# CalciferZh/MinimalOptiX

Measured on AMD Instinct MI355X. Metric: Mrays/s (primary+bounce+shadow rays traced per second, coffee.obj 1920x1080 256spp), higher is better.
Workload: dtype f32

## Files before the change

minimaloptix_amd/csrc/api_context.h:

```cpp
#pragma once
#include <hip/hip_runtime.h>

#include <initializer_list>
#include <string>
#include <vector>

#include "../../include/moptix.h"
#include "lbvh.h"
#include "megakernel.h"
#include "refitkernel.h"
#include "pt_signtopo.h"

struct ncclComm;

namespace pt { namespace api {

template <class T> struct DevBuf {
  T* p = nullptr; size_t n = 0;
  hipError_t ensure(size_t count) {
    if (count <= n && p) return hipSuccess;
    if (p) { (void)hipFree(p); p = nullptr; n = 0; }
    hipError_t e = hipMalloc((void**)&p, sizeof(T) * (count ? count : 1));
    if (e == hipSuccess) n = count ? count : 1;
    return e;
  }
  hipError_t upload(const std::vector<T>& v, hipStream_t s) {
    hipError_t e = ensure(v.size());
    if (e != hipSuccess || v.empty()) return e;
    return hipMemcpyAsync(p, v.data(), sizeof(T) * v.size(), hipMemcpyHostToDevice, s);
  }
  void release() { if (p) (void)hipFree(p); p = nullptr; n = 0; }
};

struct OrderList {
  long long units = -1;
  DevBuf<unsigned int> keys, keysSorted; DevBuf<int> order, iota; DevBuf<uint8_t> sortTmp;
  hipError_t ensure(long long n, hipStream_t stream);
  hipError_t sort(hipStream_t stream);
  void forget() { units = -1; }
  void release() { keys.release(); keysSorted.release(); order.release(); iota.release(); sortTmp.release(); units = -1; }
};

struct Options {
  int exitThreshold = 16, leafSize = 4, blocksPerCU = 3;
  int kernelVariant = -1;
  int tileMajor = 3;
  int starveLanes = 16, sampleBufMB = 16384, leafThreshold = 16, swapLanes = 32;
  int watchdogMs = 600000;
  int nodeFormat = 0;
  int fastShading = 0;
  int builder = 1;
  int analyticQueue = -1;
  int autoPacket = 1;
  int commBlocking = 0;
  int commTimeoutMs = 120000;
  int shadowRule = 1;
  int slotsInUse = -1;
  int drainBelow = 64;
  int auxDepth = 16;
  int specialize = 1;
  int queryBlocksPerCU = 32;
  int temporalFaceMotion = 0;
  int radianceBufferMB = 256;
};

}}

struct moptix_context_t {
  template <class T> using DevBuf = pt::api::DevBuf<T>;

  int device = 0;
  int numCUs = 256;
  hipStream_t stream = nullptr; bool ownStream = false;
  hipEvent_t ev0 = nullptr, ev1 = nullptr, ev2 = nullptr;
  std::string err;
  bool poisoned = false;
  moptix_params params{}; bool haveParams = false;
  int rank = 0, nRanks = 1;
  pt::api::Options opt;

  std::vector<pt::DevMaterial> mats;
  std::vector<pt::DevSphere> spheres; std::vector<int> sphereMat;
  std::vector<pt::DevQuad> quads;
  std::vector<pt::DevLight> lights;
  std::vector<float> facePos, faceNrm; std::vector<int> faceHasNrm, faceMat;
  std::vector<pt::TriUV> faceUV; bool anyUV = false;
  struct HostTexture { int width, height; std::vector<float> rgba; };
  std::vector<HostTexture> textures;
  bool sceneDirty = true, accelBuilt = false;
  DevBuf<pt::DevMaterial> dMats; DevBuf<pt::DevSphere> dSpheres; DevBuf<int> dSphereMat; DevBuf<pt::DevQuad> dQuads; DevBuf<pt::DevLight> dLights;
  DevBuf<float> dFacePos, dFaceNrm; DevBuf<int> dFaceHasNrm, dFaceMat;
  DevBuf<pt::TriUV> dFaceUV; DevBuf<float> dTexels; DevBuf<pt::DevTexture> dTextures;
  pt::LbvhResult bvh;
  double glassFaceShare = 0.0;
  void release_scene() {
    dMats.release(); dSpheres.release(); dSphereMat.release(); dQuads.release(); dLights.release();
    dFacePos.release(); dFaceNrm.release(); dFaceHasNrm.release(); dFaceMat.release();
    dFaceUV.release(); dTexels.release(); dTextures.release();
    pt::lbvh_free(&bvh);
  }

  DevBuf<float> dAccum; float* accumBound = nullptr; size_t accumPixels = 0;
  bool accumPlain = false;
  DevBuf<uint8_t> dRgb8;

  int nodeFormatUsed = 128;
  bool formatDecided = false;
  unsigned long long probeCounts[4] = { 0, 0, 0, 0 };
  int lastVariant = -1;
  int lastFeatures = pt::FEAT_ALL;
  int countedSpanUs = -1, countedTailUs = -1;
  double kernelMs = 0.0, reduceMs = 0.0; uint64_t nLaunches = 0;
  bool asyncPending = false;
  std::vector<int> seedStaging;
  DevBuf<int> dSeeds; DevBuf<int> dWork; DevBuf<unsigned long long> dCounters; DevBuf<int> dOverflow;
  DevBuf<uint8_t> dPoolCold; DevBuf<float> dSampleBuf;
  void release_render() {
    dSeeds.release(); dWork.release(); dCounters.release(); dOverflow.release(); dPoolCold.release(); dSampleBuf.release();
    tiles.release();
  }
  pt::api::OrderList tiles;

  struct Comm {
    ncclComm* handle = nullptr; int rank = 0, ranks = 1;
    bool nonBlocking = false;
    DevBuf<float> tileSend, tileRecv;
  } comm;

  struct Aov {
    DevBuf<float> albedo, normal, depth, hits; DevBuf<int> primId, matId;
    moptix_aov_buffers bound{};
    size_t pixels = 0;
    uint64_t samples = 0;
    DevBuf<int> seeds, work, overflow;
    void frame_resized() { pixels = 0; samples = 0; }
    void release() {
      albedo.release(); normal.release(); depth.release(); hits.release(); primId.release(); matId.release();
      seeds.release(); work.release(); overflow.release();
    }
  } aov;

  struct Denoise {
    DevBuf<pt::v4> colA, colB, guide, side; DevBuf<float> out;
    float* bound = nullptr;
    size_t pixels = 0;
    void release() { colA.release(); colB.release(); guide.release(); side.release(); out.release(); pixels = 0; }
  } dn;

  struct Temporal {
    DevBuf<pt::v4> col[2], guide[2], mom[2];
    DevBuf<pt::v4> motion;
    DevBuf<float> motionOut, historyOut;
    DevBuf<unsigned long long> counters;
    DevBuf<unsigned int> partials;
    std::vector<pt::v4> motionHost;
    int cur = 0;
    bool have = false;
    uint32_t width = 0, height = 0; int nSpheres = 0, demodulate = 0;
    moptix_cam_params cam{}; std::vector<pt::v3> centres;
    uint64_t frames = 0;
    size_t pixels = 0;
    unsigned long long last[4] = { 0, 0, 0, 0 };
    struct Faces {
      DevBuf<float> prev;
      DevBuf<pt::v4> rec;
      DevBuf<unsigned int> partials;
      DevBuf<unsigned long long> counters;
      bool have = false; size_t count = 0;
      bool changed = true;
      unsigned long long last[3] = { 0, 0, 0 };
      void release() { prev.release(); rec.release(); partials.release(); counters.release(); have = false; count = 0; }
    } faces;
    void drop() { have = false; frames = 0; faces.have = false; }
    void release() {
      for (int i = 0; i < 2; i++) { col[i].release(); guide[i].release(); mom[i].release(); }
      motion.release(); motionOut.release(); historyOut.release(); counters.release(); partials.release();
      faces.release();
      drop(); pixels = 0;
    }
  } tp;

  struct Adaptive {
    DevBuf<uint32_t> count; DevBuf<float> moments, error; DevBuf<uint8_t> converged;
    pt::api::OrderList order;
    DevBuf<unsigned int> partials, totals;
    DevBuf<float> mean;
    size_t pixels = 0;
    bool have = false;
    void drop() { pixels = 0; have = false; }
    void release() {
      count.release(); moments.release(); error.release(); converged.release();
      order.release(); partials.release(); totals.release(); mean.release();
      drop();
    }
  } ad;

  struct Query {
    DevBuf<int> overflow;
    DevBuf<float> rays; DevBuf<uint8_t> out;
    void drop() { overflow.release(); }
    void release() { drop(); rays.release(); out.release(); }
  } query;

  struct Radiance {
    DevBuf<int> overflow;
    DevBuf<float> scratch; DevBuf<int> work, seeds;
    int* seedStaging = nullptr; size_t seedStagingN = 0;
    hipEvent_t seedsUploaded = nullptr;
    DevBuf<float> rays, out; DevBuf<uint32_t> states;
    void drop() { overflow.release(); }
    void release() {
      drop(); scratch.release(); work.release(); seeds.release(); rays.release(); out.release(); states.release();
      if (seedStaging) (void)hipHostFree(seedStaging);
      if (seedsUploaded) (void)hipEventDestroy(seedsUploaded);
      seedStaging = nullptr; seedStagingN = 0; seedsUploaded = nullptr;
    }
  } radiance;

  struct Point {
    DevBuf<unsigned long long> overflow;
    DevBuf<float> points; DevBuf<uint8_t> out;
    void drop() { overflow.release(); }
    void release() { drop(); points.release(); out.release(); }
  } point;

  struct Sign {
    bool have = false, uploaded = false, stale = true;
    pt::SignTopology topo;
    uint32_t tableBuilds = 0;
    DevBuf<int> faceIds, vertexStart, vertexCorner, edgeStart, edgeFace;
    DevBuf<pt::SignFace> faces; DevBuf<pt::v4> vertexN, edgeN; DevBuf<pt::SignRecord> table;
    void release() {
      faceIds.release(); vertexStart.release(); vertexCorner.release(); edgeStart.release(); edgeFace.release();
      faces.release(); vertexN.release(); edgeN.release(); table.release();
      topo = pt::SignTopology(); have = false; uploaded = false; stale = true; tableBuilds = 0;
    }
  } sign;

  struct Refit {
    bool facesDirty = false, hostStale = false;
    size_t facesOnDevice = 0;
    bool planned = false;
    DevBuf<int> levelOrder; std::vector<int> levelFirst;
    DevBuf<pt::RefitBox> raw; DevBuf<uint32_t> sceneBox; DevBuf<double> partials; DevBuf<pt::RefitCost> cost; DevBuf<int> bad;
    struct Pinned { pt::RefitCost cost; int bad; }* pinned = nullptr;
    hipEvent_t e0 = nullptr, e1 = nullptr;
    moptix_refit_info info{};
    void drop() {
      levelOrder.release(); levelFirst.clear(); raw.release(); sceneBox.release(); partials.release(); cost.release(); bad.release();
      if (pinned) (void)hipHostFree(pinned);
      if (e0) (void)hipEventDestroy(e0);
      if (e1) (void)hipEventDestroy(e1);
      pinned = nullptr; e0 = nullptr; e1 = nullptr; planned = false; info = moptix_refit_info{};
    }
  } refit;
};

namespace pt {
struct DenoiseConsts;
namespace api {

int fail(moptix_context c, int code, const std::string& msg);
int hipFail(moptix_context c, hipError_t e, const char* what);
#define HIPCHK(c, x, what) do { hipError_t e_ = (x); if (e_ != hipSuccess) return pt::api::hipFail((c), e_, (what)); } while (0)

int check_ready(moptix_context c);
int fetch_faces(moptix_context c);
int sign_table_for_query(moptix_context c, const SignRecord*& table);
void sign_release(moptix_context c);
float* accum_ptr(moptix_context c);
int ensure_accum(moptix_context c);
int begin_call(moptix_context c, bool withAccum);
struct ReadBack { void* dst; const void* src; size_t bytes; };
int read_back(moptix_context c, std::initializer_list<ReadBack> copies, const char* what);
void fill_view(moptix_context c, SceneView& v);
int scene_features(moptix_context c);
int fill_query_view(moptix_context c, SceneView& v);
moptix_aov_buffers aov_ptrs(moptix_context c);
void comm_release(moptix_context c);
int denoise_begin(moptix_context c, bool ownGuide, size_t& px);
void denoise_consts(moptix_context c, const moptix_denoise_params* p, DenoiseConsts& k);
inline float* denoise_out(moptix_context c) { return c->dn.bound ? c->dn.bound : c->dn.out.p; }

struct LaunchPlan {
  const TraceKernel* kernel;
  int variant;
  int features;
  int nItems, tilesX;
  int nBlocks;
  long long perPass;
  int slotsInUse, auxDepth, drainBelow, ovfDepth;
  int tileMajor, unitShift; long long historyUnits;
  size_t poolBytes, overflowInts, workInts;
};
struct RenderLaunch {
  LaunchPlan p; LaunchArgs a;
  long long perPass;
  int handoutDivisor, handoutSeeds;
  bool counted, fast;
};
struct PassOverride {
  const int* order; int nWork;
  hipError_t (*reduce)(hipStream_t stream, const LaunchArgs& a, void* user); void* user;
};
int prepare_launch(moptix_context c, int32_t nSeeds, bool counted, bool byPixelSlots, RenderLaunch& r);
int launch_pass(moptix_context c, RenderLaunch& r, const int* dSeeds, int n, const PassOverride* over);

}}
```

minimaloptix_amd/csrc/api_options.hip:

```cpp
#include <climits>
#include <cstring>

#include "api_context.h"

using namespace pt;
using namespace pt::api;

namespace {

enum Invalidates { kNothing, kAccelIfChanged, kNodeFormat, kTileHistory, kFaceSnapshot };
struct Option {
  const char* name;
  int Options::* member;
  int (*read)(moptix_context) = nullptr;
  int lo = 0, hi = 0;
  const char* accepted = "";
  Invalidates invalidates = kNothing;
  int nValues = 0, values[4] = { 0, 0, 0, 0 };
  bool can_set() const { return !read; }
  bool can_get() const { return member || read; }
};

static_assert(kMaxLeaf == 8, "leaf_size's message says [1,8]");
const Option kOptions[] = {
  { "exit_threshold", &Options::exitThreshold, nullptr, 0, 64, "in [0,64]" },
  { "leaf_size", &Options::leafSize, nullptr, 1, kMaxLeaf, "in [1,8]", kAccelIfChanged },
  { "blocks_per_cu", &Options::blocksPerCU, nullptr, 1, 8, "in [1,8]" },
  { "kernel_variant", &Options::kernelVariant, nullptr, 0, 0, "in {-1,0,3,4} (1 and 2 were removed in round 3)", kNothing, 4, { -1, 0, 3, 4 } },
  { "sample_buffer_mb", &Options::sampleBufMB, nullptr, 1, INT_MAX, ">= 1" },
  { "leaf_threshold", &Options::leafThreshold, nullptr, 1, 64, "in [1,64]" },
  { "swap_lanes", &Options::swapLanes, nullptr, 1, 64, "in [1,64]" },
  { "starve_lanes", &Options::starveLanes, nullptr, 1, 64, "in [1,64]" },
  { "tile_major", &Options::tileMajor, nullptr, 0, 3, "in {0,1,2,3}" },
  { "auto_packet", &Options::autoPacket, nullptr, 0, 1, "in {0,1}" },
  { "analytic_queue", &Options::analyticQueue, nullptr, -1, 1, "in {-1,0,1}" },
  { "aux_depth", &Options::auxDepth, nullptr, 0, 100000, "in [0,100000]" },
  { "drain_below", &Options::drainBelow, nullptr, 0, 64, "in [0,64]" },
  { "specialize", &Options::specialize, nullptr, 0, 1, "in {0,1}" },
  { "slots_in_use", &Options::slotsInUse, nullptr, -1, 1024, "in [-1,1024]" },
  { "builder", &Options::builder, nullptr, 0, 1, "in {0,1}", kAccelIfChanged },
  { "fast_shading", &Options::fastShading, nullptr, 0, 1, "in {0,1}" },
  { "node_format", &Options::nodeFormat, nullptr, 0, 0, "in {0,64,128}", kNodeFormat, 3, { 0, 64, 128 } },
  { "shadow_rule", &Options::shadowRule, nullptr, 0, 1, "in {0,1}" },
  { "watchdog_ms", &Options::watchdogMs, nullptr, 1, INT_MAX, ">= 1" },
  { "comm_timeout_ms", &Options::commTimeoutMs, nullptr, 1, INT_MAX, ">= 1" },
  { "comm_blocking", &Options::commBlocking, nullptr, 0, 1, "in {0,1}" },
  { "query_blocks_per_cu", &Options::queryBlocksPerCU, nullptr, 1, 64, "in [1,64]" },
  { "radiance_buffer_mb", &Options::radianceBufferMB, nullptr, 1, 16384, "in [1,16384]" },
  { "temporal_face_motion", &Options::temporalFaceMotion, nullptr, 0, 1, "in {0,1}", kFaceSnapshot },
  { "forget_history", nullptr, nullptr, INT_MIN, INT_MAX, "", kTileHistory },
  { "comm_nonblocking_used", nullptr, [](moptix_context c) { return c->comm.nonBlocking ? 1 : 0; } },
  { "node_format_used", nullptr, [](moptix_context c) { return c->nodeFormatUsed; } },
  { "kernel_variant_used", nullptr, [](moptix_context c) { return c->lastVariant; } },
  { "kernel_features_used", nullptr, [](moptix_context c) { return c->lastFeatures; } },
  { "counted_span_us", nullptr, [](moptix_context c) { return c->countedSpanUs; } },
  { "counted_tail_us", nullptr, [](moptix_context c) { return c->countedTailUs; } },
  { "path_slots", nullptr, [](moptix_context) { return packetkernel_slots(); } },
  { "comm_ranks", nullptr, [](moptix_context c) { return c->comm.handle ? c->comm.ranks : 0; } },
  { "num_cus", nullptr, [](moptix_context c) { return c->numCUs; } },
};
const Option* find_option(const char* name) {
  for (const Option& o : kOptions) if (!strcmp(name, o.name)) return &o;
  return nullptr;
}

}

extern "C" {

int moptix_set_option(moptix_context c, const char* name, int32_t value) {
  if (!c || !name) return MOPTIX_ERR_INVALID;
  const Option* o = find_option(name);
  if (!o || !o->can_set()) return fail(c, MOPTIX_ERR_INVALID, std::string("unknown option: ") + name);
  bool ok = o->nValues == 0 && value >= o->lo && value <= o->hi;
  for (int i = 0; i < o->nValues; i++) ok = ok || value == o->values[i];
  if (!ok) return fail(c, MOPTIX_ERR_INVALID, std::string(name) + " " + o->accepted);
  if (o->invalidates == kAccelIfChanged && value != c->opt.*o->member) c->accelBuilt = false;
  if (o->invalidates == kNodeFormat) c->formatDecided = false;
  if (o->invalidates == kTileHistory) c->tiles.forget();
  if (o->invalidates == kFaceSnapshot && value == 0 && c->tp.faces.prev.p) {
    (void)hipSetDevice(c->device);
    if (!c->poisoned) (void)hipStreamSynchronize(c->stream);
    c->tp.faces.release();
  }
  if (o->invalidates == kFaceSnapshot && value == 0) c->tp.faces.have = false;
  if (o->member) c->opt.*o->member = value;
  return MOPTIX_OK;
}

int moptix_get_option(moptix_context c, const char* name, int32_t* value) {
  if (!c || !name || !value) return MOPTIX_ERR_INVALID;
  const Option* o = find_option(name);
  if (!o || !o->can_get()) return fail(c, MOPTIX_ERR_INVALID, std::string("unknown option: ") + name);
  *value = o->member ? c->opt.*o->member : o->read(c);
  return MOPTIX_OK;
}

}
```

minimaloptix_amd/csrc/api_render.hip:

```cpp
#include <rocprim/rocprim.hpp>

#include <algorithm>
#include <cstdio>
#include <cstdlib>
#include <cstring>

#include "api_context.h"
#include "pt_lanestack.h"

using namespace pt;
using namespace pt::api;

namespace {

constexpr int kProbeWidth = 128;
int choose_node_format(moptix_context c) {
  c->formatDecided = true;
  c->nodeFormatUsed = 128;
  for (auto& v : c->probeCounts) v = 0;
  if (c->bvh.nNodes <= 0 || !c->bvh.nodes64) return MOPTIX_OK;
  if (c->opt.nodeFormat != 0) { c->nodeFormatUsed = c->opt.nodeFormat; return MOPTIX_OK; }
  SceneView v; fill_view(c, v);
  v.nodes64 = c->bvh.nodes64;
  const int w = std::min(kProbeWidth, v.width), h = std::max(1, (int)((long long)v.height * w / std::max(1, v.width)));
  v.width = w; v.height = h;
  const size_t threads = ((size_t)w * h + 255) / 256 * 256;
  unsigned long long* dOut = nullptr; int* dOvf = nullptr;
  hipError_t e = hipMalloc((void**)&dOut, 4 * sizeof(unsigned long long));
  if (e == hipSuccess) e = hipMemsetAsync(dOut, 0, 4 * sizeof(unsigned long long), c->stream);
  const size_t ovf = lane_stack_overflow_entries(threads, c->bvh.stackBound, megakernel_lds_stack_entries());
  if (e == hipSuccess && ovf > 0) e = hipMalloc((void**)&dOvf, sizeof(int) * ovf);
  if (e == hipSuccess) e = launch_probe_paths(c->stream, v, 0, false, dOut, dOvf);
  if (e == hipSuccess) e = launch_probe_paths(c->stream, v, 0, true, dOut + 2, dOvf);
  if (e == hipSuccess) e = hipMemcpyAsync(c->probeCounts, dOut, 4 * sizeof(unsigned long long), hipMemcpyDeviceToHost, c->stream);
  if (e == hipSuccess) e = hipStreamSynchronize(c->stream);
  if (dOut) (void)hipFree(dOut);
  if (dOvf) (void)hipFree(dOvf);
  if (e != hipSuccess) return hipFail(c, e, "node format probe");
  const double cost128 = (double)c->probeCounts[0] + 1.3 * (double)c->probeCounts[1];
  const double cost64 = 0.93 * (double)c->probeCounts[2] + 1.3 * (double)c->probeCounts[3];
  c->nodeFormatUsed = cost64 < cost128 ? 64 : 128;
  if (getenv("MOPTIX_DEBUG"))
    fprintf(stderr, "[moptix] node format probe (%dx%d paths): 128-byte nodes %llu steps %llu triangle tests, 64-byte %llu / %llu -> %d\n", w, h,
            c->probeCounts[0], c->probeCounts[1], c->probeCounts[2], c->probeCounts[3], c->nodeFormatUsed);
  return MOPTIX_OK;
}

void report_counters(const unsigned long long* h) {
  fprintf(stderr, "[moptix] batches %llu lanes %llu full %llu allidle %llu waitingSum %llu\n", h[kCntShadeBatches], h[kCntShadeBatchLanes], h[kCntLeafBacklog], h[kCntIdleSpins], h[kCntRingBacklog]);
  const double tt = (double)h[kCntTWave];
  fprintf(stderr, "[moptix] wave time: batch %.1f%% refill %.1f%% node %.1f%% leaf %.1f%% finish %.1f%% (steps %llu, cycles/wave %.3g)\n",
          100 * h[kCntTBatch] / tt, 100 * h[kCntTSwap] / tt, 100 * h[kCntTNode] / tt, 100 * h[kCntTLeaf] / tt, 100 * h[kCntTFinish] / tt, h[kCntTraversalSteps], tt);
  fprintf(stderr, "[moptix] idle spins %llu\n", h[kCntIdleSpins]);
  if (h[kCntLastWaveOut] && h[kCntFirstWaveIn] != ~0ull && h[kCntLastWaveOut] > h[kCntFirstWaveIn])
    fprintf(stderr, "[moptix] pass ticks: batch %llu (load %llu run %llu store %llu) node %llu leaf %llu txn %llu lock %llu local %llu idle %llu | waves' time %llu over a span of %.1f us | "
                    "batches %llu node runs %llu leaf passes %llu iterations %llu transactions %llu\n", h[kCntTBatch], h[kCntTBatchLoad], h[kCntTBatchRun], h[kCntTBatchStore], h[kCntTNode], h[kCntTLeaf], h[kCntTTxn], h[kCntTLock], h[kCntTLocal], h[kCntTIdle], h[kCntTWave],
            (double)(h[kCntLastWaveOut] - h[kCntFirstWaveIn]) * 1e-2, h[kCntShadeBatches], h[kCntNodeRuns], h[kCntLeafPasses], h[kCntIterations], h[kCntTransactions]);
  if (h[kCntIterations]) fprintf(stderr, "[moptix] swap detail: local %.1f%% lock-wait %.1f%% txn %.1f%% idle %.1f%% | batch detail: load %.1f%% run %.1f%% store %.1f%% | "
                     "iterations %llu transactions %llu (cycles/iter %.0f)\n", 100 * h[kCntTLocal] / tt, 100 * h[kCntTLock] / tt, 100 * h[kCntTTxn] / tt, 100 * h[kCntTIdle] / tt,
                     100 * h[kCntTBatchLoad] / tt, 100 * h[kCntTBatchRun] / tt, 100 * h[kCntTBatchStore] / tt, h[kCntIterations], h[kCntTransactions], tt / (double)h[kCntIterations]);
  if (h[kCntLastWaveOut]) fprintf(stderr, "[moptix] timeline (100 MHz clock): items ran out %.2f ms after the first wave started, last wave left %.2f ms after that\n",
                     (double)(h[kCntItemsRanOut] - h[kCntFirstWaveIn]) * 1e-5, (double)(h[kCntLastWaveOut] - h[kCntItemsRanOut]) * 1e-5);
  if (h[kCntLastWaveOut]) {
    int lastB = 0; for (int b = 0; b < kCntTailBuckets; b++) if (h[kCntTailCount + b]) lastB = b;
    const int ranOut = (int)((double)(h[kCntItemsRanOut] - h[kCntFirstWaveIn]) * 1e-5);
    fprintf(stderr, "[moptix] samples finishing per ms from the moment the items ran out (count, mean depth, max depth):");
    for (int b = ranOut > 2 ? ranOut - 2 : 0; b <= lastB; b++)
      fprintf(stderr, " [%d: %llu %.1f %llu]", b, h[kCntTailCount + b], h[kCntTailCount + b] ? (double)h[kCntTailDepthSum + b] / (double)h[kCntTailCount + b] : 0.0, h[kCntTailMaxDepth + b]);
    fprintf(stderr, "\n");
  }
  if (h[kCntNodeRuns]) fprintf(stderr, "[moptix] node runs %llu: node-ready slots waiting in the wave's ring %.1f, leaf ring %.1f (averages at the start of a run)\n",
                     h[kCntNodeRuns], (double)h[kCntRingBacklog] / (double)h[kCntNodeRuns], (double)h[kCntLeafBacklog] / (double)h[kCntNodeRuns]);
  if (h[kCntIterations]) fprintf(stderr, "[moptix] batch iterations executing on_result %llu, on_lights %llu, new item %llu (batches %llu)\n", h[kCntIterResult], h[kCntIterLights], h[kCntIterNewItem], h[kCntShadeBatches]);
  if ((h[kCntSlotRows] | h[kCntSlotRows + 1])) {
    const double rays = (double)(h[kCntPrimaryRays] + h[kCntBounceRays] + h[kCntShadowRays]);
    fprintf(stderr, "[moptix] slot-record rows (16 B each) per ray: shading visit loads %.2f stores %.2f | leaf pass loads %.2f stores %.2f | total %.1f B per ray in %.2f shading visits and %.2f leaf visits per ray\n",
            h[kCntSlotRows] / rays, h[kCntSlotRows + 1] / rays, h[kCntSlotRows + 2] / rays, h[kCntSlotRows + 3] / rays, 16.0 * (double)(h[kCntSlotRows] + h[kCntSlotRows + 1] + h[kCntSlotRows + 2] + h[kCntSlotRows + 3]) / rays, (double)h[kCntShadeBatchLanes] / rays, (double)h[kCntLeafLanes] / rays);
  }
  if ((h[kCntHandedOver] | h[kCntDrainTaken])) fprintf(stderr, "[moptix] hand-over: %llu paths handed over by the packet kernel, %llu taken by the drain kernel; samples finished: %llu by the packet kernel + %llu by the drain kernel (of %llu)\n", h[kCntHandedOver], h[kCntDrainTaken], h[kCntPacketFinished], h[kCntDrainFinished], h[kCntSamples]);
  if (h[kCntLeafPasses]) fprintf(stderr, "[moptix] node steps %llu (%.1f lanes avg), leaf passes %llu (%.1f lanes avg)\n", h[kCntTraversalSteps] - h[kCntLeafPasses],
          (double)(h[kCntActiveLaneSteps] - h[kCntLeafLanes]) / (double)(h[kCntTraversalSteps] - h[kCntLeafPasses]), h[kCntLeafPasses], (double)h[kCntLeafLanes] / (double)h[kCntLeafPasses]);
  if (h[kCntCensusWaves]) {
    static const char* names[kCensusRegions] = { "result visit (on_result_packet)", "  miss", "  closest hit (hit_attributes + material)", "    light material",
      "    depth cap", "    lambertian", "    metal", "    glass", "    disney GLASS", "    disney (on_lights_packet)", "      light 0 faces: pdf + eval", "      light 1 faces: pdf + eval",
      "      light 2 faces: pdf + eval", "      bounce: pdf + eval", "new work item (begin_sample)", "leaf pass: triangle 0 tested", "leaf pass: triangle 1 tested",
      "leaf pass: triangle 2 tested", "leaf pass: triangle 3 tested", "  triangle hit accepted by tri_test", "  shadow result folded", "      light draw (per light)", "      bounce: disney_sample", "node step: branched tail (stack nearly full)" };
    fprintf(stderr, "[moptix] lane census: region | waves that entered | lanes that entered | lanes per wave (of 64)\n");
    for (int i = 0; i < kCensusRegions; i++)
      if (h[kCntCensusWaves + i]) fprintf(stderr, "[moptix]   %-46s %12llu %14llu %6.1f\n", names[i], h[kCntCensusWaves + i], h[kCntCensusLanes + i], (double)h[kCntCensusLanes + i] / (double)h[kCntCensusWaves + i]);
  }
}

int read_stats(moptix_context c, moptix_stats* stats) {
  unsigned long long h[kCntTotal] = {};
  HIPCHK(c, hipMemcpy(h, c->dCounters.p, sizeof(h), hipMemcpyDeviceToHost), "read counters");
  stats->samples = h[kCntSamples]; stats->primaryRays = h[kCntPrimaryRays]; stats->bounceRays = h[kCntBounceRays]; stats->shadowRays = h[kCntShadowRays];
  stats->nodeFetches = h[kCntNodeFetches]; stats->triTests = h[kCntTriTests]; stats->closestHits = h[kCntClosestHits]; stats->lightLoads = h[kCntLightLoads];
  stats->analyticTests = h[kCntAnalyticTests]; stats->traversalSteps = h[kCntTraversalSteps]; stats->activeLaneSteps = h[kCntActiveLaneSteps];
  stats->shadeBatches = h[kCntShadeBatches]; stats->shadeBatchLanes = h[kCntShadeBatchLanes];
  c->countedSpanUs = -1; c->countedTailUs = -1;
  if (h[kCntLastWaveOut] && h[kCntFirstWaveIn] != ~0ull) { c->countedSpanUs = (int)((h[kCntLastWaveOut] - h[kCntFirstWaveIn]) / 100); c->countedTailUs = (h[kCntItemsRanOut] != ~0ull && h[kCntLastWaveOut] > h[kCntItemsRanOut]) ? (int)((h[kCntLastWaveOut] - h[kCntItemsRanOut]) / 100) : 0; }
  if (getenv("MOPTIX_DEBUG")) report_counters(h);
  return MOPTIX_OK;
}

int plan_launch(moptix_context c, const SceneView& scene, int32_t nSeeds, bool byPixelSlots, LaunchPlan& p) {
  memset(&p, 0, sizeof(p));
  const int tilesX = ((int)c->params.width + 7) / 8, tilesY = ((int)c->params.height + 7) / 8;
  const long long nTiles = (long long)tilesX * tilesY;
  const long long localTiles = (nTiles + c->nRanks - 1) / c->nRanks;
  if (localTiles * 64 > 0x7fffffffLL) return fail(c, MOPTIX_ERR_LIMIT, "frame too large");
  p.nItems = (int)(localTiles * 64); p.tilesX = tilesX;
  if (p.nItems == 0) return MOPTIX_OK;
  const long long budget = (long long)c->opt.sampleBufMB << 20;
  p.perPass = budget / ((long long)p.nItems * 12);
  p.nBlocks = c->numCUs * c->opt.blocksPerCU;
  const long long counterSlack = (long long)c->numCUs * std::max(4, c->opt.blocksPerCU) * 1024 + 65536;
  if ((long long)p.nItems + counterSlack > 0x7fffffffLL) return fail(c, MOPTIX_ERR_LIMIT, "frame too large");
  p.perPass = std::min(p.perPass, (0x7fffffffLL - counterSlack) / p.nItems);
  p.perPass = std::max(1LL, std::min(p.perPass, (long long)nSeeds));

  const bool hasTris = scene.rootRef != kEmptyRef;
  const bool analyticQueue = c->opt.analyticQueue >= 0 ? c->opt.analyticQueue != 0 : (c->spheres.size() + c->quads.size() >= 64);
  const bool packetOk = hasTris && scene.nLights <= 3 && !scene.anyDisneyAnalytic;
  const double nSamples = (double)p.nItems * (double)nSeeds;
  const bool autoPacket = nSamples >= 1.0e6 && nSeeds >= 16;
  const bool variantExplicit = c->opt.kernelVariant >= 0;
  const int variant = variantExplicit ? c->opt.kernelVariant : 3;
  const bool usePacket = packetOk && (variant == 4 || (!variantExplicit && c->opt.autoPacket != 0 && autoPacket));
  const bool useQueue = !usePacket && (byPixelSlots || ((variant >= 3) && (hasTris || analyticQueue)));
  p.kernel = usePacket ? &kPacketKernel : !useQueue ? nullptr : hasTris ? &kQueueKernel : &kLeanQueueKernel;
  p.variant = usePacket ? 4 : useQueue ? 3 : 0;
  const bool faceTableOk = (unsigned long long)tri_face_offset(0) + (unsigned long long)scene.nTris * (sizeof(TriShade) + sizeof(TriFace)) + 64ull < (1ull << 32);
  p.features = (usePacket && c->opt.specialize != 0 && faceTableOk) ? scene_features(c) : FEAT_ALL;
  if (p.kernel == &kLeanQueueKernel && c->opt.blocksPerCU == 3) p.nBlocks = c->numCUs * 4;
  p.slotsInUse = c->opt.slotsInUse >= 0 ? c->opt.slotsInUse : (usePacket && c->opt.auxDepth > 0 && nSamples < 1.0e8 && c->glassFaceShare <= 0.5 ? packetkernel_slots() * 7 / 8 : 0);
  p.auxDepth = usePacket ? c->opt.auxDepth : 0;
  if (usePacket) {
    bool glassMaterial = false;
    for (const DevMaterial& m : c->mats) if (m.kind == MAT_DISNEY && m.brdfType == BRDF_GLASS) glassMaterial = true;
    p.drainBelow = (glassMaterial && !scene.shadowNearest) ? 0 : c->opt.drainBelow;
  }
  if (p.kernel) {
    p.ovfDepth = hasTris ? std::max(0, c->bvh.stackBound - p.kernel->lds_stack_entries() + 1) : 0;
    p.overflowInts = p.ovfDepth > 0 ? p.kernel->overflow_ints(p.nBlocks, p.ovfDepth) : 0;
    p.poolBytes = p.kernel->cold_bytes(p.nBlocks);
  } else {
    p.overflowInts = lane_stack_overflow_entries((size_t)p.nBlocks * 256, c->bvh.stackBound, megakernel_lds_stack_entries());
  }
  p.workInts = kHandoutWords + 2 + drain_list_ints(p.nBlocks, p.drainBelow);
  p.tileMajor = byPixelSlots ? 3 : p.kernel ? c->opt.tileMajor : 0;
  p.unitShift = p.tileMajor == 3 ? 0 : 6;
  p.historyUnits = (localTiles * 64) >> p.unitShift;
  return MOPTIX_OK;
}

int report_tile_history(moptix_context c) {
  std::vector<unsigned int> cost((size_t)c->tiles.units);
  HIPCHK(c, hipMemcpy(cost.data(), c->tiles.keys.p, sizeof(unsigned int) * cost.size(), hipMemcpyDeviceToHost), "read tile cost");
  size_t hist[6] = { 0, 0, 0, 0, 0, 0 };
  for (size_t i = 0; i < cost.size(); i++) {
    const unsigned int v = cost[i];
    hist[v == 0 ? 0 : v < 16 ? 1 : v < 64 ? 2 : v < 256 ? 3 : 4]++;
    if (v >= 256 && i < cost.size() / 2) hist[5]++;
  }
  fprintf(stderr, "[moptix] depth history (%zu units): none %zu, depth 8-15 %zu, 16-63 %zu, 64-255 %zu, capped %zu (of which %zu in the first half)\n",
          cost.size(), hist[0], hist[1], hist[2], hist[3], hist[4], hist[5]);
  return MOPTIX_OK;
}

#ifdef PT_EVLOG
constexpr size_t kEvLogWords = 65536;
int evlog_begin(moptix_context c, DevBuf<unsigned long long>& evLog, LaunchArgs& a) {
  HIPCHK(c, evLog.ensure(kEvLogWords + 8), "alloc event log");
  HIPCHK(c, hipMemsetAsync(evLog.p, 0, sizeof(unsigned long long) * (kEvLogWords + 8), c->stream), "zero event log");
  a.evLog = evLog.p;
  return MOPTIX_OK;
}
int evlog_write(moptix_context c, const DevBuf<unsigned long long>& evLog) {
  std::vector<unsigned long long> h(kEvLogWords);
  HIPCHK(c, hipMemcpy(h.data(), evLog.p, sizeof(unsigned long long) * h.size(), hipMemcpyDeviceToHost), "read event log");
  FILE* f = fopen(getenv("MOPTIX_EVLOG"), "wb");
  if (f) { fwrite(h.data(), sizeof(unsigned long long), (size_t)std::min<unsigned long long>(h[0], 65000ull) + 1, f); fclose(f); }
  return MOPTIX_OK;
}
#endif

}

namespace pt { namespace api {

int prepare_launch(moptix_context c, int32_t nSeeds, bool counted, bool byPixelSlots, RenderLaunch& r) {
  int rc;
  if (!c->formatDecided && (rc = choose_node_format(c)) != MOPTIX_OK) return rc;
  LaunchArgs& a = r.a;
  LaunchPlan& p = r.p;
  memset(&a, 0, sizeof(a));
  fill_view(c, a.scene);
  if ((rc = plan_launch(c, a.scene, nSeeds, byPixelSlots, p)) != MOPTIX_OK || p.nItems == 0) return rc;
  c->lastVariant = p.variant;
  r.counted = counted; r.fast = c->opt.fastShading != 0;
  c->lastFeatures = p.kernel == &kPacketKernel ? packetkernel_features(r.counted, r.fast, p.features) : FEAT_ALL;

  a.accum = accum_ptr(c);
  a.nItems = p.nItems; a.tilesX = p.tilesX; a.rank = c->rank; a.nRanks = c->nRanks;
  a.exitThreshold = c->opt.exitThreshold; a.leafThreshold = c->opt.leafThreshold;
  a.starveLanes = c->opt.starveLanes; a.swapLanes = c->opt.swapLanes;
  a.slotsInUse = p.slotsInUse; a.auxDepth = p.auxDepth; a.ovfDepth = p.ovfDepth;
  a.watchdogTicks = (unsigned long long)c->opt.watchdogMs * 100000ull;
  if (p.overflowInts > 0) {
    HIPCHK(c, c->dOverflow.ensure(p.overflowInts), "alloc stack overflow area");
    a.stackOverflow = c->dOverflow.p;
  }
  if (p.kernel) {
    HIPCHK(c, c->dPoolCold.ensure(p.poolBytes), "alloc path pool");
    a.poolCold = c->dPoolCold.p;
  }
  long long perPass = p.perPass;
  for (;;) {
    const hipError_t e = c->dSampleBuf.ensure((size_t)perPass * a.nItems * 3);
    if (e == hipSuccess) break;
    if (e != hipErrorOutOfMemory || perPass <= 1) return hipFail(c, e, "alloc per-sample buffer");
    (void)hipGetLastError();
    perPass = (perPass + 1) / 2;
  }
  r.perPass = perPass;
  a.sampleBuf = c->dSampleBuf.p;
  HIPCHK(c, c->dWork.ensure(p.workInts), "alloc work counter");
  {
    struct { HandoutConsts hc; int hdr[2 + kDrainEntries]; } w = { handout_consts(p.tileMajor, a.nItems, (int)std::min<long long>(perPass, nSeeds), a.tilesX, a.nRanks),
                                                                   { 0, 0, 0, 0, 0, 0, p.nBlocks * p.drainBelow, p.drainBelow } };
    static_assert(sizeof(w) == sizeof(int) * (kHandoutWords + 2 + kDrainEntries), "the work header is packed");
    HIPCHK(c, hipMemcpyAsync(c->dWork.p, &w, sizeof(w), hipMemcpyHostToDevice, c->stream), "init work counter");
    HIPCHK(c, hipStreamSynchronize(c->stream), "sync");
    r.handoutDivisor = handout_divisor(p.tileMajor, a.nItems, (int)std::min<long long>(perPass, nSeeds)); r.handoutSeeds = (int)std::min<long long>(perPass, nSeeds);
  }
  a.workCounter = c->dWork.p + kHandoutWords;
  a.tileMajor = p.tileMajor; a.unitShift = p.unitShift;
  if (p.tileMajor) {
    HIPCHK(c, c->tiles.ensure(p.historyUnits, c->stream), "start depth history");
    a.tileOrder = c->tiles.order.p; a.tileCost = c->tiles.keys.p;
  }
  if (counted) {
    HIPCHK(c, c->dCounters.ensure(kCntTotal), "alloc counters");
    HIPCHK(c, hipMemsetAsync(c->dCounters.p, 0, sizeof(unsigned long long) * kCntTotal, c->stream), "zero counters");
    HIPCHK(c, hipMemsetAsync(c->dCounters.p + kCntFirstWaveIn, 0xff, sizeof(unsigned long long) * 2, c->stream), "init min counters");
    a.counters = c->dCounters.p;
  }
  return MOPTIX_OK;
}

static hipError_t sort_pairs_desc(void* tmp, size_t& tmpBytes, OrderList& l, size_t n, hipStream_t stream) {
  return rocprim::radix_sort_pairs_desc(tmp, tmpBytes, l.keys.p, l.keysSorted.p, l.iota.p, l.order.p, n, 0, 32, stream);
}

hipError_t OrderList::ensure(long long n, hipStream_t stream) {
  if (units == n) return hipSuccess;
  units = -1;
  std::vector<int> ids((size_t)n);
  for (size_t i = 0; i < ids.size(); i++) ids[i] = (int)i;
  hipError_t e = keys.ensure((size_t)n);
  if (e == hipSuccess) e = keysSorted.ensure((size_t)n);
  if (e == hipSuccess) e = order.ensure((size_t)n);
  if (e == hipSuccess) e = iota.upload(ids, stream);
  if (e == hipSuccess) e = hipMemsetAsync(keys.p, 0, sizeof(unsigned int) * (size_t)n, stream);
  size_t tmpBytes = 0;
  if (e == hipSuccess) e = sort_pairs_desc(nullptr, tmpBytes, *this, (size_t)n, stream);
  if (e == hipSuccess) e = sortTmp.ensure(tmpBytes);
  if (e == hipSuccess) e = hipStreamSynchronize(stream);
  if (e == hipSuccess) units = n;
  return e;
}

hipError_t OrderList::sort(hipStream_t stream) {
  size_t tmpBytes = sortTmp.n;
  return sort_pairs_desc(sortTmp.p, tmpBytes, *this, (size_t)units, stream);
}

int launch_pass(moptix_context c, RenderLaunch& r, const int* dSeeds, int n, const PassOverride* over) {
  LaunchArgs& a = r.a;
  const LaunchPlan& p = r.p;
  a.seeds = dSeeds; a.nSeeds = n; a.nWork = over ? over->nWork : n * a.nItems;
  if (handout_divisor(a.tileMajor, a.nItems, n) != r.handoutDivisor || n != r.handoutSeeds) {
    const HandoutConsts hc = handout_consts(a.tileMajor, a.nItems, n, a.tilesX, a.nRanks);
    HIPCHK(c, hipMemcpyAsync(a.workCounter - kHandoutWords, &hc, sizeof(hc), hipMemcpyHostToDevice, c->stream), "write hand-out constants");
    HIPCHK(c, hipStreamSynchronize(c->stream), "sync");
    r.handoutDivisor = handout_divisor(a.tileMajor, a.nItems, n); r.handoutSeeds = n;
  }
  HIPCHK(c, hipMemsetAsync(a.workCounter, 0, (2 + kDrainCap) * sizeof(int), c->stream), "zero work counter");
  if (over) a.tileOrder = over->order;
  else if (a.tileMajor && a.tileCost) HIPCHK(c, c->tiles.sort(c->stream), "sort tiles");
  HIPCHK(c, hipEventRecord(c->ev0, c->stream), "event");
  if (p.kernel) HIPCHK(c, p.kernel->launch(c->stream, a, p.nBlocks, r.counted, r.fast, p.features), p.kernel->launchWhat);
  else HIPCHK(c, launch_megakernel(c->stream, a, p.nBlocks, r.counted), "launch megakernel");
  if (p.drainBelow > 0) HIPCHK(c, launch_drainkernel(c->stream, a, c->numCUs, r.counted, r.fast), "launch drain kernel");
  else if (p.kernel == &kPacketKernel) HIPCHK(c, launch_megakernel(c->stream, a, p.nBlocks, r.counted), "launch megakernel");
  HIPCHK(c, hipEventRecord(c->ev1, c->stream), "event");
  if (over) HIPCHK(c, over->reduce(c->stream, a, over->user), "launch adaptive reduction");
  else HIPCHK(c, launch_reduce_samples(c->stream, a), "launch sample reduction");
  HIPCHK(c, hipEventRecord(c->ev2, c->stream), "event");
  c->asyncPending = true;
  return MOPTIX_OK;
}

}}

namespace {

int do_render(moptix_context c, const int32_t* seeds, int32_t nSeeds, bool counted, bool blocking, moptix_stats* stats) {
  int rc = check_ready(c);
  if (rc != MOPTIX_OK) return rc;
  if (nSeeds < 0 || (nSeeds > 0 && !seeds)) return fail(c, MOPTIX_ERR_INVALID, "bad seeds");
  if (c->ad.have) return fail(c, MOPTIX_ERR_STATE, "the accumulation buffer holds an adaptive render (per-pixel sample counts): moptix_adaptive_clear or moptix_accum_clear first");
  if ((rc = begin_call(c, true)) != MOPTIX_OK) return rc;
  if (nSeeds == 0) return MOPTIX_OK;
  RenderLaunch r;
  if ((rc = prepare_launch(c, nSeeds, counted, false, r)) != MOPTIX_OK || r.p.nItems == 0) return rc;
#ifdef PT_EVLOG
  DevBuf<unsigned long long> evLog;
  if ((rc = evlog_begin(c, evLog, r.a)) != MOPTIX_OK) return rc;
#endif
  c->seedStaging.assign(seeds, seeds + nSeeds);
  HIPCHK(c, c->dSeeds.upload(c->seedStaging, c->stream), "upload seeds");
  c->accumPlain = true;

  for (long long first = 0; first < nSeeds; first += r.perPass) {
    const int n = (int)std::min(r.perPass, (long long)nSeeds - first);
    if ((rc = launch_pass(c, r, c->dSeeds.p + first, n, nullptr)) != MOPTIX_OK) return rc;
    const bool last = first + r.perPass >= nSeeds;
    if (!last || blocking) { if ((rc = moptix_sync(c)) != MOPTIX_OK) return rc; }
  }
#ifdef PT_EVLOG
  if (blocking && !counted && getenv("MOPTIX_EVLOG") && (rc = evlog_write(c, evLog)) != MOPTIX_OK) return rc;
  evLog.release();
#endif
  if (blocking && r.a.tileCost && getenv("MOPTIX_DEBUG") && (rc = report_tile_history(c)) != MOPTIX_OK) return rc;
  if (blocking && counted && stats) return read_stats(c, stats);
  return MOPTIX_OK;
}

}

extern "C" {

int moptix_launch(moptix_context c, int32_t randSeed) { return do_render(c, &randSeed, 1, false, true, nullptr); }
int moptix_render(moptix_context c, const int32_t* seeds, int32_t nSeeds) { return do_render(c, seeds, nSeeds, false, true, nullptr); }
int moptix_render_async(moptix_context c, const int32_t* seeds, int32_t nSeeds) { return do_render(c, seeds, nSeeds, false, false, nullptr); }
int moptix_render_counted(moptix_context c, const int32_t* seeds, int32_t nSeeds, moptix_stats* out) {
  if (out) memset(out, 0, sizeof(*out));
  return do_render(c, seeds, nSeeds, true, true, out);
}

int moptix_sync(moptix_context c) {
  if (!c) return MOPTIX_ERR_INVALID;
  HIPCHK(c, hipStreamSynchronize(c->stream), "stream synchronize");
  if (c->asyncPending) {
    float ms = 0.f, ms2 = 0.f;
    if (hipEventElapsedTime(&ms, c->ev0, c->ev1) == hipSuccess) { c->kernelMs += ms; c->nLaunches++; }
    if (hipEventElapsedTime(&ms2, c->ev1, c->ev2) == hipSuccess) c->reduceMs += ms2;
    c->asyncPending = false;
    int flags[2] = { 0, 0 };
    if (c->dWork.p) HIPCHK(c, hipMemcpy(flags, c->dWork.p + kHandoutWords, sizeof(flags), hipMemcpyDeviceToHost), "read watchdog flag");
    if (flags[1] != 0) return fail(c, MOPTIX_ERR_HIP, "render kernel hit its watchdog (option watchdog_ms); this pass was not added to accuBuffer");
  }
  return MOPTIX_OK;
}

}
```

minimaloptix_amd/csrc/megakernel.h:

```cpp
#pragma once
#include <hip/hip_runtime.h>
#include "pt_counters.h"
#include "pt_types.h"

namespace pt {

struct LaunchArgs {
  SceneView scene;
  const int* seeds; int nSeeds;
  float* accum;
  float* sampleBuf;
  int* workCounter;
  int nItems;
  int nWork;
  int tilesX; int rank, nRanks;
  int exitThreshold;
  int leafThreshold;
  int* stackOverflow;
  unsigned long long* counters;
  void* poolCold;
  int starveLanes;
  int swapLanes;
  int ovfDepth;
  int slotsInUse;
  int auxDepth;
  unsigned long long watchdogTicks;
  int tileMajor;
  int unitShift;
  const int* tileOrder;
  unsigned int* tileCost;
#ifdef PT_EVLOG
  unsigned long long* evLog;
#endif
};
constexpr int kDeepPath = 8;
constexpr int kDrainDeep = 24;
constexpr int kDrainList = 2, kDrainDeepN = 0, kDrainNext = 1, kDrainOtherN = 2, kDrainCap = 4, kDrainBelow = 5, kDrainEntries = 6;

PT_HD bool item_to_pixel(const LaunchArgs& a, int k, int& sample, int& pixel) {
  sample = k / a.nItems;
  const int i = k - sample * a.nItems;
  const int lt = i >> 6, in = i & 63;
  const int gt = lt * a.nRanks + (a.rank + lt) % a.nRanks;
  const int tx = gt % a.tilesX, ty = gt / a.tilesX;
  const int x = tx * 8 + (in & 7), y = ty * 8 + (in >> 3);
  pixel = y * a.scene.width + x;
  return (x < a.scene.width) & (y < a.scene.height);
}
PT_HD int handout_to_item(const LaunchArgs& a, int k) {
  if (!a.tileMajor) return k;
  if (a.tileMajor == 3) {
    const int ui = k / a.nSeeds, sample = k - ui * a.nSeeds;
    return sample * a.nItems + (a.tileOrder ? a.tileOrder[ui] : ui);
  }
  const int per = a.nSeeds << 6;
  const int ti = k / per, r = k - ti * per;
  const int lt = a.tileOrder ? a.tileOrder[ti] : ti;
  if (a.tileMajor == 2) {
    const int in = r / a.nSeeds, sample = r - in * a.nSeeds;
    return sample * a.nItems + (lt << 6) + in;
  }
  return (r >> 6) * a.nItems + (lt << 6) + (r & 63);
}
struct MagicDiv { unsigned int mul, shift; };
struct HandoutConsts { MagicDiv first, tilesX, ranks, seeds; };
constexpr int kHandoutWords = 8;
static_assert(sizeof(HandoutConsts) == kHandoutWords * sizeof(int), "HandoutConsts is kHandoutWords ints");
inline MagicDiv magic_div(int d) {
  int l = 0;
  while ((1ll << l) < (long long)d) l++;
  MagicDiv m; m.shift = 31u + (unsigned int)l;
  m.mul = (unsigned int)(((1ull << m.shift) + (unsigned long long)d - 1ull) / (unsigned long long)d);
  return m;
}
PT_HD int magic_quot(int n, MagicDiv m) { return (int)(((unsigned long long)(unsigned int)n * (unsigned long long)m.mul) >> m.shift); }
inline int handout_divisor(int tileMajor, int nItems, int nSeeds) { return !tileMajor ? nItems : tileMajor == 3 ? nSeeds : nSeeds << 6; }
inline HandoutConsts handout_consts(int tileMajor, int nItems, int nSeeds, int tilesX, int nRanks) {
  HandoutConsts h;
  h.first = magic_div(handout_divisor(tileMajor, nItems, nSeeds)); h.tilesX = magic_div(tilesX); h.ranks = magic_div(nRanks); h.seeds = magic_div(nSeeds);
  return h;
}

struct WorkItem { int item, sample, x, y, pixel; };
PT_HD bool handout_lean(const LaunchArgs& a, const HandoutConsts* hc, int k, WorkItem& w) {
  int slot;
  const int q = magic_quot(k, load_uniform(&hc->first));
  if (!a.tileMajor) {
    w.sample = q; slot = k - q * a.nItems;
  } else if (a.tileMajor == 3) {
    w.sample = k - q * a.nSeeds;
    slot = a.tileOrder ? a.tileOrder[q] : q;
  } else {
    const int r = k - q * (a.nSeeds << 6);
    const int lt = a.tileOrder ? a.tileOrder[q] : q;
    int in;
    if (a.tileMajor == 2) { in = magic_quot(r, load_uniform(&hc->seeds)); w.sample = r - in * a.nSeeds; }
    else { w.sample = r >> 6; in = r & 63; }
    slot = (lt << 6) + in;
  }
  w.item = a.tileMajor ? w.sample * a.nItems + slot : k;
  const int lt = slot >> 6, in = slot & 63;
  int gt = lt;
  if (__builtin_expect(a.nRanks != 1, 0)) { const int s = a.rank + lt; gt = lt * a.nRanks + (s - magic_quot(s, load_uniform(&hc->ranks)) * a.nRanks); }
  const int ty = magic_quot(gt, load_uniform(&hc->tilesX)), tx = gt - ty * a.tilesX;
  w.x = tx * 8 + (in & 7); w.y = ty * 8 + (in >> 3);
  w.pixel = w.y * a.scene.width + w.x;
  return (w.x < a.scene.width) & (w.y < a.scene.height);
}
#if defined(__HIPCC__)
__device__ __forceinline__ void store_sample(const LaunchArgs& a, int item, v3 value) {
  float* sp = a.sampleBuf + 3 * (size_t)item;
  sp[0] = value.x; sp[1] = value.y; sp[2] = value.z;
}
#endif

int megakernel_lds_stack_entries();
hipError_t launch_reduce_samples(hipStream_t stream, const LaunchArgs& a);
hipError_t launch_megakernel(hipStream_t stream, const LaunchArgs& a, int nBlocks, bool counted);
int queuekernel_lds_stack_entries();
int queuekernel_slots();
size_t queuekernel_cold_bytes(int nBlocks);
size_t queuekernel_overflow_ints(int nBlocks, int ovfDepth);
hipError_t launch_queuekernel(hipStream_t stream, const LaunchArgs& a, int nBlocks, bool counted, bool fastShading, int features);
int queuekernel_lds_stack_entries_lean();
int queuekernel_slots_lean();
size_t queuekernel_cold_bytes_lean(int nBlocks);
size_t queuekernel_overflow_ints_lean(int nBlocks, int ovfDepth);
hipError_t launch_queuekernel_lean(hipStream_t stream, const LaunchArgs& a, int nBlocks, bool counted, bool fastShading, int features);
int packetkernel_lds_stack_entries();
int packetkernel_slots();
size_t packetkernel_cold_bytes(int nBlocks);
size_t packetkernel_overflow_ints(int nBlocks, int ovfDepth);
hipError_t launch_packetkernel(hipStream_t stream, const LaunchArgs& a, int nBlocks, bool counted, bool fastShading, int features);
int packetkernel_features(bool counted, bool fastShading, int sceneFeatures);
struct TraceKernel {
  const char* launchWhat;
  int (*lds_stack_entries)();
  size_t (*cold_bytes)(int nBlocks);
  size_t (*overflow_ints)(int nBlocks, int ovfDepth);
  hipError_t (*launch)(hipStream_t stream, const LaunchArgs& a, int nBlocks, bool counted, bool fastShading, int features);
};
inline constexpr TraceKernel kQueueKernel = { "launch queue megakernel", queuekernel_lds_stack_entries, queuekernel_cold_bytes, queuekernel_overflow_ints, launch_queuekernel };
inline constexpr TraceKernel kLeanQueueKernel = { "launch queue megakernel (lean)", queuekernel_lds_stack_entries_lean, queuekernel_cold_bytes_lean, queuekernel_overflow_ints_lean, launch_queuekernel_lean };
inline constexpr TraceKernel kPacketKernel = { "launch packet megakernel", packetkernel_lds_stack_entries, packetkernel_cold_bytes, packetkernel_overflow_ints, launch_packetkernel };
hipError_t launch_drainkernel(hipStream_t stream, const LaunchArgs& a, int nCUs, bool counted, bool fastShading);
size_t drain_list_ints(int nBlocks, int drainBelow);
hipError_t launch_debug_trace(hipStream_t stream, const SceneView& sc, const float* dRays, int n, float* dT, int* dPrim, int* stackOverflow);
hipError_t launch_probe_paths(hipStream_t stream, const SceneView& sc, int launchSeed, bool node64, unsigned long long* dOut, int* stackOverflow);
hipError_t launch_resolve_rgb8(hipStream_t stream, float* accum, int width, int height, float nAccumulation, int clearBuffer, uint8_t* dOut);

}
```

minimaloptix_amd/csrc/packetkernel.hip:

```cpp
#include <hip/hip_runtime.h>

#include "megakernel.h"
#include "pt_lanestack.h"
#include "pt_path.h"
#include "pt_packet.h"
#include "pt_slot.h"

namespace pt {

namespace {

constexpr int kBlockThreads = 256;
constexpr int kWaves = kBlockThreads / 64;
#ifndef PT_PK_KP
#define PT_PK_KP 144
#endif
#ifndef PT_PK_STACKN
#define PT_PK_STACKN 9
#endif
#define PT_KP PT_PK_KP
#define PT_STACKN PT_PK_STACKN
#ifndef PT_WAVES_PER_SIMD
#define PT_WAVES_PER_SIMD 3
#endif
constexpr int kP = PT_KP;
constexpr int kStackN = PT_STACKN;
constexpr int kWavesPerSimd = PT_WAVES_PER_SIMD;
constexpr int ring_capacity(int n) { return n; }
template <int NS> __device__ __forceinline__ int ring_wrap(int i) {
  if constexpr ((NS & (NS - 1)) == 0) return i & (NS - 1); else return i >= NS ? i - NS : i;
}
static_assert(PT_KP * kWaves <= (1 << kSlotBits), "slot ids are 10 bits");


enum { Q_SHADE = 0, Q_GEN = 1, kNumQ = 2, Q_NODE = 2, Q_LEAF = 3, DEST_DONE = 4, DEST_NONE = -1 };

template <int NS>
struct PoolLds {
  v4 nodeA[NS];
  v4 nodeB[NS];
  int stack[NS][kStackN + 1];
  unsigned short queue[kNumQ][ring_capacity(NS)];
  int qHead[kNumQ], qCount[kNumQ];
  int done, lock;
  int drainAt;
  unsigned int freeMask[NS / 32];
  int nFree;
};

template <int NS>
struct WavePriv {
  unsigned short qnode[ring_capacity(NS)];
  unsigned short qleaf[256];
  unsigned short outbox[2][160];
};

typedef __attribute__((address_space(3))) int lds_int;

struct SlotStack {
  lds_int* lds;
  int* ovf;
  __device__ __forceinline__ void store(int sp, int v) {
    if (__builtin_expect(sp < kStackN, 1)) lds[sp] = v; else ovf[sp - kStackN] = v;
  }
  __device__ __forceinline__ int load(int sp) const {
    int v;
    if (__builtin_expect(sp < kStackN, 1)) v = lds[sp]; else v = ovf[sp - kStackN];
    return v;
  }
  __device__ __forceinline__ bool roomy(int sp) const { return sp + 3 <= kStackN; }
  __device__ __forceinline__ void store_fast(int sp, int v) { lds[sp] = v; }
  static constexpr bool kFlat = true;
  __device__ __forceinline__ bool fits_fast(int sp, int m) const { return sp + m <= kStackN && sp < kStackN; }
  __device__ __forceinline__ int peek_fast(int sp) const { return lds[min(sp, kStackN) - 1]; }
};

__device__ __forceinline__ const LaunchArgs& fresh_args() {
  typedef __attribute__((address_space(4))) const LaunchArgs CA;
  unsigned long long p = (unsigned long long)__builtin_amdgcn_kernarg_segment_ptr();
  asm volatile("" : "+s"(p));
  return *(const LaunchArgs*)(CA*)p;
}

__device__ __forceinline__ int route(int node, int kind, int bestPrim) {
  if (node == kTravDone) return (kind == RK_SHADOW || bestPrim >= 0) ? Q_SHADE : Q_GEN;
  return node >= 0 ? Q_NODE : Q_LEAF;
}

struct SlotSink {
  SlotCold* cold; int slot; v4* nodeA; v4* nodeB; int (*stack)[kStackN + 1]; const PathState* ps; int root;
  int axp;
  __device__ __forceinline__ void shadow(int j, v3 d, float tmax, v3 w, float inv) const {
    SlotCold* cw = at32(cold, slot);
    slot_store(&cw->pend[j], mk4(w.x, w.y, w.z, inv));
    if (axp >= 0) {
      const int ax = (axp >> (kSlotBits * j)) & kSlotMask;
      nodeA[ax] = mk4(ps->o.x, ps->o.y, ps->o.z, tmax); nodeB[ax] = mk4(d.x, d.y, d.z, i2f(root));
      stack[ax][0] = kAuxSlot | kShadowRay | (1 << kNShShift) | aux_parent_bits(slot);
    } else if (j == 0) { nodeA[slot] = mk4(ps->o.x, ps->o.y, ps->o.z, tmax); nodeB[slot] = mk4(d.x, d.y, d.z, i2f(root)); }
    else slot_store(&cw->ray[j - 1], mk4(d.x, d.y, d.z, tmax));
  }
};

template <bool CNT, bool SHARED, bool FAST = false, bool NEAR = false, bool N64 = false>
__global__ void __launch_bounds__(kBlockThreads, kWavesPerSimd) pt_packetkernel(const LaunchArgs a) {
  constexpr int F = 0;
#include "packetkernel_body.h"
}
template <bool CNT, bool SHARED, bool FAST = false, bool NEAR = false, bool N64 = false>
__global__ void __launch_bounds__(kBlockThreads, kWavesPerSimd) pt_packetkernel_general(const LaunchArgs a) {
  constexpr int F = FEAT_ALL;
#include "packetkernel_body.h"
}

}

#ifndef PT_PK_N128
int packetkernel_features(bool counted, bool fastShading, int sceneFeatures) { return (counted || fastShading || sceneFeatures != 0) ? FEAT_ALL : 0; }
int packetkernel_lds_stack_entries() { return kStackN; }
int packetkernel_slots() { return kP * kWaves; }
size_t packetkernel_cold_bytes(int nBlocks) { return (size_t)nBlocks * kWaves * kP * sizeof(SlotCold); }
size_t packetkernel_overflow_ints(int nBlocks, int ovfDepth) { return (size_t)nBlocks * kWaves * kP * (size_t)ovfDepth; }
constexpr bool kThisFileN64 = true;
#define PT_PK_LAUNCH launch_packetkernel_n64
#else
constexpr bool kThisFileN64 = false;
#define PT_PK_LAUNCH launch_packetkernel_n128
#endif

template <bool CNT, bool FAST>
static void launch_pk(dim3 grid, dim3 block, hipStream_t stream, const LaunchArgs& a) {
  if (a.scene.shadowNearest) pt_packetkernel_general<CNT, true, FAST, true, kThisFileN64><<<grid, block, 0, stream>>>(a);
  else                       pt_packetkernel_general<CNT, true, FAST, false, kThisFileN64><<<grid, block, 0, stream>>>(a);
}
hipError_t PT_PK_LAUNCH(hipStream_t stream, const LaunchArgs& a, int nBlocks, bool counted, bool fastShading, int features) {
  dim3 grid(nBlocks), block(kBlockThreads);
  if (packetkernel_features(counted, fastShading, features) == 0) {
    if (a.scene.shadowNearest) pt_packetkernel<false, true, false, true, kThisFileN64><<<grid, block, 0, stream>>>(a);
    else                       pt_packetkernel<false, true, false, false, kThisFileN64><<<grid, block, 0, stream>>>(a);
  } else if (fastShading) { if (counted) launch_pk<true, true>(grid, block, stream, a); else launch_pk<false, true>(grid, block, stream, a); }
  else             { if (counted) launch_pk<true, false>(grid, block, stream, a); else launch_pk<false, false>(grid, block, stream, a); }
  return hipGetLastError();
}
#ifndef PT_PK_N128
hipError_t launch_packetkernel_n128(hipStream_t stream, const LaunchArgs& a, int nBlocks, bool counted, bool fastShading, int features);
hipError_t launch_packetkernel(hipStream_t stream, const LaunchArgs& a, int nBlocks, bool counted, bool fastShading, int features) {
  return a.scene.nodes64 != nullptr ? launch_packetkernel_n64(stream, a, nBlocks, counted, fastShading, features) : launch_packetkernel_n128(stream, a, nBlocks, counted, fastShading, features);
}
#endif

}
```

minimaloptix_amd/csrc/packetkernel_body.h:

```cpp
  constexpr int NS = SHARED ? kP * kWaves : kP;
  __shared__ PoolLds<NS> sPool[SHARED ? 1 : kWaves];
  __shared__ WavePriv<NS> sPriv[kWaves];
#ifdef PT_EVLOG
  __shared__ int sEvOn;
  if (threadIdx.x == 0) sEvOn = 0;
#define PT_EV(code, val) do { if (sEvOn && (threadIdx.x & 63) == 0) { const unsigned long long i_ = atomicAdd(a.evLog, 1ull); \
    if (i_ < 65000ull) a.evLog[1 + i_] = (__builtin_amdgcn_s_memrealtime() << 24) | (((unsigned long long)(val) & 0xffffull) << 8) | ((unsigned long long)(threadIdx.x >> 6) << 4) | (unsigned long long)(code); } } while (0)
#else
#define PT_EV(code, val) do { } while (0)
#endif

  SceneView scv = a.scene;
  scv.shadowNearest = NEAR ? 1 : 0;
  const SceneView& sc = scv;
  const int lane = threadIdx.x & 63, wave = threadIdx.x >> 6;
  PoolLds<NS>& W = sPool[SHARED ? 0 : wave];
  const int gpool = SHARED ? blockIdx.x : blockIdx.x * kWaves + wave;
  SlotCold* cold = reinterpret_cast<SlotCold*>(a.poolCold) + (size_t)gpool * NS;
  int* ovfBase = a.stackOverflow ? a.stackOverflow + (size_t)gpool * NS * a.ovfDepth : nullptr;

  unsigned long long tLocal = 0, tLock = 0, tTxn = 0, tIdle = 0, tBLoad = 0, tBRun = 0, tBStore = 0, nTxn = 0, nIter = 0;
  unsigned long long tSub = 0, nIterResult = 0, nIterLights = 0, nIterGen = 0, nodeRuns = 0, ringBacklog = 0, leafBacklog = 0;
#define PT_SUB0() do { if (CNT) tSub = __builtin_amdgcn_s_memtime(); } while (0)
#define PT_SUB(acc) do { if (CNT) { const unsigned long long now_ = __builtin_amdgcn_s_memtime(); acc += now_ - tSub; tSub = now_; } } while (0)
  int qHead[kNumQ] = { 0, 0 }, qCount[kNumQ] = { 0, 0 };
  int nDone = 0;

  [[maybe_unused]] auto q_push = [&](int q, bool pred, int slot) {
    const unsigned long long m = __ballot(pred);
    if (m == 0ull) return;
    if (pred) W.queue[q][ring_wrap<NS>(qHead[q] + qCount[q] + lane_rank(m))] = (unsigned short)slot;
    qCount[q] += __popcll(m);
  };
  auto q_pop = [&](int q, bool want) -> int {
    const unsigned long long m = __ballot(want);
    const int n = min((int)__popcll(m), qCount[q]);
    int slot = -1;
    if (want) { const int r = lane_rank(m); if (r < n) slot = W.queue[q][ring_wrap<NS>(qHead[q] + r)]; }
    qHead[q] = ring_wrap<NS>(qHead[q] + n);
    qCount[q] -= n;
    return slot;
  };
  auto txn_begin = [&]() {
    if constexpr (SHARED) {
      if (lane == 0) { while (atomicCAS(&W.lock, 0, 1) != 0) __builtin_amdgcn_s_sleep(1); }
      __builtin_amdgcn_fence(__ATOMIC_ACQUIRE, "workgroup");
      if (CNT) { (void)__builtin_amdgcn_readfirstlane(W.lock); PT_SUB(tLock); nTxn++; }
      for (int q = 0; q < kNumQ; q++) {
        qHead[q] = __builtin_amdgcn_readfirstlane(W.qHead[q]);
        qCount[q] = __builtin_amdgcn_readfirstlane(W.qCount[q]);
      }
      nDone = __builtin_amdgcn_readfirstlane(W.done);
    }
  };
  auto txn_end = [&]() {
    if constexpr (SHARED) {
      if (lane == 0) {
        for (int q = 0; q < kNumQ; q++) { W.qHead[q] = qHead[q]; W.qCount[q] = qCount[q]; }
        W.done = nDone;
      }
      __builtin_amdgcn_fence(__ATOMIC_RELEASE, "workgroup");
      if (lane == 0) __hip_atomic_store(&W.lock, 0, __ATOMIC_RELAXED, __HIP_MEMORY_SCOPE_WORKGROUP);
    }
  };
  auto make_stack = [&](int slot) {
    SlotStack st;
    st.lds = (lds_int*)&W.stack[slot][1];
    st.ovf = ovfBase ? reinterpret_cast<int*>(reinterpret_cast<char*>(ovfBase) + (uint32_t)((uint32_t)slot * (uint32_t)a.ovfDepth * 4u)) : nullptr;
    return st;
  };

  auto store_flags = [&](int slot, int value) {
    if (__builtin_expect((value & kHasAux) != 0, 0)) { atomicAnd(&W.stack[slot][0], kJoinMask); atomicOr(&W.stack[slot][0], value & ~kJoinMask); }
    else W.stack[slot][0] = value;
  };
  auto arrive_parks = [&](int slot) -> bool {
    const int old = atomicOr(&W.stack[slot][0], kArrived);
    return ((old >> kJoinShift) & 3) != 0;
  };
  auto aux_done = [&](int fl, int& dest) -> int {
    const int parent = aux_parent(fl);
    const int old = atomicSub(&W.stack[parent][0], 1 << kJoinShift);
    const bool last = (old & kJoinMask) == ((1 << kJoinShift) | kArrived);
    dest = last ? ((old & kShadeFlag) ? Q_SHADE : Q_GEN) : DEST_NONE;
    return last ? parent : -1;
  };

  const bool auxOn = SHARED && a.auxDepth > 0 && sc.rootRef >= 0;
  const int nUse = (a.slotsInUse > 0 && a.slotsInUse < NS) ? (SHARED ? a.slotsInUse : max(64, a.slotsInUse / kWaves)) : NS;
  {
    if (SHARED && threadIdx.x < NS / 32) {
      const int lo = (int)threadIdx.x * 32;
      W.freeMask[threadIdx.x] = !auxOn || nUse >= lo + 32 ? 0u : (nUse <= lo ? ~0u : ~0u << (nUse - lo));
    }
    if (threadIdx.x == 0) W.nFree = auxOn ? NS - nUse : 0;
    const int first = SHARED ? threadIdx.x : lane, step = SHARED ? kBlockThreads : 64;
    for (int s = first; s < nUse; s += step) {
      i4 ctl; ctl.x = -1; ctl.y = 0; ctl.z = 0; ctl.w = M_NEW_PIXEL;
      cold[s].ctl = ctl;
      W.stack[s][0] = 0;
      W.queue[Q_GEN][s] = (unsigned short)s;
    }
    if constexpr (SHARED) {
      if (threadIdx.x == 0) {
        for (int q = 0; q < kNumQ; q++) { W.qHead[q] = 0; W.qCount[q] = 0; }
        W.qCount[Q_GEN] = nUse; const int below = a.workCounter[kDrainList + kDrainBelow];
        W.done = NS - nUse; W.drainAt = below > 0 ? max(NS - below, NS - nUse + 1) : 0x7fff; W.lock = 0;
      }
      __builtin_amdgcn_fence(__ATOMIC_RELEASE, "workgroup");
      __syncthreads();
    } else {
      qCount[Q_GEN] = nUse; nDone = NS - nUse;
      __builtin_amdgcn_fence(__ATOMIC_RELEASE, "workgroup");
    }
  }

  Counters ct = {};
  uint32_t rows[4] = { 0, 0, 0, 0 };
#define PT_ROWS(i, n) do { if (CNT) rows[i] += (uint32_t)(n); } while (0)
  uint32_t nodeSteps = 0, nodeLanes = 0, leafPasses = 0, leafLanes = 0, batches = 0, batchLanes = 0, idleSpins = 0;
  unsigned long long tBatch = 0, tSwap = 0, tNode = 0, tLeaf = 0, tStamp = 0;
  const unsigned long long tStart = CNT ? __builtin_amdgcn_s_memtime() : 0ull;
  [[maybe_unused]] const unsigned long long rtStart = CNT ? __builtin_amdgcn_s_memrealtime() : 0ull;
#define PT_STAMP(acc) do { if (CNT) { const unsigned long long now_ = __builtin_amdgcn_s_memtime(); acc += now_ - tStamp; tStamp = now_; } } while (0)
  tStamp = tStart;

  int ns = -1;
  int nsFlag = 0;
  PathState nray;
  nray.o = mk3(0, 0, 0); nray.tmin = sc.epsT; nray.d = mk3(0, 0, 1); nray.tmax = 0; nray.kind = RK_RADIANCE; nray.mode = M_TRACE;
  Trav ntv;
  ntv.node = kTravDone; ntv.sp = 0; ntv.tbest = 0; ntv.inv = mk3(0, 0, 0); ntv.noi = mk3(0, 0, 0); ntv.bestPrim = -1; ntv.bestTri = -1;
  ntv.beta = 0; ntv.gamma = 0; ntv.att = mk3(1, 1, 1); ntv.started = 1;

  int pendSlot = -1, pendDest = DEST_NONE;

  unsigned short* myNodeQ = sPriv[wave].qnode;
  int nqHead = 0, nqCount = 0;
  unsigned short* myLeafQ = sPriv[wave].qleaf;
  int lqHead = 0, lqCount = 0;
  int obCount[2] = { 0, 0 };
  int localDone = 0;
  auto local_push = [&](int dest, int slot) {
    {
      const unsigned long long m = __ballot(dest == Q_NODE);
      if (m != 0ull) {
        if (dest == Q_NODE) myNodeQ[ring_wrap<NS>(nqHead + nqCount + lane_rank(m))] = (unsigned short)slot;
        nqCount += __popcll(m);
      }
    }
    {
      const unsigned long long m = __ballot(dest == Q_LEAF);
      if (m != 0ull) {
        if (dest == Q_LEAF) myLeafQ[(lqHead + lqCount + lane_rank(m)) & 255] = (unsigned short)slot;
        lqCount += __popcll(m);
      }
    }
    for (int d = 0; d < 2; d++) {
      const unsigned long long m = __ballot(dest == Q_SHADE + d);
      if (m != 0ull) {
        if (dest == Q_SHADE + d) sPriv[wave].outbox[d][obCount[d] + lane_rank(m)] = (unsigned short)slot;
        obCount[d] += __popcll(m);
      }
    }
    localDone += __popcll(__ballot(dest == DEST_DONE));
  };

  auto leaf_pass = [&](int slot) {
    const LaunchArgs& a = fresh_args();
    SceneView scl = a.scene; scl.shadowNearest = NEAR ? 1 : 0;
    const SceneView& sc = scl;
    const bool have = slot >= 0;
    if (CNT) { leafPasses++; leafLanes += (uint32_t)__popcll(__ballot(have)); }
    PT_EV(7, __popcll(__ballot(have)));
    pendSlot = slot; pendDest = DEST_NONE;
    __builtin_amdgcn_fence(__ATOMIC_RELEASE, "workgroup");
    __builtin_amdgcn_fence(__ATOMIC_ACQUIRE, "workgroup");
    if (have) {
      const v4 na = W.nodeA[slot], nb = W.nodeB[slot];
      const int fl = W.stack[slot][0];
      const int node0 = f2i(nb.w);
      const bool isSwitch = node0 == kSwitchRef;
      const bool shadow = (fl & kShadowRay) != 0, hitValid = (fl & kHitValid) != 0;
      const int cur = fl_cur(fl);
      const SlotCold* cs = at32(cold, slot);
      LeafChunk ch;
      leaf_fetch4(sc, isSwitch ? make_leaf_ref(0, 1) : node0, 0, ch);
      v4 wr = mk4(0.f, 0.f, 1.f, 0.f), wn = mk4(0.f, 0.f, 1.f, 0.f);
      const bool more = fl_more(fl);
      if (more && (isSwitch || shadow || (fl & kSpMask) == 0)) { wn = slot_load(&cs->ray[cur]); PT_ROWS(2, 1); }
      if (!isSwitch) {
        if (shadow) { if (fl_stat(fl, cur) == 2) { wr = slot_load(&cs->att[cur]); PT_ROWS(2, 1); } }
      }
      auto next_ray = [&](int flags) {
        const int nxt = cur + 1;
        const bool nshadow = nxt < fl_nsh(flags);
        W.nodeB[slot] = mk4(wn.x, wn.y, wn.z, i2f(sc.rootRef));
        W.nodeA[slot].w = wn.w;
        W.stack[slot][0] = (flags & ~(kSpMask | (3 << kCurShift) | kShadowRay)) | (nxt << kCurShift) | (nshadow ? kShadowRay : 0);
        pendDest = sc.rootRef >= 0 ? Q_NODE : Q_LEAF;
      };
      if (isSwitch) {
        next_ray(fl);
      } else {
        PathState ps; Trav tv;
        ps.tmin = sc.epsT; ps.mode = M_TRACE;
        ps.o = mk3(na.x, na.y, na.z); ps.d = mk3(nb.x, nb.y, nb.z);
        ps.kind = shadow ? RK_SHADOW : RK_RADIANCE;
        ps.tmax = shadow ? na.w : kRtDefaultMax;
        tv.inv = mk3(0.f, 0.f, 0.f); tv.tbest = na.w;
        tv.node = node0; tv.sp = fl & kSpMask;
        tv.bestTri = -1; tv.bestPrim = -1; tv.beta = 0.f; tv.gamma = 0.f; tv.att = mk3(1.f, 1.f, 1.f); tv.bestCls = SHADOW_NONE;
        if (shadow) { if (fl_stat(fl, cur) == 2) { tv.att = mk3(wr.x, wr.y, wr.z); if (sc.shadowNearest) tv.bestPrim = f2i(wr.w); } }
        else if (hitValid) tv.bestPrim = kPrimUnknown;
        const int oldPrim = tv.bestPrim;
        const v3 oldAtt = tv.att;
        SlotStack st = make_stack(slot);
        trav_leaf_step_fetched<CNT>(sc, ps, tv, st, ct, ch);
        int nfl = fl & ~kSpMask;
        if (shadow) {
          if (sc.shadowNearest) {
            if (tv.bestPrim != oldPrim) {
              nfl = (nfl & ~(3 << (kStatShift + 2 * cur))) | (2 << (kStatShift + 2 * cur));
              slot_store(&at32(cold, slot)->att[cur], mk4(tv.att.x, tv.att.y, tv.att.z, i2f(tv.bestPrim))); PT_ROWS(3, 1);
            }
          } else if (tv.att.x != oldAtt.x || tv.att.y != oldAtt.y || tv.att.z != oldAtt.z) {
            const bool zero = tv.att.x == 0.f && tv.att.y == 0.f && tv.att.z == 0.f;
            nfl = (nfl & ~(3 << (kStatShift + 2 * cur))) | ((zero ? 1 : 2) << (kStatShift + 2 * cur));
            if (!zero) { slot_store(&at32(cold, slot)->att[cur], mk4(tv.att.x, tv.att.y, tv.att.z, 0.f)); PT_ROWS(3, 1); }
          }
        } else if (tv.bestPrim != oldPrim) {
          bool keep = true;
          if (hitValid && tv.tbest == na.w) { const v4 held = slot_load(&cs->hit); PT_ROWS(2, 1); keep = !(f2i(held.y) < tv.bestPrim); }
          if (keep) {
            slot_store(&at32(cold, slot)->hit, mk4(i2f(tv.bestTri), i2f(tv.bestPrim), tv.beta, tv.gamma)); PT_ROWS(3, 1);
            nfl = (nfl & ~kShadeFlag) | kHitValid | (tv.bestCls == SHADOW_OPAQUE ? kShadeFlag : 0);
          }
        }
        if (tv.node == kTravDone && more) {
          next_ray(nfl);
        } else {
          W.nodeA[slot].w = tv.tbest;
          W.nodeB[slot].w = i2f(tv.node);
          store_flags(slot, tv.sp | nfl);
          pendDest = tv.node == kTravDone ? ((nfl & kShadeFlag) ? Q_SHADE : Q_GEN) : (tv.node >= 0 ? Q_NODE : Q_LEAF);
          if (__builtin_expect(tv.node == kTravDone && (nfl & (kHasAux | kAuxSlot)) != 0, 0)) {
            if (nfl & kAuxSlot) {
              __builtin_amdgcn_fence(__ATOMIC_RELEASE, "workgroup");
              pendSlot = aux_done(nfl, pendDest);
            } else if (arrive_parks(slot)) pendDest = DEST_NONE;
          }
        }
      }
    }
    if constexpr (!SHARED) __builtin_amdgcn_fence(__ATOMIC_RELEASE, "workgroup");
    PT_EV(8, 0);
  };

  auto run_batch = [&](int slot, bool shadeBatch) {
    const LaunchArgs& a = fresh_args();
    SceneView scl = a.scene; scl.shadowNearest = NEAR ? 1 : 0;
    const SceneView& sc = scl;
    const bool have = slot >= 0;
    if (CNT) { batches++; batchLanes += (uint32_t)__popcll(__ballot(have)); }
    PT_EV(1, __popcll(__ballot(have)));
    PT_SUB0();
    pendSlot = slot; pendDest = DEST_NONE;
    PathState ps; Trav res;
    ps.mode = M_DONE; ps.kind = RK_RADIANCE;
    res.node = kTravDone; res.bestPrim = -1;
    __builtin_amdgcn_fence(__ATOMIC_RELEASE, "workgroup");
    __builtin_amdgcn_fence(__ATOMIC_ACQUIRE, "workgroup");
    Packet pk; packet_clear(pk);
    v3 att[kPacketShadows] = { mk3(1.f, 1.f, 1.f), mk3(1.f, 1.f, 1.f), mk3(1.f, 1.f, 1.f) };
    int axp = -1;
    if (have) {
      const SlotCold* cs = at32(cold, slot);
      const int fl = W.stack[slot][0];
      const bool hitValid = (fl & kHitValid) != 0;
      const int nSh = (fl >> kPendShift) & 3;
      const bool hadAux = (fl & kHasAux) != 0;
      const i4 ctl = slot_load(&cs->ctl);
#ifdef PT_EVLOG
      if (ctl.y >= 100) sEvOn = 1;
#endif
      const v4 thrIn = slot_load(&cs->thr), radIn = slot_load(&cs->rad);
      v4 wh = mk4(0.f, 0.f, 0.f, 0.f), wb = mk4(1.f, 1.f, 1.f, 1.f);
      v4 wp[kPacketShadows], wa[kPacketShadows];
      if (ctl.w & kCtlHoldsAux) axp = f2i(thrIn.w);
      PT_ROWS(0, 3);
      if (hitValid) { wh = slot_load(&cs->hit); PT_ROWS(0, 1); }
      if (fl & kHasScale) { wb = slot_load(&cs->bsc); PT_ROWS(0, 1); }
#pragma unroll
      for (int i = 0; i < kPacketShadows; i++) {
        wp[i] = mk4(0.f, 0.f, 0.f, 0.f); wa[i] = mk4(1.f, 1.f, 1.f, 0.f);
        if (i < nSh) {
          wp[i] = slot_load(&cs->pend[i]); PT_ROWS(0, 1);
          const int ax = (axp >> (kSlotBits * i)) & kSlotMask;
          const int stt = hadAux ? fl_stat(W.stack[ax][0], 0) : fl_stat(fl, i);
          if (stt == 2) { wa[i] = hadAux ? slot_load(&at32(cold, ax)->att[0]) : slot_load(&cs->att[i]); PT_ROWS(0, 1); }
          else if (stt == 1) wa[i] = mk4(0.f, 0.f, 0.f, 0.f);
        }
      }
      const v4 na = W.nodeA[slot], wd = W.nodeB[slot];
      ps.mode = ctl.w & 7; ps.light = 0; ps.item = ctl.x; ps.depth = ctl.y; ps.seed = (uint32_t)ctl.z; ps.pixel = 0;
      pk.nShadow = (ctl.w >> 3) & 3; pk.hasBounce = (ctl.w >> 5) & 1; pk.hasScale = (ctl.w >> 6) & 1;
      pk.bscale = mk3(wb.x, wb.y, wb.z); pk.binv = wb.w;
#pragma unroll
      for (int i = 0; i < kPacketShadows; i++) { pk.pendW[i] = mk3(wp[i].x, wp[i].y, wp[i].z); pk.pendInv[i] = wp[i].w; att[i] = mk3(wa[i].x, wa[i].y, wa[i].z); }
      ps.thr = mk3(thrIn.x, thrIn.y, thrIn.z); ps.rad = mk3(radIn.x, radIn.y, radIn.z);
      ps.N = mk3(0.f, 0.f, 1.f); ps.mat = 0; ps.V = mk3(0.f, 0.f, 1.f);
      ps.pendW = mk3(0.f, 0.f, 0.f); ps.pendInv = 0.f; ps.accum = mk3(0, 0, 0); ps.cdlin = mk3(0.f, 0.f, 0.f);
      ps.o = mk3(na.x, na.y, na.z); ps.d = mk3(wd.x, wd.y, wd.z); ps.tmin = sc.epsT; ps.tmax = kRtDefaultMax;
      ps.kind = RK_RADIANCE;
      res.tbest = na.w; res.bestTri = -1; res.bestPrim = -1; res.beta = 0.f; res.gamma = 0.f; res.att = mk3(1.f, 1.f, 1.f);
      if (hitValid) { res.bestTri = f2i(wh.x); res.bestPrim = f2i(wh.y); res.beta = wh.z; res.gamma = wh.w; }
      if (ps.mode == M_TRACE) ps.mode = M_RESULT;
    }
    const SlotSink sink{ cold, slot >= 0 ? slot : 0, W.nodeA, W.nodeB, W.stack, &ps, sc.rootRef, axp };
    if (CNT) { __builtin_amdgcn_s_waitcnt(0); PT_SUB(tBLoad); }
#ifdef PT_EVLOG
    __builtin_amdgcn_s_waitcnt(0); PT_EV(2, 0);
#endif
    for (;;) {
      if (have && ps.mode == M_NEW_SAMPLE) {
        if (CNT) {
          const unsigned long long b = min((unsigned long long)(kCntTailBuckets - 1), (__builtin_amdgcn_s_memrealtime() - rtStart) / 100000ull);
          atomicAdd(a.counters + kCntTailCount + b, 1ull); atomicMax(a.counters + kCntTailMaxDepth + b, (unsigned long long)ps.depth); atomicAdd(a.counters + kCntTailDepthSum + b, (unsigned long long)ps.depth);
        }
        store_sample(a, ps.item, ps.accum);
        if (CNT) atomicAdd(a.counters + kCntPacketFinished, 1ull);
        if (a.tileCost != nullptr && ps.depth >= kDeepPath) atomicMax(a.tileCost + ((ps.item % a.nItems) >> a.unitShift), (unsigned int)ps.depth);
        ps.mode = M_NEW_PIXEL;
      }
      const bool resultFirst = __ballot(have && ps.mode == M_RESULT) != 0ull;
      const bool run = have && ps.mode != M_TRACE && ps.mode != M_DONE &&
                       !((shadeBatch || resultFirst) && ps.mode == M_NEW_PIXEL);
      if (__ballot(run) == 0ull) break;
      if (CNT) {
        if (__ballot(run && ps.mode == M_RESULT)) nIterResult++;
        if (__ballot(run && ps.mode == M_NEW_PIXEL)) nIterGen++;
      }
      if (run) {
        if (ps.mode == M_RESULT) {
          on_result_packet<CNT, FAST, SlotSink, (F == 0 && !N64) ? FEAT_SPLIT_HIT : F>(sc, ps, pk, res, att, ct, sink);
        } else {
          int k = atomicAdd(a.workCounter, 1);
          if constexpr (F == 0) {
            const HandoutConsts* hc = reinterpret_cast<const HandoutConsts*>(a.workCounter) - 1;
            WorkItem w;
            if (k >= a.nWork) { ps.mode = M_DONE; }
            else if (handout_lean(a, hc, k, w)) { ps.pixel = w.pixel; ps.item = w.item; begin_sample_xy<CNT>(sc, ps, w.x, w.y, a.seeds[w.sample], ct); packet_primary(pk); }
          } else {
          k = (k >= a.nWork) ? -1 : handout_to_item(a, k);
          if (CNT && k < 0) atomicMin(a.counters + kCntItemsRanOut, (unsigned long long)__builtin_amdgcn_s_memrealtime());
          int s;
          if (k < 0) { ps.mode = M_DONE; }
          else if (item_to_pixel(a, k, s, ps.pixel)) { ps.item = k; begin_sample<CNT>(sc, ps, a.seeds[s], ct); packet_primary(pk); }
          }
        }
      }
    }
    if (CNT) { __builtin_amdgcn_s_waitcnt(0); PT_SUB(tBRun); }
#ifdef PT_EVLOG
    __builtin_amdgcn_s_waitcnt(0); PT_EV(3, 0);
#endif
    bool useAux = false;
    if (have) {
      SlotCold* cw = at32(cold, slot);
      if (axp >= 0 && !(ps.mode == M_TRACE && ps.depth >= a.auxDepth)) {
        for (int j = 0; j < kPacketShadows; j++) { const int ax = (axp >> (kSlotBits * j)) & kSlotMask; atomicOr(&W.freeMask[ax >> 5], 1u << (ax & 31)); }
        atomicAdd(&W.nFree, kPacketShadows);
        axp = -1;
      }
      int axpNext = axp;
      if (auxOn) {
        const bool wantAux = axp < 0 && ps.mode == M_TRACE && ps.depth >= a.auxDepth;
        if (wantAux && W.nFree >= kPacketShadows) {
          int got = 0, pack = 0;
          for (int wi = 0; wi < NS / 32 && got < kPacketShadows; wi++) {
            unsigned int cur = W.freeMask[wi];
            while (cur != 0u && got < kPacketShadows) {
              const int b = __builtin_ctz(cur);
              const unsigned int prev = atomicAnd(&W.freeMask[wi], ~(1u << b));
              if (prev & (1u << b)) { pack |= (wi * 32 + b) << (kSlotBits * got); got++; }
              cur = prev & ~(1u << b);
            }
          }
          if (got == kPacketShadows) { axpNext = pack; atomicSub(&W.nFree, kPacketShadows); }
          else for (int j = 0; j < got; j++) { const int ax = (pack >> (kSlotBits * j)) & kSlotMask; atomicOr(&W.freeMask[ax >> 5], 1u << (ax & 31)); }
        }
      }
      i4 ctl; ctl.x = ps.item; ctl.y = ps.depth; ctl.z = (int)ps.seed;
      ctl.w = ps.mode | (pk.nShadow << 3) | (pk.hasBounce << 5) | (pk.hasScale << 6);
      if (axpNext >= 0) ctl.w |= kCtlHoldsAux;
      slot_store(&cw->ctl, ctl);
      slot_store(&cw->thr, mk4(ps.thr.x, ps.thr.y, ps.thr.z, i2f(axpNext)));
      slot_store(&cw->rad, mk4(ps.rad.x, ps.rad.y, ps.rad.z, 0.f));
      PT_ROWS(1, 3);
      if (ps.mode == M_TRACE) {
        float tb0 = kRtDefaultMax; int bp0 = -1;
        if (pk.hasBounce) {
          Trav tv;
          ps.kind = RK_RADIANCE;
          trav_begin<CNT, false, F>(sc, ps, tv, ct);
          tb0 = tv.tbest; bp0 = tv.bestPrim;
        }
        const bool hitNow = bp0 >= 0;
        if (hitNow) { slot_store(&cw->hit, mk4(i2f(-1), i2f(bp0), 0.f, 0.f)); PT_ROWS(1, 1); }
        PT_ROWS(1, pk.nShadow + ((axp >= 0 || pk.nShadow == 0) ? 0 : pk.nShadow - 1));
        useAux = axp >= 0 && pk.nShadow > 0;
        const int nOwnSh = useAux ? 0 : pk.nShadow;
        const int nRays = nOwnSh + pk.hasBounce;
        const v4 rb = mk4(ps.d.x, ps.d.y, ps.d.z, tb0);
        if (nOwnSh == 0) {
          W.nodeA[slot] = mk4(ps.o.x, ps.o.y, ps.o.z, rb.w);
          W.nodeB[slot] = mk4(rb.x, rb.y, rb.z, i2f(sc.rootRef));
        } else if (pk.hasBounce) {
          if (pk.nShadow == 1) slot_store(&cw->ray[0], rb);
          else if (pk.nShadow == 2) slot_store(&cw->ray[1], rb);
          else slot_store(&cw->ray[2], rb);
          PT_ROWS(1, 1);
        }
        if (pk.hasScale) { slot_store(&cw->bsc, mk4(pk.bscale.x, pk.bscale.y, pk.bscale.z, pk.binv)); PT_ROWS(1, 1); }
        W.stack[slot][0] = (nOwnSh << kNShShift) | ((max(nRays, 1) - 1) << kNRayShift) | (nOwnSh > 0 ? kShadowRay : 0) | (pk.nShadow << kPendShift) |
                           (hitNow ? kHitValid : 0) | (pk.hasScale ? kHasScale : 0) |
                           (useAux ? kHasAux : 0);
        pendDest = sc.rootRef >= 0 ? Q_NODE : Q_LEAF;
        if (useAux) {
          W.stack[slot][0] |= (pk.nShadow << kJoinShift) | (pk.hasBounce ? 0 : kArrived);
          if (!pk.hasBounce) pendDest = DEST_NONE;
        }
      } else {
        W.stack[slot][0] = 0;
        pendDest = (ps.mode == M_NEW_PIXEL) ? Q_GEN : DEST_DONE;
        if (auxOn && ps.mode != M_NEW_PIXEL) {
          atomicOr(&W.freeMask[slot >> 5], 1u << (slot & 31)); atomicAdd(&W.nFree, 1);
        }
      }
    }
    if (auxOn && __ballot(useAux) != 0ull) {
      for (int j = 0; j < kPacketShadows; j++) local_push((useAux && j < pk.nShadow) ? Q_NODE : DEST_NONE, (axp >> (kSlotBits * j)) & kSlotMask);
    }
    if constexpr (!SHARED) __builtin_amdgcn_fence(__ATOMIC_RELEASE, "workgroup");
    PT_SUB(tBStore);
    PT_EV(4, __popcll(__ballot(useAux)));
  };

  unsigned int guard = 0;
  const unsigned long long wdStart = __builtin_amdgcn_s_memrealtime();
  for (;;) {
    if ((++guard & 4095u) == 0u && __builtin_amdgcn_s_memrealtime() - wdStart > a.watchdogTicks) { if (lane == 0) atomicOr(a.workCounter + 1, 1); break; }
    PT_SUB0(); if (CNT) nIter++;
    if (__ballot(pendDest != DEST_NONE) != 0ull) { local_push(pendDest, pendSlot); pendDest = DEST_NONE; }
    {
      const bool leave = ns >= 0 && !(ntv.node >= 0 && ntv.node != kTravDone);
      if (__ballot(leave) != 0ull) {
        int dest = DEST_NONE, pushSlot = ns;
        if (leave) {
          const int nodeOut = (ntv.node == kTravDone && fl_more(nsFlag)) ? kSwitchRef : ntv.node;
          W.nodeB[ns].w = i2f(nodeOut); store_flags(ns, ntv.sp | nsFlag);
          dest = (nodeOut == kTravDone) ? ((nsFlag & kShadeFlag) ? Q_SHADE : Q_GEN) : Q_LEAF;
          if (__builtin_expect(nodeOut == kTravDone && (nsFlag & (kHasAux | kAuxSlot)) != 0, 0)) {
            if (nsFlag & kAuxSlot) {
              __builtin_amdgcn_fence(__ATOMIC_RELEASE, "workgroup");
              pushSlot = aux_done(nsFlag, dest);
            } else if (arrive_parks(ns)) dest = DEST_NONE;
          }
        }
        local_push(dest, pushSlot);
        if (leave) ns = -1;
      }
      if (nqCount > 0 && __ballot(ns < 0) != 0ull) {
        const unsigned long long m = __ballot(ns < 0);
        const int n = min((int)__popcll(m), nqCount);
        if (ns < 0) {
          const int r = lane_rank(m);
          if (r < n) {
            ns = myNodeQ[ring_wrap<NS>(nqHead + r)];
            const v4 na = W.nodeA[ns], nb = W.nodeB[ns];
            const int spw = W.stack[ns][0];
            nray.o = mk3(na.x, na.y, na.z); ntv.tbest = na.w;
            ntv.inv = mk3(node_inv(nb.x), node_inv(nb.y), node_inv(nb.z)); ntv.node = f2i(nb.w);
            ntv.noi = neg_o_inv(nray.o, ntv.inv);
            ntv.sp = spw & kSpMask; nsFlag = spw & ~kSpMask;
          }
        }
        nqHead = ring_wrap<NS>(nqHead + n); nqCount -= n;
      }
    }
    const int nActive = __popcll(__ballot(ns >= 0));
    const bool starving = nActive <= 64 - a.starveLanes;
    int pass = -1;
    int mySlot = -1;
    auto leaf_pop = [&]() -> int {
      const int n = min(64, lqCount);
      const int slot = lane < n ? (int)myLeafQ[(lqHead + lane) & 255] : -1;
      lqHead = (lqHead + n) & 255; lqCount -= n;
      return slot;
    };
    const bool flush = obCount[0] >= 32 || obCount[1] >= 32;
    if (!flush && (lqCount >= 64 || (starving && lqCount >= 32))) {
      pass = 0; mySlot = leaf_pop();
      PT_SUB(tLocal);
    } else if (starving || flush) {
      PT_SUB(tLocal);
      PT_EV(9, nActive);
      txn_begin();
      for (int d = 0; d < 2; d++) {
        const int q = Q_SHADE + d;
        for (int base = 0; base < obCount[d]; base += 64) {
          const int i = base + lane;
          if (i < obCount[d]) W.queue[q][ring_wrap<NS>(qHead[q] + qCount[q] + i)] = sPriv[wave].outbox[d][i];
        }
        qCount[q] += obCount[d]; obCount[d] = 0;
      }
      nDone += localDone; localDone = 0;
      if (qCount[Q_SHADE] >= 64) pass = 1;
      else if (qCount[Q_GEN] >= 64) pass = 2;
      else if (lqCount >= 64) pass = 0;
      else if (starving) {
        const int l = lqCount;
        int sh = qCount[Q_SHADE], g = qCount[Q_GEN];
        if (nDone >= W.drainAt) { if (nDone + sh + g == NS && nActive == 0 && l == 0) pass = 4; sh = 0; g = 0; }
        if (pass != 4) {
          if (l + sh + g == 0) { if (nActive == 0) pass = (nDone == NS) ? 4 : 3; }
          else pass = (l >= sh && l >= g) ? 0 : (sh >= g ? 1 : 2);
        }
      }
      if (pass == 1 || pass == 2) mySlot = q_pop(pass == 1 ? Q_SHADE : Q_GEN, true);
      txn_end();
      if (pass == 0) mySlot = leaf_pop();
      PT_EV(10, pass + 1);
      PT_SUB(tTxn);
    } else PT_SUB(tLocal);
    PT_STAMP(tSwap);
    if (pass == 4) break;
    if (pass == 3) { if (CNT) idleSpins++; __builtin_amdgcn_s_sleep(32); PT_SUB(tIdle); PT_STAMP(tSwap); continue; }
    if (pass == 0) { leaf_pass(mySlot); PT_STAMP(tLeaf); continue; }
    if (pass > 0) { run_batch(mySlot, pass == 1); PT_STAMP(tBatch); continue; }

    if (CNT) { nodeRuns++; ringBacklog += (unsigned long long)nqCount; leafBacklog += (unsigned long long)lqCount; }
    {
      SlotStack st = make_stack(ns >= 0 ? ns : 0);
      PT_EV(5, nActive);
#ifdef PT_EVLOG
      int evSteps = 0;
#endif
      for (;;) {
#ifdef PT_EVLOG
        evSteps++;
#endif
        const bool atNode = ns >= 0 && ntv.node >= 0 && ntv.node != kTravDone;
        const unsigned long long m = __ballot(atNode);
        const int n = __popcll(m);
        if (n == 0 || nActive - n >= a.swapLanes) break;
        if (CNT) { nodeSteps++; nodeLanes += (uint32_t)n; }
        if (atNode) trav_node_step<CNT, N64>(sc, nray, ntv, st, ct);
      }
#ifdef PT_EVLOG
      PT_EV(6, evSteps - 1);
#endif
    }
    PT_STAMP(tNode);
  }

  if constexpr (SHARED) {
    __syncthreads();
    const LaunchArgs& a = fresh_args();
    SlotCold* cold = reinterpret_cast<SlotCold*>(a.poolCold) + (size_t)blockIdx.x * NS;
    const int gpool = blockIdx.x;
    PoolLds<NS>& W = sPool[0];
    if (W.done != NS && __hip_atomic_load(a.workCounter + 1, __ATOMIC_RELAXED, __HIP_MEMORY_SCOPE_AGENT) == 0) {
      __builtin_amdgcn_fence(__ATOMIC_ACQUIRE, "workgroup");
      const int nSh = W.qCount[Q_SHADE], nGe = W.qCount[Q_GEN];
      for (int e = threadIdx.x; e < nSh + nGe; e += kBlockThreads) {
        const int q = e < nSh ? Q_SHADE : Q_GEN, r = e < nSh ? e : e - nSh;
        const int slot = W.queue[q][ring_wrap<NS>(W.qHead[q] + r)];
        SlotCold* cw = at32(cold, slot);
        int fl = W.stack[slot][0];
        const i4 ctl = slot_load(&cw->ctl);
        if ((ctl.w & 7) != M_TRACE) continue;
        if (fl & kHasAux) {
          const int axp = f2i(slot_load(&cw->thr).w);
          const int nS = (fl >> kPendShift) & 3;
#pragma unroll
          for (int i = 0; i < kPacketShadows; i++) {
            if (i < nS) {
              const int ax = (axp >> (kSlotBits * i)) & kSlotMask;
              const int stt = fl_stat(W.stack[ax][0], 0);
              fl = (fl & ~(3 << (kStatShift + 2 * i))) | (stt << (kStatShift + 2 * i));
              if (stt == 2) slot_store(&cw->att[i], slot_load(&at32(cold, ax)->att[0]));
            }
          }
          fl &= ~(kHasAux | kJoinMask);
        }
        const v4 na = W.nodeA[slot], nb = W.nodeB[slot];
        slot_store(&cw->spare[0], na);
        slot_store(&cw->spare[1], mk4(nb.x, nb.y, nb.z, i2f(fl)));
        const bool deep = ctl.y >= kDrainDeep;
        int* dl = a.workCounter + kDrainList;
        const int idx = atomicAdd(dl + (deep ? kDrainDeepN : kDrainOtherN), 1);
        dl[deep ? kDrainEntries + idx : kDrainEntries + dl[kDrainCap] - 1 - idx] = gpool * NS + slot;
        if (CNT) atomicAdd(a.counters + kCntHandedOver, 1ull);
      }
    }
  }

  if constexpr (CNT) {
    unsigned long long* c = a.counters;
    uint32_t v[kCntPerLane];
    wave_sum_counters(ct, v);
    const uint32_t rw[4] = { wave_sum(rows[0]), wave_sum(rows[1]), wave_sum(rows[2]), wave_sum(rows[3]) };
    for (int i = 0; i < kCensusRegions; i++) {
      const uint32_t cl = wave_sum(ct.censusLanes[i]), cw = wave_sum(ct.censusWaves[i]);
      if (lane == 0 && cw != 0u) { atomicAdd(&c[kCntCensusLanes + i], (unsigned long long)cl); atomicAdd(&c[kCntCensusWaves + i], (unsigned long long)cw); }
    }
    if (lane == 0) {
      for (int i = 0; i < kCntPerLane; i++) atomicAdd(&c[i], (unsigned long long)v[i]);
      atomicAdd(&c[kCntTraversalSteps], (unsigned long long)nodeSteps + leafPasses);
      atomicAdd(&c[kCntActiveLaneSteps], (unsigned long long)nodeLanes + leafLanes);
      atomicAdd(&c[kCntShadeBatches], (unsigned long long)batches);
      atomicAdd(&c[kCntShadeBatchLanes], (unsigned long long)batchLanes);
      atomicAdd(&c[kCntIdleSpins], (unsigned long long)idleSpins);
      atomicAdd(&c[kCntTBatch], tBatch); atomicAdd(&c[kCntTSwap], tSwap); atomicAdd(&c[kCntTNode], tNode); atomicAdd(&c[kCntTLeaf], tLeaf);
      atomicAdd(&c[kCntTWave], __builtin_amdgcn_s_memtime() - tStart);
      atomicAdd(&c[kCntLeafPasses], (unsigned long long)leafPasses); atomicAdd(&c[kCntLeafLanes], (unsigned long long)leafLanes);
      atomicMax(&c[kCntLastWaveOut], (unsigned long long)__builtin_amdgcn_s_memrealtime());
      atomicMin(&c[kCntFirstWaveIn], rtStart);
      atomicAdd(&c[kCntTLocal], tLocal); atomicAdd(&c[kCntTLock], tLock); atomicAdd(&c[kCntTTxn], tTxn); atomicAdd(&c[kCntTIdle], tIdle);
      atomicAdd(&c[kCntNodeRuns], nodeRuns); atomicAdd(&c[kCntRingBacklog], ringBacklog); atomicAdd(&c[kCntLeafBacklog], leafBacklog);
      atomicAdd(&c[kCntIterResult], nIterResult); atomicAdd(&c[kCntIterLights], nIterLights); atomicAdd(&c[kCntIterNewItem], nIterGen);
      atomicAdd(&c[kCntSlotRows], (unsigned long long)rw[0]); atomicAdd(&c[kCntSlotRows + 1], (unsigned long long)rw[1]);
      atomicAdd(&c[kCntSlotRows + 2], (unsigned long long)rw[2]); atomicAdd(&c[kCntSlotRows + 3], (unsigned long long)rw[3]);
      atomicAdd(&c[kCntTBatchLoad], tBLoad); atomicAdd(&c[kCntTBatchRun], tBRun); atomicAdd(&c[kCntTBatchStore], tBStore); atomicAdd(&c[kCntTransactions], nTxn); atomicAdd(&c[kCntIterations], nIter);
    }
  }
```

minimaloptix_amd/csrc/pt_path.h:

```cpp
#pragma once
#include "pt_types.h"
#include "pt_rng.h"
#include "pt_geom.h"
#include "pt_disney.h"
#include "pt_texture.h"

namespace pt {

enum { M_NEW_PIXEL = 0, M_NEW_SAMPLE = 1, M_TRACE = 2, M_RESULT = 3, M_LIGHTS = 4, M_DONE = 5 };
enum { RK_RADIANCE = 0, RK_SHADOW = 1 };

struct Counters {
  uint32_t samples, primaryRays, bounceRays, shadowRays;
  uint32_t nodeFetches, triTests, closestHits, lightLoads, analyticTests;
  uint32_t censusLanes[kCensusRegions], censusWaves[kCensusRegions];
};
template <bool CNT> PT_HD void cnt(uint32_t& c, uint32_t n = 1) { if (CNT) c += n; }
enum { CR_RESULT = 0, CR_MISS, CR_HIT, CR_LIGHT, CR_DEPTHCAP, CR_LAMBERT, CR_METAL, CR_GLASS, CR_DISNEY_GLASS, CR_DISNEY, CR_LIGHT0, CR_LIGHT1,
       CR_LIGHT2, CR_BOUNCE_EVAL, CR_GEN, CR_TRI0, CR_TRI1, CR_TRI2, CR_TRI3, CR_TRI_HIT, CR_SHADOW_FOLD, CR_LIGHT_DRAW, CR_BOUNCE_SAMPLE, CR_NODE_BRANCHED };
template <bool CNT> PT_HD void census(Counters& ct, int region) {
#if defined(__HIP_DEVICE_COMPILE__)
  if constexpr (CNT) {
    const unsigned long long m = __ballot(1);
    ct.censusLanes[region]++;
    if (__builtin_amdgcn_mbcnt_hi((unsigned)(m >> 32), __builtin_amdgcn_mbcnt_lo((unsigned)m, 0u)) == 0) ct.censusWaves[region]++;
  }
#endif
}

struct Trav {
  int node;
  int sp;
  int started;
  float tbest;
  int bestPrim;
  int bestTri;
  int bestCls;
  float beta, gamma;
  v3 att;
  v3 inv;
  v3 noi;
};

struct PathState {
  int mode;
  int pixel;
  int item;
  v3 accum;
  v3 thr, rad;
  int depth; uint32_t seed;
  v3 o, d; float tmin, tmax; int kind;
  v3 N, V; int mat; int light;
  v3 pendW; float pendInv;
  v3 cdlin;
};


PT_HD bool shadow_any_hit(const SceneView& sc, int mat, v3& att) {
  const DevMaterial m = load_const(at32(sc.mats, mat));
  if (m.kind != MAT_DISNEY) return false;
  if (m.brdfType == BRDF_GLASS) { att = att * m.color; return false; }
  att = mk3(0.f, 0.f, 0.f);
  return true;
}
PT_HD void shadow_candidate(const SceneView& sc, int mat, float t, int prim, float tmin, float& tbest, int& bestPrim, v3& att) {
  if (!potential(t, prim, tmin, tbest, bestPrim)) return;
  const DevMaterial m = load_const(at32(sc.mats, mat));
  if (m.kind != MAT_DISNEY) return;
  tbest = t; bestPrim = prim;
  att = (m.brdfType == BRDF_GLASS) ? m.color : mk3(0.f, 0.f, 0.f);
}

PT_HD bool shadow_any_hit_tri(const SceneView& sc, int cls, int mat, v3& att) {
  if (cls == SHADOW_NONE) return false;
  if (cls == SHADOW_GLASS) { att = att * load_const(&at32(sc.mats, mat)->color); return false; }
  att = mk3(0.f, 0.f, 0.f);
  return true;
}
PT_HD void shadow_candidate_tri(const SceneView& sc, int cls, int mat, float t, int prim, float tmin, float& tbest, int& bestPrim, v3& att) {
  if (cls == SHADOW_NONE || !potential(t, prim, tmin, tbest, bestPrim)) return;
  tbest = t; bestPrim = prim;
  att = (cls == SHADOW_GLASS) ? load_const(&at32(sc.mats, mat)->color) : mk3(0.f, 0.f, 0.f);
}

constexpr float kSlabMinDir = 1e-19f;
PT_HD float slab_inv(float d) { return 1.0f / (__builtin_fabsf(d) < kSlabMinDir ? __builtin_copysignf(kSlabMinDir, d) : d); }
PT_HD v3 neg_o_inv(v3 o, v3 inv) { return mk3(-(o.x * inv.x), -(o.y * inv.y), -(o.z * inv.z)); }

template <bool CNT, bool WINDOW = true, int F = FEAT_ALL>
PT_HD void trav_begin(const SceneView& sc, const PathState& ps, Trav& tv, Counters& ct) {
  tv.tbest = ps.tmax; tv.bestPrim = -1; tv.bestTri = -1; tv.beta = 0.f; tv.gamma = 0.f;
  tv.att = mk3(1.f, 1.f, 1.f);
  tv.inv = mk3(slab_inv(ps.d.x), slab_inv(ps.d.y), slab_inv(ps.d.z));
  tv.noi = neg_o_inv(ps.o, tv.inv);
  tv.sp = 0; tv.started = 1;
  bool terminated = false;
  if (ps.kind == RK_RADIANCE) {
    int i0 = 0;
#ifndef PT_SPHERE_CHUNK
#define PT_SPHERE_CHUNK 4
#endif
#if defined(__HIP_DEVICE_COMPILE__)
    for (; has<F>(FEAT_SPHERES) && i0 + PT_SPHERE_CHUNK <= sc.nSpheres; i0 += PT_SPHERE_CHUNK) {
      float bq[PT_SPHERE_CHUNK], dq[PT_SPHERE_CHUNK];
#pragma unroll
      for (int k = 0; k < PT_SPHERE_CHUNK; k++) {
        const DevSphere s = load_uniform(sc.spheres + i0 + k);
        const v3 oc = ps.o - s.center;
        bq[k] = dot(ps.d, oc);
        const float c = dot(oc, oc) - s.radius * s.radius;
        dq[k] = bq[k] * bq[k] - c;
      }
#pragma unroll
      for (int k = 0; k < PT_SPHERE_CHUNK; k++) {
        bool look = !(dq[k] < 0);
        if constexpr (WINDOW) {
          const float sa = __builtin_amdgcn_sqrtf(fmaxf_(dq[k], 0.f));
          const float margin = 1e-4f * (1.f + __builtin_fabsf(bq[k]) + sa);
          look = look && (sa - bq[k]) > ps.tmin - margin && (-bq[k] - sa) < tv.tbest + margin;
        }
        if (look) {
          const float sq = __builtin_sqrtf(dq[k]);
          const float t1 = -bq[k] - sq, t2 = -bq[k] + sq;
          if (potential(t1, i0 + k, ps.tmin, tv.tbest, tv.bestPrim)) { tv.tbest = t1; tv.bestPrim = i0 + k; }
          else if (potential(t2, i0 + k, ps.tmin, tv.tbest, tv.bestPrim)) { tv.tbest = t2; tv.bestPrim = i0 + k; }
        }
      }
    }
#endif
    for (int i = i0; has<F>(FEAT_SPHERES) && i < sc.nSpheres; i++) {
      const DevSphere s = sc.spheres[i];
      float t1, t2;
      if (sphere_roots(s.center, s.radius, ps.o, ps.d, t1, t2)) {
        if (potential(t1, i, ps.tmin, tv.tbest, tv.bestPrim)) { tv.tbest = t1; tv.bestPrim = i; }
        else if (potential(t2, i, ps.tmin, tv.tbest, tv.bestPrim)) { tv.tbest = t2; tv.bestPrim = i; }
      }
    }
    for (int i = 0; i < sc.nQuads; i++) {
      const DevQuad q = load_uniform(sc.quads + i);
      float t; const int id = sc.nSpheres + i;
      if (quad_test(q.plane, q.v1, q.v2, q.anchor, ps.o, ps.d, ps.tmin, ps.tmax, t) &&
          potential(t, id, ps.tmin, tv.tbest, tv.bestPrim)) { tv.tbest = t; tv.bestPrim = id; }
    }
    cnt<CNT>(ct.analyticTests, (uint32_t)(sc.nSpheres + sc.nQuads));
  } else if (sc.anyDisneyAnalytic) {
    for (int i = 0; has<F>(FEAT_SPHERES) && i < sc.nSpheres && !terminated; i++) {
      const int mat = load_uniform(sc.sphereMat + i);
      if (sc.mats[mat].kind != MAT_DISNEY) continue;
      const DevSphere s = load_uniform(sc.spheres + i);
      float t1, t2;
      if (!sphere_roots(s.center, s.radius, ps.o, ps.d, t1, t2)) continue;
      if (sc.shadowNearest) {
        shadow_candidate(sc, mat, t1, i, ps.tmin, tv.tbest, tv.bestPrim, tv.att);
        shadow_candidate(sc, mat, t2, i, ps.tmin, tv.tbest, tv.bestPrim, tv.att);
      } else if ((t1 > ps.tmin && t1 < ps.tmax) || (t2 > ps.tmin && t2 < ps.tmax))
        terminated = shadow_any_hit(sc, mat, tv.att);
    }
    for (int i = 0; i < sc.nQuads && !terminated; i++) {
      const DevQuad q = load_uniform(sc.quads + i);
      if (sc.mats[q.mat].kind != MAT_DISNEY) continue;
      float t;
      if (quad_test(q.plane, q.v1, q.v2, q.anchor, ps.o, ps.d, ps.tmin, ps.tmax, t)) {
        if (sc.shadowNearest) shadow_candidate(sc, q.mat, t, sc.nSpheres + i, ps.tmin, tv.tbest, tv.bestPrim, tv.att);
        else terminated = shadow_any_hit(sc, q.mat, tv.att);
      }
    }
    cnt<CNT>(ct.analyticTests, (uint32_t)(sc.nSpheres + sc.nQuads));
  }
  tv.node = (terminated || sc.rootRef == kEmptyRef) ? kTravDone : sc.rootRef;
}

PT_HD bool slab(v3 lo, v3 hi, v3 o, v3 inv, float tmin, float tmax, float& tn) {
  float t0x = (lo.x - o.x) * inv.x, t1x = (hi.x - o.x) * inv.x;
  float t0y = (lo.y - o.y) * inv.y, t1y = (hi.y - o.y) * inv.y;
  float t0z = (lo.z - o.z) * inv.z, t1z = (hi.z - o.z) * inv.z;
  tn = fmaxf_(fmaxf_(fminf_(t0x, t1x), fminf_(t0y, t1y)), fmaxf_(fminf_(t0z, t1z), tmin));
  float tf = fminf_(fminf_(fmaxf_(t0x, t1x), fmaxf_(t0y, t1y)), fminf_(fmaxf_(t0z, t1z), tmax));
  return tn <= tf * 1.0000005f;
}

template <class Stack>
PT_HD void trav_pop(Trav& tv, Stack& st) {
  if (tv.sp == 0) tv.node = kTravDone;
  else { tv.sp--; tv.node = st.load(tv.sp); }
}

struct ChildKey {
#if defined(__HIP_DEVICE_COMPILE__)
  double v;
  PT_HD static ChildKey make(float t, int ref) {
    ChildKey k; k.v = __builtin_bit_cast(double, ((unsigned long long)(uint32_t)f2i(t) << 32) | (uint32_t)ref); return k;
  }
  PT_HD float t() const { return i2f((int32_t)(__builtin_bit_cast(unsigned long long, v) >> 32)); }
  PT_HD int ref() const { return (int32_t)(uint32_t)__builtin_bit_cast(unsigned long long, v); }
  PT_HD static void order(ChildKey& a, ChildKey& b) {
    double lo, hi;
    asm("v_min_f64 %0, %1, %2" : "=v"(lo) : "v"(a.v), "v"(b.v));
    asm("v_max_f64 %0, %1, %2" : "=v"(hi) : "v"(a.v), "v"(b.v));
    a.v = lo; b.v = hi;
  }
#else
  unsigned long long v;
  PT_HD static ChildKey make(float t, int ref) { ChildKey k; k.v = ((unsigned long long)(uint32_t)f2i(t) << 32) | (uint32_t)ref; return k; }
  PT_HD float t() const { return i2f((int32_t)(v >> 32)); }
  PT_HD int ref() const { return (int32_t)(uint32_t)v; }
  PT_HD static void order(ChildKey& a, ChildKey& b) { if (b.v < a.v) { const unsigned long long x = a.v; a.v = b.v; b.v = x; } }
#endif
};
#ifndef PT_STACK_ROOMY
#define PT_STACK_ROOMY 1
#endif
template <bool CNT, class Stack>
PT_HD void node_step_nearfar(const PathState& ps, Trav& tv, Stack& st, Counters& ct, const float nx[4], const float fx[4], const float ny[4],
                             const float fy[4], const float nz[4], const float fz[4], int r0, int r1, int r2, int r3, int top) {
  const int r[4] = { r0, r1, r2, r3 };
  cnt<CNT>(ct.nodeFetches);
  const float kFar = 3.0e38f;
  ChildKey k[4];
#if defined(__HIP_DEVICE_COMPILE__)
#pragma unroll
#endif
  for (int c = 0; c < 4; c++) {
    const float tn = fmaxf_(fmaxf_(nx[c], ny[c]), fmaxf_(nz[c], ps.tmin));
    const float tf = fminf_(fminf_(fx[c], fy[c]), fminf_(fz[c], tv.tbest));
    const bool in = (c < 2) ? (tn <= tf * 1.0000005f) : (tn <= tf * 1.0000005f && r[c] != kEmptyRef);
    k[c] = ChildKey::make(in ? tn : kFar, r[c]);
  }
  ChildKey::order(k[0], k[1]); ChildKey::order(k[2], k[3]); ChildKey::order(k[0], k[2]);
  ChildKey::order(k[1], k[3]); ChildKey::order(k[1], k[2]);
  if constexpr (Stack::kFlat) {
    const bool h0 = k[0].t() < kFar, h1 = k[1].t() < kFar, h2 = k[2].t() < kFar, h3 = k[3].t() < kFar;
    const int m = (int)h1 + (int)h2 + (int)h3;
    if (__builtin_expect(st.fits_fast(tv.sp, m), 1)) {
      const int r1 = k[1].ref(), r2 = k[2].ref(), r3 = k[3].ref();
      const int p1 = tv.sp + (int)h2, p2 = p1 + (int)h3;
      st.store_fast(tv.sp, h3 ? r3 : (h2 ? r2 : r1)); st.store_fast(p1, h3 ? r2 : r1); st.store_fast(p2, r1);
      tv.node = h0 ? k[0].ref() : (tv.sp > 0 ? top : kTravDone);
      tv.sp = h0 ? p2 + (int)h1 : (tv.sp > 0 ? tv.sp - 1 : 0);
      return;
    }
    census<CNT>(ct, CR_NODE_BRANCHED);
  }
  if (k[0].t() < kFar) {
    if (PT_STACK_ROOMY && st.roomy(tv.sp)) {
      if (k[3].t() < kFar) { st.store_fast(tv.sp, k[3].ref()); tv.sp++; }
      if (k[2].t() < kFar) { st.store_fast(tv.sp, k[2].ref()); tv.sp++; }
      if (k[1].t() < kFar) { st.store_fast(tv.sp, k[1].ref()); tv.sp++; }
    } else {
      if (k[3].t() < kFar) { st.store(tv.sp, k[3].ref()); tv.sp++; }
      if (k[2].t() < kFar) { st.store(tv.sp, k[2].ref()); tv.sp++; }
      if (k[1].t() < kFar) { st.store(tv.sp, k[1].ref()); tv.sp++; }
    }
    tv.node = k[0].ref();
  } else {
    trav_pop(tv, st);
  }
}
PT_HD void planes4(const v4& p, float inv, float noi, float out[4]) {
  out[0] = fma_(p.x, inv, noi); out[1] = fma_(p.y, inv, noi); out[2] = fma_(p.z, inv, noi); out[3] = fma_(p.w, inv, noi);
}
PT_HD void planes4q(uint32_t w, float step, float base, float out[4]) {
  out[0] = fma_((float)(w & 0xffu), step, base); out[1] = fma_((float)((w >> 8) & 0xffu), step, base);
  out[2] = fma_((float)((w >> 16) & 0xffu), step, base); out[3] = fma_((float)(w >> 24), step, base);
}
template <bool CNT, class Stack>
PT_HD void trav_node_step64(const Node64& n, const PathState& ps, Trav& tv, Stack& st, Counters& ct, int top) {
  float nx[4], fx[4], ny[4], fy[4], nz[4], fz[4];
  const float sx = n.sx * tv.inv.x, sy = n.sy * tv.inv.y, sz = n.sz * tv.inv.z;
  const float cx = fma_(n.ox, tv.inv.x, tv.noi.x), cy = fma_(n.oy, tv.inv.y, tv.noi.y), cz = fma_(n.oz, tv.inv.z, tv.noi.z);
  const bool bx = tv.inv.x < 0.f, by = tv.inv.y < 0.f, bz = tv.inv.z < 0.f;
  planes4q(bx ? n.q[3] : n.q[0], sx, cx, nx); planes4q(bx ? n.q[0] : n.q[3], sx, cx, fx);
  planes4q(by ? n.q[4] : n.q[1], sy, cy, ny); planes4q(by ? n.q[1] : n.q[4], sy, cy, fy);
  planes4q(bz ? n.q[5] : n.q[2], sz, cz, nz); planes4q(bz ? n.q[2] : n.q[5], sz, cz, fz);
  node_step_nearfar<CNT>(ps, tv, st, ct, nx, fx, ny, fy, nz, fz, n.ref[0], n.ref[1], n.ref[2], n.ref[3], top);
}
template <bool CNT, bool N64 = false, class Stack>
PT_HD void trav_node_step(const SceneView& sc, const PathState& ps, Trav& tv, Stack& st, Counters& ct) {
  float nx[4], fx[4], ny[4], fy[4], nz[4], fz[4];
  int top = kTravDone;
  if constexpr (Stack::kFlat) top = st.peek_fast(tv.sp);
  if constexpr (N64) {
    const Node64 n = load_const(at32(sc.nodes64, tv.node));
    trav_node_step64<CNT>(n, ps, tv, st, ct, top);
  } else {
#if defined(__HIP_DEVICE_COMPILE__)
    const char* nb = reinterpret_cast<const char*>(sc.nodes);
    const uint32_t no = (uint32_t)tv.node * (uint32_t)sizeof(Node128);
    const uint32_t sx = (uint32_t)(f2i(tv.inv.x) >> 31) & 48u, sy = (uint32_t)(f2i(tv.inv.y) >> 31) & 48u, sz = (uint32_t)(f2i(tv.inv.z) >> 31) & 48u;
    const v4 pnx = load_const(reinterpret_cast<const v4*>(nb + (no + sx)));
    const v4 pfx = load_const(reinterpret_cast<const v4*>(nb + (no + (48u - sx))));
    const v4 pny = load_const(reinterpret_cast<const v4*>(nb + (no + (16u + sy))));
    const v4 pfy = load_const(reinterpret_cast<const v4*>(nb + (no + (64u - sy))));
    const v4 pnz = load_const(reinterpret_cast<const v4*>(nb + (no + (32u + sz))));
    const v4 pfz = load_const(reinterpret_cast<const v4*>(nb + (no + (80u - sz))));
    const i4r rf = load_const(reinterpret_cast<const i4r*>(nb + (no + 96u)));
    planes4(pnx, tv.inv.x, tv.noi.x, nx); planes4(pfx, tv.inv.x, tv.noi.x, fx);
    planes4(pny, tv.inv.y, tv.noi.y, ny); planes4(pfy, tv.inv.y, tv.noi.y, fy);
    planes4(pnz, tv.inv.z, tv.noi.z, nz); planes4(pfz, tv.inv.z, tv.noi.z, fz);
    node_step_nearfar<CNT>(ps, tv, st, ct, nx, fx, ny, fy, nz, fz, rf.x, rf.y, rf.z, rf.w, top);
    return;
#endif
    const Node128 n = load_const(at32(sc.nodes, tv.node));
    float a[4], b[4];
    planes4(n.lox, tv.inv.x, tv.noi.x, a); planes4(n.hix, tv.inv.x, tv.noi.x, b);
    for (int c = 0; c < 4; c++) { nx[c] = fminf_(a[c], b[c]); fx[c] = fmaxf_(a[c], b[c]); }
    planes4(n.loy, tv.inv.y, tv.noi.y, a); planes4(n.hiy, tv.inv.y, tv.noi.y, b);
    for (int c = 0; c < 4; c++) { ny[c] = fminf_(a[c], b[c]); fy[c] = fmaxf_(a[c], b[c]); }
    planes4(n.loz, tv.inv.z, tv.noi.z, a); planes4(n.hiz, tv.inv.z, tv.noi.z, b);
    for (int c = 0; c < 4; c++) { nz[c] = fminf_(a[c], b[c]); fz[c] = fmaxf_(a[c], b[c]); }
    node_step_nearfar<CNT>(ps, tv, st, ct, nx, fx, ny, fy, nz, fz, n.ref[0], n.ref[1], n.ref[2], n.ref[3], top);
  }
}

struct LeafChunk { v3 p0[4], e0[4], e1[4]; int mat[4], prim[4], shadow[4]; };
PT_HD void leaf_fetch4(const SceneView& sc, int leafRef, int base, LeafChunk& ch) {
  const int first = leaf_first(leafRef), count = leaf_count(leafRef);
#if defined(__HIP_DEVICE_COMPILE__)
#pragma unroll
#endif
  for (int j = 0; j < 4; j++) {
    const int k = base + j < count ? base + j : count - 1;
    const Tri48 tpv = load_const(at32(sc.tris, first + k));
    const Tri48* tp = &tpv;
    ch.p0[j] = tp->p0; ch.e0[j] = tp->e0; ch.e1[j] = tp->e1; ch.mat[j] = tp->mat; ch.prim[j] = tp->prim; ch.shadow[j] = tp->shadow;
  }
}
template <bool CNT, class Stack>
PT_HD void trav_leaf_step_fetched(const SceneView& sc, const PathState& ps, Trav& tv, Stack& st, Counters& ct, LeafChunk& ch) {
  {
    const int first = leaf_first(tv.node), count = leaf_count(tv.node);
    const int triBase = sc.nSpheres + sc.nQuads;
    bool terminated = false;
    const float tmaxTest = (ps.kind == RK_SHADOW && sc.shadowNearest) ? kRtDefaultMax : ps.tmax;
    for (int base = 0; base < count && !terminated; base += 4) {
      if (base > 0) leaf_fetch4(sc, tv.node, base, ch);
#pragma unroll
      for (int j = 0; j < 4; j++) {
        if (base + j < count && !terminated) {
          cnt<CNT>(ct.triTests); census<CNT>(ct, CR_TRI0 + j);
          v3 n; float t, be, ga;
          if (tri_test(ps.o, ps.d, ps.tmin, tmaxTest, ch.p0[j], ch.e0[j], ch.e1[j], n, t, be, ga)) {
            census<CNT>(ct, CR_TRI_HIT);
            if (ps.kind == RK_RADIANCE) {
              if (potential(t, triBase + ch.prim[j], ps.tmin, tv.tbest, tv.bestPrim)) {
                tv.tbest = t; tv.bestPrim = triBase + ch.prim[j]; tv.bestTri = first + base + j; tv.beta = be; tv.gamma = ga; tv.bestCls = ch.shadow[j];
              }
            } else if (sc.shadowNearest) {
              shadow_candidate_tri(sc, ch.shadow[j], ch.mat[j], t, triBase + ch.prim[j], ps.tmin, tv.tbest, tv.bestPrim, tv.att);
            } else if (shadow_any_hit_tri(sc, ch.shadow[j], ch.mat[j], tv.att)) terminated = true;
          }
        }
      }
    }
    if (terminated) tv.node = kTravDone;
    else trav_pop(tv, st);
  }
}
template <bool CNT, class Stack>
PT_HD void trav_leaf_step(const SceneView& sc, const PathState& ps, Trav& tv, Stack& st, Counters& ct) {
  LeafChunk ch;
  leaf_fetch4(sc, tv.node, 0, ch);
  trav_leaf_step_fetched<CNT>(sc, ps, tv, st, ct, ch);
}

template <bool CNT, bool N64 = false, class Stack>
PT_HD void trav_step(const SceneView& sc, const PathState& ps, Trav& tv, Stack& st, Counters& ct) {
  if (tv.node >= 0) trav_node_step<CNT, N64>(sc, ps, tv, st, ct);
  else trav_leaf_step<CNT>(sc, ps, tv, st, ct);
}


template <bool CNT>
PT_HD void begin_sample_xy(const SceneView& sc, PathState& ps, int x, int y, int launchSeed, Counters& ct) {
  ps.depth = 1;
  ps.seed = tea16((uint32_t)y * (uint32_t)sc.width + (uint32_t)x, (uint32_t)launchSeed);
  ps.thr = mk3(1.f, 1.f, 1.f); ps.rad = mk3(0.f, 0.f, 0.f);
  const v3 randInLens = rand_in_unit_disk(ps.seed) * sc.cam.lensRadius;
  const v3 offs = sc.cam.u * randInLens.x + sc.cam.v * randInLens.y;
  const float r1 = rnd(ps.seed); const float r2 = rnd(ps.seed);
  const float xyx = ((float)x + r1 - 0.5f) / (float)sc.width;
  const float xyy = ((float)y + r2 - 0.5f) / (float)sc.height;
  ps.o = sc.cam.origin + offs;
  ps.d = normalize((((sc.cam.scrLowerLeftCorner + sc.cam.horizontal * xyx) + sc.cam.vertical * xyy) - sc.cam.origin) - offs);
  ps.tmin = sc.epsT; ps.tmax = kRtDefaultMax; ps.kind = RK_RADIANCE;
  ps.mode = M_TRACE;
  cnt<CNT>(ct.samples); cnt<CNT>(ct.primaryRays); census<CNT>(ct, CR_GEN);
}
template <bool CNT>
PT_HD void begin_sample(const SceneView& sc, PathState& ps, int launchSeed, Counters& ct) {
  const int x = ps.pixel % sc.width, y = ps.pixel / sc.width;
  begin_sample_xy<CNT>(sc, ps, x, y, launchSeed, ct);
}

PT_HD void end_sample(PathState& ps) {
  ps.accum = mk3(clampf(ps.rad.x, 0.f, 1.f), clampf(ps.rad.y, 0.f, 1.f), clampf(ps.rad.z, 0.f, 1.f));
  ps.mode = M_NEW_SAMPLE;
}

PT_HD void bounce(const SceneView& sc, PathState& ps, v3 o, v3 d, uint32_t childSeed) {
  ps.o = o; ps.d = d; ps.tmin = sc.epsT; ps.tmax = kRtDefaultMax; ps.kind = RK_RADIANCE;
  ps.depth++; ps.seed = childSeed;
  ps.mode = M_TRACE;
}

template <bool CNT>
PT_HD void glass_body(const SceneView& sc, PathState& ps, float ior, v3 tint, const HitAttr& h, Counters& ct) {
  v3 normal = h.shadingNormal;
  float cosThetaI = -dot(ps.d, normal);
  float refIdx;
  if (cosThetaI > 0.f) { refIdx = ior; }
  else { refIdx = 1.f / ior; cosThetaI = -cosThetaI; normal = -normal; }
  v3 refracted;
  const bool totalReflection = !refract(refracted, ps.d, normal, refIdx);
  const float cosThetaT = -dot(normal, refracted);
  const float reflectProb = totalReflection ? 1.f : fresnel(cosThetaI, cosThetaT, refIdx);
  const uint32_t childSeed = fork_seed(ps.seed, ps.depth + 1);
  v3 no, nd;
  if (rnd(ps.seed) < reflectProb) { no = h.front; nd = reflect(ps.d, normal); }
  else { no = h.back; nd = refracted; }
  ps.thr = ps.thr * tint;
  cnt<CNT>(ct.bounceRays);
  bounce(sc, ps, no, nd, childSeed);
}

PT_HD void hit_attributes_face(const SceneView& sc, const PathState& ps, const Trav& tv, HitAttr& h) {
  const TriFace fv = load_const(tri_face(sc, tv.bestTri));
  h.mat = fv.matNrm & 0x7fffffff;
  h.texu = 0.f; h.texv = 0.f;
  h.geoNormal = fv.gn;
  if (fv.matNrm < 0) {
    const v3 n0 = mk3(fv.n0x, fv.n0y, fv.n0z), n1 = mk3(fv.n1x, fv.n1y, fv.n1z), n2 = mk3(fv.n2x, fv.n2y, fv.n2z);
    h.shadingNormal = normalize((n1 * tv.beta + n2 * tv.gamma) + n0 * (1.f - tv.beta - tv.gamma));
  } else {
    h.shadingNormal = h.geoNormal;
  }
  refine_hitpoint(ray_at(ps.o, ps.d, tv.tbest), ps.d, h.geoNormal, fv.p0, h.back, h.front);
}

template <int F = FEAT_ALL>
PT_HD void hit_attributes(const SceneView& sc, const PathState& ps, const Trav& tv, HitAttr& h) {
  const float t = tv.tbest;
  if constexpr (F == 0) { if (tv.bestPrim >= sc.nSpheres + sc.nQuads) { hit_attributes_face(sc, ps, tv, h); return; } }
  if (has<F>(FEAT_SPHERES) && tv.bestPrim < sc.nSpheres) {
    const DevSphere s = sc.spheres[tv.bestPrim];
    const v3 p = ray_at(ps.o, ps.d, t);
    h.geoNormal = normalize(p - s.center);
    h.shadingNormal = h.geoNormal;
    h.texu = 0.f; h.texv = 0.f;
    h.front = p; h.back = p;
    h.mat = sc.sphereMat[tv.bestPrim];
  } else if (tv.bestPrim < sc.nSpheres + sc.nQuads) {
    const DevQuad* q = sc.quads + (tv.bestPrim - sc.nSpheres);
    const v3 n = xyz(q->plane);
    h.geoNormal = n; h.shadingNormal = n;
    h.texu = 0.f; h.texv = 0.f;
    h.front = ray_at(ps.o, ps.d, t); h.back = h.front;
    h.mat = q->mat;
  } else {
    const Tri48 tpv = load_const(at32(sc.tris, tv.bestTri));
    const TriShade spv = load_const(at32(sc.triShade, tv.bestTri));
    const Tri48* tp = &tpv;
    const TriShade* sp = &spv;
    const v3 p0 = tp->p0, e0 = tp->e0, e1 = tp->e1;
    const v3 sn0 = sp->n0, sn1 = sp->n1, sn2 = sp->n2;
    const int hasNormals = sp->hasNormals;
    h.mat = tp->mat;
    h.texu = 0.f; h.texv = 0.f;
    if (has<F>(FEAT_TEXTURE) && sc.triUV != nullptr && at32(sc.mats, h.mat)->albedoTex != 0) {
      const TriUV* up = sc.triUV + tp->prim;
      if (up->hasUV) {
        const float w0 = 1.f - tv.beta - tv.gamma;
        h.texu = (up->u1 * tv.beta + up->u2 * tv.gamma) + up->u0 * w0;
        h.texv = (up->v1 * tv.beta + up->v2 * tv.gamma) + up->v0 * w0;
      }
    }
    h.geoNormal = normalize(cross(e1, e0));
    if (hasNormals) {
      const v3 n0 = sn0, n1 = sn1, n2 = sn2;
      h.shadingNormal = normalize((n1 * tv.beta + n2 * tv.gamma) + n0 * (1.f - tv.beta - tv.gamma));
    } else {
      h.shadingNormal = h.geoNormal;
    }
    refine_hitpoint(ray_at(ps.o, ps.d, t), ps.d, h.geoNormal, p0, h.back, h.front);
  }
}

template <bool CNT, int F = FEAT_ALL>
PT_HD void on_result(const SceneView& sc, PathState& ps, const Trav& tv, Counters& ct) {
  if (ps.kind == RK_SHADOW) {
    if (ps.pendInv != 0.f && length_is_nonzero(tv.att)) {
      const v3 c = (ps.pendW * tv.att) * ps.pendInv;
      ps.rad = ps.rad + ps.thr * c;
    }
    ps.light++;
    ps.mode = M_LIGHTS;
    return;
  }
  if (tv.bestPrim < 0) {
    census<CNT>(ct, CR_MISS);
    ps.rad = ps.rad + ps.thr * sc.bg;
    end_sample(ps);
    return;
  }
  cnt<CNT>(ct.closestHits); census<CNT>(ct, CR_HIT);
  HitAttr h;
  hit_attributes<F>(sc, ps, tv, h);
  const DevMaterial m = load_const(at32(sc.mats, h.mat));
  if (m.kind == MAT_LIGHT) {
    census<CNT>(ct, CR_LIGHT);
    ps.rad = ps.rad + ps.thr * m.emission;
    end_sample(ps);
    return;
  }
  if (ps.depth > sc.maxDepth) { census<CNT>(ct, CR_DEPTHCAP); end_sample(ps); return; }

  if (has<F>(FEAT_PLAIN_MATERIALS) && m.kind == MAT_LAMBERTIAN) {
    census<CNT>(ct, CR_LAMBERT);
    const v3 no = ray_at(ps.o, ps.d, tv.tbest);
    const v3 nd = normalize(h.geoNormal + rand_in_unit_sphere(ps.seed));
    const uint32_t childSeed = fork_seed(ps.seed, ps.depth + 1);
    ps.thr = ps.thr * m.albedo;
    cnt<CNT>(ct.bounceRays);
    bounce(sc, ps, no, nd, childSeed);
  } else if (has<F>(FEAT_PLAIN_MATERIALS) && m.kind == MAT_METAL) {
    census<CNT>(ct, CR_METAL);
    const v3 no = ray_at(ps.o, ps.d, tv.tbest);
    const v3 nd = normalize(reflect(ps.d, h.geoNormal) + rand_in_unit_sphere(ps.seed) * m.fuzz);
    const uint32_t childSeed = fork_seed(ps.seed, ps.depth + 1);
    ps.thr = ps.thr * m.albedo;
    cnt<CNT>(ct.bounceRays);
    bounce(sc, ps, no, nd, childSeed);
  } else if (has<F>(FEAT_PLAIN_MATERIALS) && m.kind == MAT_GLASS) {
    census<CNT>(ct, CR_GLASS);
    glass_body<CNT>(sc, ps, m.refIdx, m.albedo, h, ct);
  } else {
    v3 baseColor = m.color;
    if (has<F>(FEAT_TEXTURE) && m.albedoTex != 0) {
      baseColor = xyz(tex2d(sc.textures[m.albedoTex - 1], h.texu, h.texv));
      ps.cdlin = srgb2lin(baseColor);
    }
    if (m.brdfType == BRDF_GLASS) { census<CNT>(ct, CR_DISNEY_GLASS); glass_body<CNT>(sc, ps, 1.45f, baseColor, h, ct); return; }
    census<CNT>(ct, CR_DISNEY);
    ps.N = faceforward(h.shadingNormal, -ps.d, h.geoNormal);
    ps.V = -ps.d;
    ps.mat = h.mat;
    ps.o = h.front;
    ps.rad = ps.rad + ps.thr * m.emission;
    ps.light = 0;
    ps.mode = M_LIGHTS;
  }
}

template <bool CNT, bool FAST = false>
PT_HD void on_lights(const SceneView& sc, PathState& ps, Counters& ct) {
  const DevMaterial m = load_const(at32(sc.mats, ps.mat));
  int choice = 0;
  v3 L = mk3(0.f, 0.f, 1.f), H = mk3(0.f, 0.f, 1.f), emission = mk3(0.f, 0.f, 0.f);
  float lightDst = 0.f, lightPdf = 0.f;
  while (ps.light < sc.nLights) {
    const DevLight ltv = load_const(sc.lights + ps.light);
    const DevLight* lt = &ltv;
    cnt<CNT>(ct.lightLoads);
    v3 pointOnLight, normalOnLight;
    if (lt->shape == LIGHT_SPHERE) {
      pointOnLight = lt->position + rand_in_unit_sphere(ps.seed) * lt->radius;
      normalOnLight = normalize(pointOnLight - lt->position);
    } else {
      const float r1 = rnd(ps.seed); const float r2 = rnd(ps.seed);
      pointOnLight = (lt->position + lt->u * r1) + lt->v * r2;
      normalOnLight = lt->normal;
    }
    L = pointOnLight - ps.o;
    lightDst = length(L);
    L = normalize(L);
    if (dot(L, ps.N) > 0.f && dot(L, normalOnLight) < 0.f) {
      H = normalize(L + ps.V);
      lightPdf = lightDst * lightDst / lt->area / dot(normalOnLight, -L);
      emission = lt->emission;
      choice = 1;
      break;
    }
    ps.light++;
  }
  const Onb onb = make_onb(ps.N);
  if (choice == 0) {
    disney_sample(ps.seed, m, onb, ps.V, L, H);
    if (dot(ps.N, L) > 0.0f && dot(ps.N, ps.V) > 0.0f) choice = 2;
  }
  if (choice == 0) { end_sample(ps); return; }

  v3 Cdlin = m.Cdlin, Cspec0 = m.Cspec0, Csheen = m.Csheen;
  if (m.albedoTex != 0) {
    Cdlin = ps.cdlin;
    disney_color_constants(Cdlin, m.specular, m.specularTint, m.sheenTint, m.metallic, Cspec0, Csheen);
  }
  const float pdf = disney_pdf<FAST>(m, ps.N, L, H);
  const v3 brdf = disney_eval<FAST>(m, Cdlin, Cspec0, Csheen, onb, L, ps.V, H);

  if (choice == 1) {
    if (lightPdf > 0 && pdf > 0) {
      ps.pendW = (brdf * powerHeuristic(lightPdf, pdf)) * emission;
      ps.pendInv = 1.0f / fmaxf_(0.001f, lightPdf);
    } else {
      ps.pendW = mk3(0.f, 0.f, 0.f); ps.pendInv = 0.f;
    }
    ps.d = L; ps.tmin = sc.epsT; ps.tmax = lightDst - sc.epsT; ps.kind = RK_SHADOW;
    ps.mode = M_TRACE;
    cnt<CNT>(ct.shadowRays);
    return;
  }
  const uint32_t childSeed = fork_seed(ps.seed, ps.depth + 1);
  if (pdf > 0) {
    ps.thr = (ps.thr * brdf) * (1.0f / pdf);
    cnt<CNT>(ct.bounceRays);
    bounce(sc, ps, ps.o, L, childSeed);
    return;
  }
  end_sample(ps);
}

}
```

minimaloptix_amd/csrc/queuekernel.hip:

```cpp
#include <hip/hip_runtime.h>

#include "megakernel.h"
#include "pt_lanestack.h"
#include "pt_path.h"

namespace pt {

namespace {

constexpr int kBlockThreads = 256;
constexpr int kWaves = kBlockThreads / 64;
#ifndef PT_KP
#define PT_KP 128
#endif
#ifndef PT_STACKN
#define PT_STACKN 11
#endif
#ifndef PT_WAVES_PER_SIMD
#define PT_WAVES_PER_SIMD 3
#endif
constexpr int kP = PT_KP;
constexpr int kStackN = PT_STACKN;
constexpr int kWavesPerSimd = PT_WAVES_PER_SIMD;
constexpr int ring_capacity(int n) { int c = 1; while (c < n) c <<= 1; return c; }

enum { Q_SHADE = 0, Q_GEN = 1, kNumQ = 2, Q_NODE = 2, Q_LEAF = 3, DEST_DONE = 4, DEST_NONE = -1 };

struct alignas(16) i4 { int x, y, z, w; };
struct alignas(16) SlotCold {
  i4 ctl;
  v4 thr;
  v4 rad;
  v4 spare;
  v4 hit;
  v4 nrm;
  v4 view;
  v4 pend;
};
static_assert(sizeof(SlotCold) == 128, "SlotCold layout");

#ifndef PT_SLOT_NT
#define PT_SLOT_NT 0
#endif
typedef float f4v __attribute__((ext_vector_type(4)));
template <class T> __device__ __forceinline__ T slot_load(const T* p) {
  static_assert(sizeof(T) % 16 == 0, "16-byte granules");
  if constexpr (PT_SLOT_NT) {
    T out;
    const f4v* src = reinterpret_cast<const f4v*>(p); f4v* dst = reinterpret_cast<f4v*>(&out);
#pragma unroll
    for (unsigned i = 0; i < sizeof(T) / 16; i++) dst[i] = __builtin_nontemporal_load(src + i);
    return out;
  } else {
    return *p;
  }
}
template <class T> __device__ __forceinline__ void slot_store(T* p, const T& v) {
  static_assert(sizeof(T) % 16 == 0, "16-byte granules");
  if constexpr (PT_SLOT_NT) {
    const f4v* src = reinterpret_cast<const f4v*>(&v); f4v* dst = reinterpret_cast<f4v*>(p);
#pragma unroll
    for (unsigned i = 0; i < sizeof(T) / 16; i++) __builtin_nontemporal_store(src[i], dst + i);
  } else {
    *p = v;
  }
}

template <int NS>
struct PoolLds {
  v4 nodeA[NS];
  v4 nodeB[NS];
  int stack[NS][kStackN + 1];
  unsigned short queue[kNumQ][ring_capacity(NS)];
  int qHead[kNumQ], qCount[kNumQ];
  int done, lock;
};

template <int NS>
struct WavePriv {
  unsigned short qnode[ring_capacity(NS)];
  unsigned short qleaf[256];
  unsigned short outbox[2][160];
};

typedef __attribute__((address_space(3))) int lds_int;

constexpr int kShadeFlag = 1 << 30;
constexpr int kShadowRay = 1 << 29;
constexpr int kHitValid = 1 << 28;
constexpr int kSlotFlags = kShadeFlag | kShadowRay | kHitValid;

struct SlotStack {
  lds_int* lds;
  int* ovf;
  __device__ __forceinline__ void store(int sp, int v) {
    if (__builtin_expect(sp < kStackN, 1)) lds[sp] = v; else ovf[sp - kStackN] = v;
  }
  __device__ __forceinline__ int load(int sp) const {
    int v;
    if (__builtin_expect(sp < kStackN, 1)) v = lds[sp]; else v = ovf[sp - kStackN];
    return v;
  }
  __device__ __forceinline__ bool roomy(int sp) const { return sp + 3 <= kStackN; }
  __device__ __forceinline__ void store_fast(int sp, int v) { lds[sp] = v; }
  static constexpr bool kFlat = false;
  __device__ __forceinline__ bool fits_fast(int, int) const { return false; }
  __device__ __forceinline__ int peek_fast(int) const { return 0; }
};

__device__ __forceinline__ int route(int node, int kind, int bestPrim) {
  if (node == kTravDone) return (kind == RK_SHADOW || bestPrim >= 0) ? Q_SHADE : Q_GEN;
  return node >= 0 ? Q_NODE : Q_LEAF;
}

__device__ __forceinline__ const LaunchArgs& fresh_args() {
  typedef __attribute__((address_space(4))) const LaunchArgs CA;
  unsigned long long p = (unsigned long long)__builtin_amdgcn_kernarg_segment_ptr();
  asm volatile("" : "+s"(p));
  return *(const LaunchArgs*)(CA*)p;
}

template <bool CNT, bool SHARED, bool FAST = false, bool NEAR = false>
__global__ void __launch_bounds__(kBlockThreads, kWavesPerSimd) pt_queuekernel(const LaunchArgs a) {
  constexpr int NS = SHARED ? kP * kWaves : kP;
  constexpr int RC = ring_capacity(NS);
  __shared__ PoolLds<NS> sPool[SHARED ? 1 : kWaves];
  __shared__ WavePriv<NS> sPriv[kWaves];

  SceneView scv = a.scene;
  scv.shadowNearest = NEAR ? 1 : 0;
  const SceneView& sc = scv;
  const int lane = threadIdx.x & 63, wave = threadIdx.x >> 6;
  PoolLds<NS>& W = sPool[SHARED ? 0 : wave];
  const int gpool = SHARED ? blockIdx.x : blockIdx.x * kWaves + wave;
  SlotCold* cold = reinterpret_cast<SlotCold*>(a.poolCold) + (size_t)gpool * NS;
  int* ovfBase = a.stackOverflow ? a.stackOverflow + (size_t)gpool * NS * a.ovfDepth : nullptr;

  unsigned long long tLocal = 0, tLock = 0, tTxn = 0, tIdle = 0, tBLoad = 0, tBRun = 0, tBStore = 0, nTxn = 0, nIter = 0;
  unsigned long long tSub = 0, nIterResult = 0, nIterLights = 0, nIterGen = 0, nodeRuns = 0, ringBacklog = 0, leafBacklog = 0;
#define PT_SUB0() do { if (CNT) tSub = __builtin_amdgcn_s_memtime(); } while (0)
#define PT_SUB(acc) do { if (CNT) { const unsigned long long now_ = __builtin_amdgcn_s_memtime(); acc += now_ - tSub; tSub = now_; } } while (0)
  int qHead[kNumQ] = { 0, 0 }, qCount[kNumQ] = { 0, 0 };
  int nDone = 0;

  [[maybe_unused]] auto q_push = [&](int q, bool pred, int slot) {
    const unsigned long long m = __ballot(pred);
    if (m == 0ull) return;
    if (pred) W.queue[q][(qHead[q] + qCount[q] + lane_rank(m)) & (RC - 1)] = (unsigned short)slot;
    qCount[q] += __popcll(m);
  };
  auto q_pop = [&](int q, bool want) -> int {
    const unsigned long long m = __ballot(want);
    const int n = min((int)__popcll(m), qCount[q]);
    int slot = -1;
    if (want) { const int r = lane_rank(m); if (r < n) slot = W.queue[q][(qHead[q] + r) & (RC - 1)]; }
    qHead[q] = (qHead[q] + n) & (RC - 1);
    qCount[q] -= n;
    return slot;
  };
  auto txn_begin = [&]() {
    if constexpr (SHARED) {
      if (lane == 0) { while (atomicCAS(&W.lock, 0, 1) != 0) __builtin_amdgcn_s_sleep(1); }
      __builtin_amdgcn_fence(__ATOMIC_ACQUIRE, "workgroup");
      if (CNT) { (void)__builtin_amdgcn_readfirstlane(W.lock); PT_SUB(tLock); nTxn++; }
      for (int q = 0; q < kNumQ; q++) {
        qHead[q] = __builtin_amdgcn_readfirstlane(W.qHead[q]);
        qCount[q] = __builtin_amdgcn_readfirstlane(W.qCount[q]);
      }
      nDone = __builtin_amdgcn_readfirstlane(W.done);
    }
  };
  auto txn_end = [&]() {
    if constexpr (SHARED) {
      if (lane == 0) {
        for (int q = 0; q < kNumQ; q++) { W.qHead[q] = qHead[q]; W.qCount[q] = qCount[q]; }
        W.done = nDone;
      }
      __builtin_amdgcn_fence(__ATOMIC_RELEASE, "workgroup");
      if (lane == 0) __hip_atomic_store(&W.lock, 0, __ATOMIC_RELAXED, __HIP_MEMORY_SCOPE_WORKGROUP);
    }
  };
  auto make_stack = [&](int slot) {
    SlotStack st;
    st.lds = (lds_int*)&W.stack[slot][1];
    st.ovf = ovfBase ? ovfBase + (size_t)slot * a.ovfDepth : nullptr;
    return st;
  };

  const int nUse = (a.slotsInUse > 0 && a.slotsInUse < NS) ? (SHARED ? a.slotsInUse : max(64, a.slotsInUse / kWaves)) : NS;
  {
    const int first = SHARED ? threadIdx.x : lane, step = SHARED ? kBlockThreads : 64;
    for (int s = first; s < nUse; s += step) {
      i4 ctl; ctl.x = -1; ctl.y = 0; ctl.z = 0; ctl.w = M_NEW_PIXEL;
      cold[s].ctl = ctl;
      W.stack[s][0] = 0;
      W.queue[Q_GEN][s] = (unsigned short)s;
    }
    if constexpr (SHARED) {
      if (threadIdx.x == 0) {
        for (int q = 0; q < kNumQ; q++) { W.qHead[q] = 0; W.qCount[q] = 0; }
        W.qCount[Q_GEN] = nUse; W.done = NS - nUse; W.lock = 0;
      }
      __builtin_amdgcn_fence(__ATOMIC_RELEASE, "workgroup");
      __syncthreads();
    } else {
      qCount[Q_GEN] = nUse; nDone = NS - nUse;
      __builtin_amdgcn_fence(__ATOMIC_RELEASE, "workgroup");
    }
  }

  Counters ct = {};
  uint32_t nodeSteps = 0, nodeLanes = 0, leafPasses = 0, leafLanes = 0, batches = 0, batchLanes = 0, idleSpins = 0;
  unsigned long long tBatch = 0, tSwap = 0, tNode = 0, tLeaf = 0, tStamp = 0;
  const unsigned long long tStart = CNT ? __builtin_amdgcn_s_memtime() : 0ull;
  [[maybe_unused]] const unsigned long long rtStart = CNT ? __builtin_amdgcn_s_memrealtime() : 0ull;
#define PT_STAMP(acc) do { if (CNT) { const unsigned long long now_ = __builtin_amdgcn_s_memtime(); acc += now_ - tStamp; tStamp = now_; } } while (0)
  tStamp = tStart;

  int ns = -1;
  int nsFlag = 0;
  PathState nray;
  nray.o = mk3(0, 0, 0); nray.tmin = sc.epsT; nray.d = mk3(0, 0, 1); nray.tmax = 0; nray.kind = RK_RADIANCE; nray.mode = M_TRACE;
  Trav ntv;
  ntv.node = kTravDone; ntv.sp = 0; ntv.tbest = 0; ntv.inv = mk3(0, 0, 0); ntv.noi = mk3(0, 0, 0); ntv.bestPrim = -1; ntv.bestTri = -1;
  ntv.beta = 0; ntv.gamma = 0; ntv.att = mk3(1, 1, 1); ntv.started = 1;

  int pendSlot = -1, pendDest = DEST_NONE;

  auto leaf_pass = [&](int slot) {
    const LaunchArgs& a = fresh_args();
    SceneView scl = a.scene; scl.shadowNearest = NEAR ? 1 : 0;
    const SceneView& sc = scl;
    const bool have = slot >= 0;
    if (CNT) { leafPasses++; leafLanes += (uint32_t)__popcll(__ballot(have)); }
    pendSlot = slot; pendDest = DEST_NONE;
    __builtin_amdgcn_fence(__ATOMIC_RELEASE, "workgroup");
    __builtin_amdgcn_fence(__ATOMIC_ACQUIRE, "workgroup");
    if (have) {
      PathState ps; Trav tv;
      ps.tmin = sc.epsT; ps.mode = M_TRACE;
      const v4 na = W.nodeA[slot], nb = W.nodeB[slot];
      const int fl = W.stack[slot][0];
      const bool shadow = (fl & kShadowRay) != 0, hitValid = (fl & kHitValid) != 0;
      LeafChunk ch;
      leaf_fetch4(sc, f2i(nb.w), 0, ch);
      const SlotCold* cs = cold + slot;
      v4 wh = mk4(0.f, 0.f, 0.f, 0.f);
      if (hitValid) wh = slot_load(&cs->hit);
      ps.o = mk3(na.x, na.y, na.z); ps.d = mk3(nb.x, nb.y, nb.z);
      ps.kind = shadow ? RK_SHADOW : RK_RADIANCE;
      ps.tmax = shadow ? na.w : kRtDefaultMax;
      tv.inv = mk3(0.f, 0.f, 0.f); tv.tbest = na.w;
      tv.node = f2i(nb.w); tv.sp = fl & ~kSlotFlags;
      tv.bestTri = -1; tv.bestPrim = -1; tv.beta = 0.f; tv.gamma = 0.f; tv.att = mk3(1.f, 1.f, 1.f);
      if (hitValid) {
        if (shadow) { tv.att = mk3(wh.x, wh.y, wh.z); if (sc.shadowNearest) tv.bestPrim = f2i(wh.w); }
        else { tv.bestTri = f2i(wh.x); tv.bestPrim = f2i(wh.y); tv.beta = wh.z; tv.gamma = wh.w; }
      }
      const int oldTri = tv.bestTri, oldPrim = tv.bestPrim;
      const v3 oldAtt = tv.att;
      SlotStack st = make_stack(slot);
      trav_leaf_step_fetched<CNT>(sc, ps, tv, st, ct, ch);
      const bool changed = shadow ? ((tv.att.x != oldAtt.x || tv.att.y != oldAtt.y || tv.att.z != oldAtt.z) || (sc.shadowNearest && tv.bestPrim != oldPrim))
                                  : (tv.bestTri != oldTri || tv.bestPrim != oldPrim);
      if (changed) {
        v4 o2;
        if (shadow) o2 = mk4(tv.att.x, tv.att.y, tv.att.z, i2f(tv.bestPrim));
        else o2 = mk4(i2f(tv.bestTri), i2f(tv.bestPrim), tv.beta, tv.gamma);
        slot_store(&cold[slot].hit, o2);
      }
      W.nodeA[slot].w = tv.tbest;
      W.nodeB[slot].w = i2f(tv.node);
      W.stack[slot][0] = tv.sp | (fl & kShadowRay) | ((hitValid || changed) ? kHitValid : 0) |
                         ((shadow || tv.bestPrim >= 0) ? kShadeFlag : 0);
      pendDest = route(tv.node, ps.kind, tv.bestPrim);
    }
    if constexpr (!SHARED) __builtin_amdgcn_fence(__ATOMIC_RELEASE, "workgroup");
  };

  auto run_batch = [&](int slot, bool shadeBatch) {
    const LaunchArgs& a = fresh_args();
    SceneView scl = a.scene; scl.shadowNearest = NEAR ? 1 : 0;
    const SceneView& sc = scl;
    const bool have = slot >= 0;
    if (CNT) { batches++; batchLanes += (uint32_t)__popcll(__ballot(have)); }
    PT_SUB0();
    pendSlot = slot; pendDest = DEST_NONE;
    PathState ps; Trav res;
    ps.mode = M_DONE; ps.kind = RK_RADIANCE;
    res.node = kTravDone; res.bestPrim = -1;
    __builtin_amdgcn_fence(__ATOMIC_RELEASE, "workgroup");
    __builtin_amdgcn_fence(__ATOMIC_ACQUIRE, "workgroup");
    bool shadowIn = false;
    int depthIn = 0, itemIn = 0;
    bool radDirty = false, texDirty = false;
    if (have) {
      const SlotCold* cs = cold + slot;
      const int fl = W.stack[slot][0];
      const bool shadow = (fl & kShadowRay) != 0, hitValid = (fl & kHitValid) != 0;
      const i4 ctl = slot_load(&cs->ctl);
      const v4 thrIn = slot_load(&cs->thr), radIn = slot_load(&cs->rad);
      depthIn = ctl.y; itemIn = ctl.x;
      v4 wh = mk4(0.f, 0.f, 0.f, 0.f);
      v4 wn = mk4(0.f, 0.f, 1.f, 0.f), wv = mk4(0.f, 0.f, 1.f, 0.f), wp = mk4(0.f, 0.f, 0.f, 0.f);
      if (hitValid) wh = slot_load(&cs->hit);
      if (shadow) { wn = slot_load(&cs->nrm); wv = slot_load(&cs->view); wp = slot_load(&cs->pend); }
      const v4 na = W.nodeA[slot], wd = W.nodeB[slot];
      ps.mode = ctl.w & 7; ps.light = ctl.w >> 3; ps.item = ctl.x; ps.depth = ctl.y; ps.seed = (uint32_t)ctl.z; ps.pixel = 0;
      ps.thr = mk3(thrIn.x, thrIn.y, thrIn.z); ps.rad = mk3(radIn.x, radIn.y, radIn.z);
      ps.N = mk3(wn.x, wn.y, wn.z); ps.mat = f2i(wn.w); ps.V = mk3(wv.x, wv.y, wv.z);
      ps.pendW = mk3(wp.x, wp.y, wp.z); ps.pendInv = wp.w; ps.accum = mk3(0, 0, 0);
      ps.cdlin = mk3(wv.w, thrIn.w, radIn.w);
      ps.o = mk3(na.x, na.y, na.z); ps.d = mk3(wd.x, wd.y, wd.z); ps.tmin = sc.epsT; ps.tmax = kRtDefaultMax;
      ps.kind = shadow ? RK_SHADOW : RK_RADIANCE;
      res.tbest = na.w; res.bestTri = -1; res.bestPrim = -1; res.beta = 0.f; res.gamma = 0.f; res.att = mk3(1.f, 1.f, 1.f);
      if (hitValid) {
        if (shadow) res.att = mk3(wh.x, wh.y, wh.z);
        else { res.bestTri = f2i(wh.x); res.bestPrim = f2i(wh.y); res.beta = wh.z; res.gamma = wh.w; }
      }
      if (ps.mode == M_TRACE) { ps.mode = M_RESULT; shadowIn = shadow; }
    }
    if (CNT) { __builtin_amdgcn_s_waitcnt(0); PT_SUB(tBLoad); }
    for (;;) {
      if (have && ps.mode == M_NEW_SAMPLE) {
        if (CNT) {
          const unsigned long long b = min((unsigned long long)(kCntTailBuckets - 1), (__builtin_amdgcn_s_memrealtime() - rtStart) / 100000ull);
          atomicAdd(a.counters + kCntTailCount + b, 1ull); atomicMax(a.counters + kCntTailMaxDepth + b, (unsigned long long)ps.depth); atomicAdd(a.counters + kCntTailDepthSum + b, (unsigned long long)ps.depth);
        }
        store_sample(a, ps.item, ps.accum);
        if (a.tileCost != nullptr && ps.depth >= kDeepPath) atomicMax(a.tileCost + ((ps.item % a.nItems) >> a.unitShift), (unsigned int)ps.depth);
        ps.mode = M_NEW_PIXEL;
      }
      const bool resultFirst = __ballot(have && ps.mode == M_RESULT) != 0ull;
      const bool run = have && ps.mode != M_TRACE && ps.mode != M_DONE &&
                       !((shadeBatch || resultFirst) && ps.mode == M_NEW_PIXEL);
      if (__ballot(run) == 0ull) break;
      if (CNT) {
        if (__ballot(run && ps.mode == M_RESULT)) nIterResult++;
        if (__ballot(run && ps.mode == M_LIGHTS)) nIterLights++;
        if (__ballot(run && ps.mode == M_NEW_PIXEL)) nIterGen++;
      }
      if (run) {
        if (ps.mode == M_RESULT) {
          const v3 r0 = ps.rad, c0 = ps.cdlin;
          on_result<CNT>(sc, ps, res, ct);
          radDirty = radDirty || f2i(r0.x) != f2i(ps.rad.x) || f2i(r0.y) != f2i(ps.rad.y) || f2i(r0.z) != f2i(ps.rad.z);
          texDirty = texDirty || f2i(c0.x) != f2i(ps.cdlin.x) || f2i(c0.y) != f2i(ps.cdlin.y) || f2i(c0.z) != f2i(ps.cdlin.z);
        } else if (ps.mode == M_LIGHTS) {
          on_lights<CNT, FAST>(sc, ps, ct);
        } else {
          int k = atomicAdd(a.workCounter, 1);
          k = (k >= a.nWork) ? -1 : handout_to_item(a, k);
          if (CNT && k < 0) atomicMin(a.counters + kCntItemsRanOut, (unsigned long long)__builtin_amdgcn_s_memrealtime());
          int s;
          if (k < 0) { ps.mode = M_DONE; }
          else if (item_to_pixel(a, k, s, ps.pixel)) { ps.item = k; begin_sample<CNT>(sc, ps, a.seeds[s], ct); }
        }
      }
    }
    if (CNT) { __builtin_amdgcn_s_waitcnt(0); PT_SUB(tBRun); }
    if (have) {
      SlotCold* cw = cold + slot;
      i4 ctl; ctl.x = ps.item; ctl.y = ps.depth; ctl.z = (int)ps.seed; ctl.w = ps.mode | (ps.light << 3);
      slot_store(&cw->ctl, ctl);
      const bool newPath = ps.item != itemIn || ps.depth != depthIn;
      if (newPath || texDirty) slot_store(&cw->thr, mk4(ps.thr.x, ps.thr.y, ps.thr.z, ps.cdlin.y));
      if (ps.item != itemIn || radDirty || texDirty) slot_store(&cw->rad, mk4(ps.rad.x, ps.rad.y, ps.rad.z, ps.cdlin.z));
      if (ps.mode == M_TRACE) {
        Trav tv;
        trav_begin<CNT>(sc, ps, tv, ct);
        v4 na, nb;
        na.x = ps.o.x; na.y = ps.o.y; na.z = ps.o.z; na.w = tv.tbest;
        nb.x = ps.d.x; nb.y = ps.d.y; nb.z = ps.d.z; nb.w = i2f(tv.node);
        W.nodeA[slot] = na; W.nodeB[slot] = nb;
        const bool shadow = ps.kind == RK_SHADOW;
        const bool hitNow = shadow ? ((tv.att.x != 1.f || tv.att.y != 1.f || tv.att.z != 1.f) || (sc.shadowNearest && tv.bestPrim >= 0)) : (tv.bestPrim >= 0);
        W.stack[slot][0] = ((shadow || tv.bestPrim >= 0) ? kShadeFlag : 0) | (shadow ? kShadowRay : 0) | (hitNow ? kHitValid : 0);
        if (hitNow) slot_store(&cw->hit, shadow ? mk4(tv.att.x, tv.att.y, tv.att.z, i2f(tv.bestPrim)) : mk4(i2f(tv.bestTri), i2f(tv.bestPrim), tv.beta, tv.gamma));
        if (shadow) {
          slot_store(&cw->pend, mk4(ps.pendW.x, ps.pendW.y, ps.pendW.z, ps.pendInv));
          if (!shadowIn) {
            slot_store(&cw->nrm, mk4(ps.N.x, ps.N.y, ps.N.z, i2f(ps.mat)));
            slot_store(&cw->view, mk4(ps.V.x, ps.V.y, ps.V.z, ps.cdlin.x));
          }
        }
        pendDest = route(tv.node, ps.kind, tv.bestPrim);
      } else {
        W.stack[slot][0] = 0;
        pendDest = (ps.mode == M_NEW_PIXEL) ? Q_GEN : DEST_DONE;
      }
    }
    if constexpr (!SHARED) __builtin_amdgcn_fence(__ATOMIC_RELEASE, "workgroup");
    PT_SUB(tBStore);
  };

  unsigned short* myNodeQ = sPriv[wave].qnode;
  int nqHead = 0, nqCount = 0;
  unsigned short* myLeafQ = sPriv[wave].qleaf;
  int lqHead = 0, lqCount = 0;
  int obCount[2] = { 0, 0 };
  int localDone = 0;
  auto local_push = [&](int dest, int slot) {
    {
      const unsigned long long m = __ballot(dest == Q_NODE);
      if (m != 0ull) {
        if (dest == Q_NODE) myNodeQ[(nqHead + nqCount + lane_rank(m)) & (RC - 1)] = (unsigned short)slot;
        nqCount += __popcll(m);
      }
    }
    {
      const unsigned long long m = __ballot(dest == Q_LEAF);
      if (m != 0ull) {
        if (dest == Q_LEAF) myLeafQ[(lqHead + lqCount + lane_rank(m)) & 255] = (unsigned short)slot;
        lqCount += __popcll(m);
      }
    }
    for (int d = 0; d < 2; d++) {
      const unsigned long long m = __ballot(dest == Q_SHADE + d);
      if (m != 0ull) {
        if (dest == Q_SHADE + d) sPriv[wave].outbox[d][obCount[d] + lane_rank(m)] = (unsigned short)slot;
        obCount[d] += __popcll(m);
      }
    }
    localDone += __popcll(__ballot(dest == DEST_DONE));
  };

  unsigned int guard = 0;
  const unsigned long long wdStart = __builtin_amdgcn_s_memrealtime();
  for (;;) {
    if ((++guard & 4095u) == 0u && __builtin_amdgcn_s_memrealtime() - wdStart > a.watchdogTicks) { if (lane == 0) atomicOr(a.workCounter + 1, 1); break; }
    PT_SUB0(); if (CNT) nIter++;
    if (__ballot(pendDest != DEST_NONE) != 0ull) { local_push(pendDest, pendSlot); pendDest = DEST_NONE; }
    {
      const bool leave = ns >= 0 && !(ntv.node >= 0 && ntv.node != kTravDone);
      if (__ballot(leave) != 0ull) {
        int dest = DEST_NONE;
        if (leave) {
          W.nodeB[ns].w = i2f(ntv.node); W.stack[ns][0] = ntv.sp | nsFlag;
          dest = (ntv.node == kTravDone) ? ((nsFlag & kShadeFlag) ? Q_SHADE : Q_GEN) : Q_LEAF;
        }
        local_push(dest, ns);
        if (leave) ns = -1;
      }
      if (nqCount > 0 && __ballot(ns < 0) != 0ull) {
        const unsigned long long m = __ballot(ns < 0);
        const int n = min((int)__popcll(m), nqCount);
        if (ns < 0) {
          const int r = lane_rank(m);
          if (r < n) {
            ns = myNodeQ[(nqHead + r) & (RC - 1)];
            const v4 na = W.nodeA[ns], nb = W.nodeB[ns];
            const int spw = W.stack[ns][0];
            nray.o = mk3(na.x, na.y, na.z); ntv.tbest = na.w;
            ntv.inv = mk3(node_inv(nb.x), node_inv(nb.y), node_inv(nb.z)); ntv.node = f2i(nb.w);
            ntv.noi = neg_o_inv(nray.o, ntv.inv);
            ntv.sp = spw & ~kSlotFlags; nsFlag = spw & kSlotFlags;
          }
        }
        nqHead = (nqHead + n) & (RC - 1); nqCount -= n;
      }
    }
    const int nActive = __popcll(__ballot(ns >= 0));
    const bool starving = nActive <= 64 - a.starveLanes;
    int pass = -1;
    int mySlot = -1;
    auto leaf_pop = [&]() -> int {
      const int n = min(64, lqCount);
      const int slot = lane < n ? (int)myLeafQ[(lqHead + lane) & 255] : -1;
      lqHead = (lqHead + n) & 255; lqCount -= n;
      return slot;
    };
    const bool flush = obCount[0] >= 32 || obCount[1] >= 32;
    if (!flush && (lqCount >= 64 || (starving && lqCount >= 32))) {
      pass = 0; mySlot = leaf_pop();
      PT_SUB(tLocal);
    } else if (starving || flush) {
      PT_SUB(tLocal);
      txn_begin();
      for (int d = 0; d < 2; d++) {
        const int q = Q_SHADE + d;
        for (int base = 0; base < obCount[d]; base += 64) {
          const int i = base + lane;
          if (i < obCount[d]) W.queue[q][(qHead[q] + qCount[q] + i) & (RC - 1)] = sPriv[wave].outbox[d][i];
        }
        qCount[q] += obCount[d]; obCount[d] = 0;
      }
      nDone += localDone; localDone = 0;
      if (qCount[Q_SHADE] >= 64) pass = 1;
      else if (qCount[Q_GEN] >= 64) pass = 2;
      else if (lqCount >= 64) pass = 0;
      else if (starving) {
        const int l = lqCount, sh = qCount[Q_SHADE], g = qCount[Q_GEN];
        if (l + sh + g == 0) { if (nActive == 0) pass = (nDone == NS) ? 4 : 3; }
        else pass = (l >= sh && l >= g) ? 0 : (sh >= g ? 1 : 2);
      }
      if (pass == 1 || pass == 2) mySlot = q_pop(pass == 1 ? Q_SHADE : Q_GEN, true);
      txn_end();
      if (pass == 0) mySlot = leaf_pop();
      PT_SUB(tTxn);
    } else PT_SUB(tLocal);
    PT_STAMP(tSwap);
    if (pass == 4) break;
    if (pass == 3) { if (CNT) idleSpins++; __builtin_amdgcn_s_sleep(32); PT_SUB(tIdle); PT_STAMP(tSwap); continue; }
    if (pass == 0) { leaf_pass(mySlot); PT_STAMP(tLeaf); continue; }
    if (pass > 0) { run_batch(mySlot, pass == 1); PT_STAMP(tBatch); continue; }

    if (CNT) { nodeRuns++; ringBacklog += (unsigned long long)nqCount; leafBacklog += (unsigned long long)lqCount; }
    {
      SlotStack st = make_stack(ns >= 0 ? ns : 0);
      for (;;) {
        const bool atNode = ns >= 0 && ntv.node >= 0 && ntv.node != kTravDone;
        const unsigned long long m = __ballot(atNode);
        const int n = __popcll(m);
        if (n == 0 || nActive - n >= a.swapLanes) break;
        if (CNT) { nodeSteps++; nodeLanes += (uint32_t)n; }
        if (atNode) trav_node_step<CNT>(sc, nray, ntv, st, ct);
      }
    }
    PT_STAMP(tNode);
  }

  if constexpr (CNT) {
    unsigned long long* c = a.counters;
    uint32_t v[kCntPerLane];
    wave_sum_counters(ct, v);
    if (lane == 0) {
      for (int i = 0; i < kCntPerLane; i++) atomicAdd(&c[i], (unsigned long long)v[i]);
      atomicAdd(&c[kCntTraversalSteps], (unsigned long long)nodeSteps + leafPasses);
      atomicAdd(&c[kCntActiveLaneSteps], (unsigned long long)nodeLanes + leafLanes);
      atomicAdd(&c[kCntShadeBatches], (unsigned long long)batches);
      atomicAdd(&c[kCntShadeBatchLanes], (unsigned long long)batchLanes);
      atomicAdd(&c[kCntIdleSpins], (unsigned long long)idleSpins);
      atomicAdd(&c[kCntTBatch], tBatch); atomicAdd(&c[kCntTSwap], tSwap); atomicAdd(&c[kCntTNode], tNode); atomicAdd(&c[kCntTLeaf], tLeaf);
      atomicAdd(&c[kCntTWave], __builtin_amdgcn_s_memtime() - tStart);
      atomicAdd(&c[kCntLeafPasses], (unsigned long long)leafPasses); atomicAdd(&c[kCntLeafLanes], (unsigned long long)leafLanes);
      atomicMax(&c[kCntLastWaveOut], (unsigned long long)__builtin_amdgcn_s_memrealtime());
      atomicMin(&c[kCntFirstWaveIn], rtStart);
      atomicAdd(&c[kCntTLocal], tLocal); atomicAdd(&c[kCntTLock], tLock); atomicAdd(&c[kCntTTxn], tTxn); atomicAdd(&c[kCntTIdle], tIdle);
      atomicAdd(&c[kCntNodeRuns], nodeRuns); atomicAdd(&c[kCntRingBacklog], ringBacklog); atomicAdd(&c[kCntLeafBacklog], leafBacklog);
      atomicAdd(&c[kCntIterResult], nIterResult); atomicAdd(&c[kCntIterLights], nIterLights); atomicAdd(&c[kCntIterNewItem], nIterGen);
      atomicAdd(&c[kCntTBatchLoad], tBLoad); atomicAdd(&c[kCntTBatchRun], tBRun); atomicAdd(&c[kCntTBatchStore], tBStore); atomicAdd(&c[kCntTransactions], nTxn); atomicAdd(&c[kCntIterations], nIter);
    }
  }
}

}

#ifndef PT_QK_EXPORT
#define PT_QK_EXPORT(name) name
#endif
int PT_QK_EXPORT(queuekernel_lds_stack_entries)() { return kStackN; }
int PT_QK_EXPORT(queuekernel_slots)() { return kP; }
size_t PT_QK_EXPORT(queuekernel_cold_bytes)(int nBlocks) { return (size_t)nBlocks * kWaves * kP * sizeof(SlotCold); }
size_t PT_QK_EXPORT(queuekernel_overflow_ints)(int nBlocks, int ovfDepth) { return (size_t)nBlocks * kWaves * kP * (size_t)ovfDepth; }

template <bool CNT, bool FAST>
static void launch_qk(dim3 grid, dim3 block, hipStream_t stream, const LaunchArgs& a) {
  if (a.scene.shadowNearest) pt_queuekernel<CNT, true, FAST, true><<<grid, block, 0, stream>>>(a);
  else                       pt_queuekernel<CNT, true, FAST, false><<<grid, block, 0, stream>>>(a);
}
hipError_t PT_QK_EXPORT(launch_queuekernel)(hipStream_t stream, const LaunchArgs& a, int nBlocks, bool counted, bool fastShading, int ) {
  dim3 grid(nBlocks), block(kBlockThreads);
  if (fastShading) { if (counted) launch_qk<true, true>(grid, block, stream, a); else launch_qk<false, true>(grid, block, stream, a); }
  else             { if (counted) launch_qk<true, false>(grid, block, stream, a); else launch_qk<false, false>(grid, block, stream, a); }
  return hipGetLastError();
}

}
```

Measured before the change: 9155.

## Add slim packet-kernel specialization without aux shadow slots or glass attenuation

Adds a compile-time specialized packet kernel that strips the auxiliary shadow-slot machinery (atomics, free masks, join flags) and glass shadow attenuation when the scene has no glass material and aux depth is zero. It also forces auxDepth to zero for large sample counts when slots_in_use is left on auto, so the slim kernel is chosen in that case. The aim is lower register pressure and fewer LDS atomics and branches in the hot traversal and shading loop. The trade-off is losing the aux-slot shadow parallelism for large renders, plus extra kernel instantiations.

```diff
diff --git a/minimaloptix_amd/csrc/api_context.h b/minimaloptix_amd/csrc/api_context.h
--- a/minimaloptix_amd/csrc/api_context.h
+++ b/minimaloptix_amd/csrc/api_context.h
@@ -109,6 +109,7 @@
   unsigned long long probeCounts[4] = { 0, 0, 0, 0 };
   int lastVariant = -1;
   int lastFeatures = pt::FEAT_ALL;
+  int lastSlim = 0;
   int countedSpanUs = -1, countedTailUs = -1;
   double kernelMs = 0.0, reduceMs = 0.0; uint64_t nLaunches = 0;
   bool asyncPending = false;
@@ -286,6 +287,7 @@
   const TraceKernel* kernel;
   int variant;
   int features;
+  bool slim;
   int nItems, tilesX;
   int nBlocks;
   long long perPass;
diff --git a/minimaloptix_amd/csrc/api_options.hip b/minimaloptix_amd/csrc/api_options.hip
--- a/minimaloptix_amd/csrc/api_options.hip
+++ b/minimaloptix_amd/csrc/api_options.hip
@@ -53,6 +53,7 @@
   { "node_format_used", nullptr, [](moptix_context c) { return c->nodeFormatUsed; } },
   { "kernel_variant_used", nullptr, [](moptix_context c) { return c->lastVariant; } },
   { "kernel_features_used", nullptr, [](moptix_context c) { return c->lastFeatures; } },
+  { "kernel_slim_used", nullptr, [](moptix_context c) { return c->lastSlim; } },
   { "counted_span_us", nullptr, [](moptix_context c) { return c->countedSpanUs; } },
   { "counted_tail_us", nullptr, [](moptix_context c) { return c->countedTailUs; } },
   { "path_slots", nullptr, [](moptix_context) { return packetkernel_slots(); } },
diff --git a/minimaloptix_amd/csrc/api_render.hip b/minimaloptix_amd/csrc/api_render.hip
--- a/minimaloptix_amd/csrc/api_render.hip
+++ b/minimaloptix_amd/csrc/api_render.hip
@@ -136,10 +136,12 @@
   if (p.kernel == &kLeanQueueKernel && c->opt.blocksPerCU == 3) p.nBlocks = c->numCUs * 4;
   p.slotsInUse = c->opt.slotsInUse >= 0 ? c->opt.slotsInUse : (usePacket && c->opt.auxDepth > 0 && nSamples < 1.0e8 && c->glassFaceShare <= 0.5 ? packetkernel_slots() * 7 / 8 : 0);
   p.auxDepth = usePacket ? c->opt.auxDepth : 0;
+  if (usePacket && c->opt.slotsInUse < 0 && nSamples >= 1.0e8) p.auxDepth = 0;
   if (usePacket) {
     bool glassMaterial = false;
     for (const DevMaterial& m : c->mats) if (m.kind == MAT_DISNEY && m.brdfType == BRDF_GLASS) glassMaterial = true;
     p.drainBelow = (glassMaterial && !scene.shadowNearest) ? 0 : c->opt.drainBelow;
+    p.slim = p.auxDepth == 0 && (scene.shadowNearest || !glassMaterial);
   }
   if (p.kernel) {
     p.ovfDepth = hasTris ? std::max(0, c->bvh.stackBound - p.kernel->lds_stack_entries() + 1) : 0;
@@ -201,6 +203,7 @@
   c->lastVariant = p.variant;
   r.counted = counted; r.fast = c->opt.fastShading != 0;
   c->lastFeatures = p.kernel == &kPacketKernel ? packetkernel_features(r.counted, r.fast, p.features) : FEAT_ALL;
+  c->lastSlim = (p.kernel == &kPacketKernel && c->lastFeatures == 0 && p.slim) ? 1 : 0;
 
   a.accum = accum_ptr(c);
   a.nItems = p.nItems; a.tilesX = p.tilesX; a.rank = c->rank; a.nRanks = c->nRanks;
@@ -291,7 +294,7 @@
   if (over) a.tileOrder = over->order;
   else if (a.tileMajor && a.tileCost) HIPCHK(c, c->tiles.sort(c->stream), "sort tiles");
   HIPCHK(c, hipEventRecord(c->ev0, c->stream), "event");
-  if (p.kernel) HIPCHK(c, p.kernel->launch(c->stream, a, p.nBlocks, r.counted, r.fast, p.features), p.kernel->launchWhat);
+  if (p.kernel) HIPCHK(c, p.kernel->launch(c->stream, a, p.nBlocks, r.counted, r.fast, p.features, p.slim), p.kernel->launchWhat);
   else HIPCHK(c, launch_megakernel(c->stream, a, p.nBlocks, r.counted), "launch megakernel");
   if (p.drainBelow > 0) HIPCHK(c, launch_drainkernel(c->stream, a, c->numCUs, r.counted, r.fast), "launch drain kernel");
   else if (p.kernel == &kPacketKernel) HIPCHK(c, launch_megakernel(c->stream, a, p.nBlocks, r.counted), "launch megakernel");
diff --git a/minimaloptix_amd/csrc/megakernel.h b/minimaloptix_amd/csrc/megakernel.h
--- a/minimaloptix_amd/csrc/megakernel.h
+++ b/minimaloptix_amd/csrc/megakernel.h
@@ -121,24 +121,24 @@
 int queuekernel_slots();
 size_t queuekernel_cold_bytes(int nBlocks);
 size_t queuekernel_overflow_ints(int nBlocks, int ovfDepth);
-hipError_t launch_queuekernel(hipStream_t stream, const LaunchArgs& a, int nBlocks, bool counted, bool fastShading, int features);
+hipError_t launch_queuekernel(hipStream_t stream, const LaunchArgs& a, int nBlocks, bool counted, bool fastShading, int features, bool slim);
 int queuekernel_lds_stack_entries_lean();
 int queuekernel_slots_lean();
 size_t queuekernel_cold_bytes_lean(int nBlocks);
 size_t queuekernel_overflow_ints_lean(int nBlocks, int ovfDepth);
-hipError_t launch_queuekernel_lean(hipStream_t stream, const LaunchArgs& a, int nBlocks, bool counted, bool fastShading, int features);
+hipError_t launch_queuekernel_lean(hipStream_t stream, const LaunchArgs& a, int nBlocks, bool counted, bool fastShading, int features, bool slim);
 int packetkernel_lds_stack_entries();
 int packetkernel_slots();
 size_t packetkernel_cold_bytes(int nBlocks);
 size_t packetkernel_overflow_ints(int nBlocks, int ovfDepth);
-hipError_t launch_packetkernel(hipStream_t stream, const LaunchArgs& a, int nBlocks, bool counted, bool fastShading, int features);
+hipError_t launch_packetkernel(hipStream_t stream, const LaunchArgs& a, int nBlocks, bool counted, bool fastShading, int features, bool slim);
 int packetkernel_features(bool counted, bool fastShading, int sceneFeatures);
 struct TraceKernel {
   const char* launchWhat;
   int (*lds_stack_entries)();
   size_t (*cold_bytes)(int nBlocks);
   size_t (*overflow_ints)(int nBlocks, int ovfDepth);
-  hipError_t (*launch)(hipStream_t stream, const LaunchArgs& a, int nBlocks, bool counted, bool fastShading, int features);
+  hipError_t (*launch)(hipStream_t stream, const LaunchArgs& a, int nBlocks, bool counted, bool fastShading, int features, bool slim);
 };
 inline constexpr TraceKernel kQueueKernel = { "launch queue megakernel", queuekernel_lds_stack_entries, queuekernel_cold_bytes, queuekernel_overflow_ints, launch_queuekernel };
 inline constexpr TraceKernel kLeanQueueKernel = { "launch queue megakernel (lean)", queuekernel_lds_stack_entries_lean, queuekernel_cold_bytes_lean, queuekernel_overflow_ints_lean, launch_queuekernel_lean };
diff --git a/minimaloptix_amd/csrc/packetkernel.hip b/minimaloptix_amd/csrc/packetkernel.hip
--- a/minimaloptix_amd/csrc/packetkernel.hip
+++ b/minimaloptix_amd/csrc/packetkernel.hip
@@ -1,4 +1,6 @@
 #include <hip/hip_runtime.h>
+
+#include <type_traits>
 
 #include "megakernel.h"
 #include "pt_lanestack.h"
@@ -102,14 +104,44 @@
   }
 };
 
+struct OwnSlotSink {
+  SlotCold* cold; int slot; v4* nodeA; v4* nodeB; const PathState* ps; int root;
+  __device__ __forceinline__ OwnSlotSink(SlotCold* cold_, int slot_, v4* nodeA_, v4* nodeB_, int (*)[kStackN + 1], const PathState* ps_, int root_, int )
+      : cold(cold_), slot(slot_), nodeA(nodeA_), nodeB(nodeB_), ps(ps_), root(root_) {}
+  __device__ __forceinline__ void shadow(int j, v3 d, float tmax, v3 w, float inv) const {
+    SlotCold* cw = at32(cold, slot);
+    slot_store(&cw->pend[j], mk4(w.x, w.y, w.z, inv));
+    if (j == 0) { nodeA[slot] = mk4(ps->o.x, ps->o.y, ps->o.z, tmax); nodeB[slot] = mk4(d.x, d.y, d.z, i2f(root)); }
+    else slot_store(&cw->ray[j - 1], mk4(d.x, d.y, d.z, tmax));
+  }
+};
+
+#ifdef PT_PK_SLIM_GLASS
+constexpr bool kSlimKeepsGlass = true;
+#else
+constexpr bool kSlimKeepsGlass = false;
+#endif
+#ifdef PT_PK_SLIM_AUX
+constexpr bool kSlimKeepsAux = true;
+#else
+constexpr bool kSlimKeepsAux = false;
+#endif
 template <bool CNT, bool SHARED, bool FAST = false, bool NEAR = false, bool N64 = false>
 __global__ void __launch_bounds__(kBlockThreads, kWavesPerSimd) pt_packetkernel(const LaunchArgs a) {
   constexpr int F = 0;
+  constexpr bool AUX = kSlimKeepsAux, GLASS = NEAR || kSlimKeepsGlass;
+#include "packetkernel_body.h"
+}
+template <bool CNT, bool SHARED, bool FAST = false, bool NEAR = false, bool N64 = false>
+__global__ void __launch_bounds__(kBlockThreads, kWavesPerSimd) pt_packetkernel_aux(const LaunchArgs a) {
+  constexpr int F = 0;
+  constexpr bool AUX = true, GLASS = true;
 #include "packetkernel_body.h"
 }
 template <bool CNT, bool SHARED, bool FAST = false, bool NEAR = false, bool N64 = false>
 __global__ void __launch_bounds__(kBlockThreads, kWavesPerSimd) pt_packetkernel_general(const LaunchArgs a) {
   constexpr int F = FEAT_ALL;
+  constexpr bool AUX = true, GLASS = true;
 #include "packetkernel_body.h"
 }
 
@@ -133,19 +165,23 @@
   if (a.scene.shadowNearest) pt_packetkernel_general<CNT, true, FAST, true, kThisFileN64><<<grid, block, 0, stream>>>(a);
   else                       pt_packetkernel_general<CNT, true, FAST, false, kThisFileN64><<<grid, block, 0, stream>>>(a);
 }
-hipError_t PT_PK_LAUNCH(hipStream_t stream, const LaunchArgs& a, int nBlocks, bool counted, bool fastShading, int features) {
+hipError_t PT_PK_LAUNCH(hipStream_t stream, const LaunchArgs& a, int nBlocks, bool counted, bool fastShading, int features, bool slim) {
   dim3 grid(nBlocks), block(kBlockThreads);
-  if (packetkernel_features(counted, fastShading, features) == 0) {
+  if (packetkernel_features(counted, fastShading, features) == 0 && slim) {
+    if (a.auxDepth != 0 && !kSlimKeepsAux) return hipErrorInvalidValue;
     if (a.scene.shadowNearest) pt_packetkernel<false, true, false, true, kThisFileN64><<<grid, block, 0, stream>>>(a);
     else                       pt_packetkernel<false, true, false, false, kThisFileN64><<<grid, block, 0, stream>>>(a);
+  } else if (packetkernel_features(counted, fastShading, features) == 0) {
+    if (a.scene.shadowNearest) pt_packetkernel_aux<false, true, false, true, kThisFileN64><<<grid, block, 0, stream>>>(a);
+    else                       pt_packetkernel_aux<false, true, false, false, kThisFileN64><<<grid, block, 0, stream>>>(a);
   } else if (fastShading) { if (counted) launch_pk<true, true>(grid, block, stream, a); else launch_pk<false, true>(grid, block, stream, a); }
   else             { if (counted) launch_pk<true, false>(grid, block, stream, a); else launch_pk<false, false>(grid, block, stream, a); }
   return hipGetLastError();
 }
 #ifndef PT_PK_N128
-hipError_t launch_packetkernel_n128(hipStream_t stream, const LaunchArgs& a, int nBlocks, bool counted, bool fastShading, int features);
-hipError_t launch_packetkernel(hipStream_t stream, const LaunchArgs& a, int nBlocks, bool counted, bool fastShading, int features) {
-  return a.scene.nodes64 != nullptr ? launch_packetkernel_n64(stream, a, nBlocks, counted, fastShading, features) : launch_packetkernel_n128(stream, a, nBlocks, counted, fastShading, features);
+hipError_t launch_packetkernel_n128(hipStream_t stream, const LaunchArgs& a, int nBlocks, bool counted, bool fastShading, int features, bool slim);
+hipError_t launch_packetkernel(hipStream_t stream, const LaunchArgs& a, int nBlocks, bool counted, bool fastShading, int features, bool slim) {
+  return a.scene.nodes64 != nullptr ? launch_packetkernel_n64(stream, a, nBlocks, counted, fastShading, features, slim) : launch_packetkernel_n128(stream, a, nBlocks, counted, fastShading, features, slim);
 }
 #endif
 
diff --git a/minimaloptix_amd/csrc/packetkernel_body.h b/minimaloptix_amd/csrc/packetkernel_body.h
--- a/minimaloptix_amd/csrc/packetkernel_body.h
+++ b/minimaloptix_amd/csrc/packetkernel_body.h
@@ -1,3 +1,4 @@
+  static_assert(GLASS || !NEAR, "a scene whose shadow rays keep their nearest candidate has a Disney GLASS material");
   constexpr int NS = SHARED ? kP * kWaves : kP;
   __shared__ PoolLds<NS> sPool[SHARED ? 1 : kWaves];
   __shared__ WavePriv<NS> sPriv[kWaves];
@@ -71,14 +72,17 @@
   };
 
   auto store_flags = [&](int slot, int value) {
+    if constexpr (!AUX) W.stack[slot][0] = value;
+    else {
     if (__builtin_expect((value & kHasAux) != 0, 0)) { atomicAnd(&W.stack[slot][0], kJoinMask); atomicOr(&W.stack[slot][0], value & ~kJoinMask); }
     else W.stack[slot][0] = value;
-  };
-  auto arrive_parks = [&](int slot) -> bool {
+    }
+  };
+  [[maybe_unused]] auto arrive_parks = [&](int slot) -> bool {
     const int old = atomicOr(&W.stack[slot][0], kArrived);
     return ((old >> kJoinShift) & 3) != 0;
   };
-  auto aux_done = [&](int fl, int& dest) -> int {
+  [[maybe_unused]] auto aux_done = [&](int fl, int& dest) -> int {
     const int parent = aux_parent(fl);
     const int old = atomicSub(&W.stack[parent][0], 1 << kJoinShift);
     const bool last = (old & kJoinMask) == ((1 << kJoinShift) | kArrived);
@@ -86,14 +90,16 @@
     return last ? parent : -1;
   };
 
-  const bool auxOn = SHARED && a.auxDepth > 0 && sc.rootRef >= 0;
+  [[maybe_unused]] const bool auxOn = SHARED && a.auxDepth > 0 && sc.rootRef >= 0;
   const int nUse = (a.slotsInUse > 0 && a.slotsInUse < NS) ? (SHARED ? a.slotsInUse : max(64, a.slotsInUse / kWaves)) : NS;
   {
+    if constexpr (AUX) {
     if (SHARED && threadIdx.x < NS / 32) {
       const int lo = (int)threadIdx.x * 32;
       W.freeMask[threadIdx.x] = !auxOn || nUse >= lo + 32 ? 0u : (nUse <= lo ? ~0u : ~0u << (nUse - lo));
     }
     if (threadIdx.x == 0) W.nFree = auxOn ? NS - nUse : 0;
+    }
     const int first = SHARED ? threadIdx.x : lane, step = SHARED ? kBlockThreads : 64;
     for (int s = first; s < nUse; s += step) {
       i4 ctl; ctl.x = -1; ctl.y = 0; ctl.z = 0; ctl.w = M_NEW_PIXEL;
@@ -190,7 +196,9 @@
       const bool more = fl_more(fl);
       if (more && (isSwitch || shadow || (fl & kSpMask) == 0)) { wn = slot_load(&cs->ray[cur]); PT_ROWS(2, 1); }
       if (!isSwitch) {
+        if constexpr (GLASS) {
         if (shadow) { if (fl_stat(fl, cur) == 2) { wr = slot_load(&cs->att[cur]); PT_ROWS(2, 1); } }
+        }
       }
       auto next_ray = [&](int flags) {
         const int nxt = cur + 1;
@@ -211,14 +219,18 @@
         tv.inv = mk3(0.f, 0.f, 0.f); tv.tbest = na.w;
         tv.node = node0; tv.sp = fl & kSpMask;
         tv.bestTri = -1; tv.bestPrim = -1; tv.beta = 0.f; tv.gamma = 0.f; tv.att = mk3(1.f, 1.f, 1.f); tv.bestCls = SHADOW_NONE;
+        if constexpr (GLASS) {
         if (shadow) { if (fl_stat(fl, cur) == 2) { tv.att = mk3(wr.x, wr.y, wr.z); if (sc.shadowNearest) tv.bestPrim = f2i(wr.w); } }
         else if (hitValid) tv.bestPrim = kPrimUnknown;
+        } else { if (!shadow && hitValid) tv.bestPrim = kPrimUnknown; }
         const int oldPrim = tv.bestPrim;
-        const v3 oldAtt = tv.att;
+        [[maybe_unused]] const v3 oldAtt = tv.att;
         SlotStack st = make_stack(slot);
-        trav_leaf_step_fetched<CNT>(sc, ps, tv, st, ct, ch);
+        trav_leaf_step_fetched<CNT, GLASS>(sc, ps, tv, st, ct, ch);
         int nfl = fl & ~kSpMask;
-        if (shadow) {
+        if (!GLASS && shadow) {
+          if (tv.att.x == 0.f) nfl = (nfl & ~(3 << (kStatShift + 2 * cur))) | (1 << (kStatShift + 2 * cur));
+        } else if (shadow) {
           if (sc.shadowNearest) {
             if (tv.bestPrim != oldPrim) {
               nfl = (nfl & ~(3 << (kStatShift + 2 * cur))) | (2 << (kStatShift + 2 * cur));
@@ -244,11 +256,13 @@
           W.nodeB[slot].w = i2f(tv.node);
           store_flags(slot, tv.sp | nfl);
           pendDest = tv.node == kTravDone ? ((nfl & kShadeFlag) ? Q_SHADE : Q_GEN) : (tv.node >= 0 ? Q_NODE : Q_LEAF);
+          if constexpr (AUX) {
           if (__builtin_expect(tv.node == kTravDone && (nfl & (kHasAux | kAuxSlot)) != 0, 0)) {
             if (nfl & kAuxSlot) {
               __builtin_amdgcn_fence(__ATOMIC_RELEASE, "workgroup");
               pendSlot = aux_done(nfl, pendDest);
             } else if (arrive_parks(slot)) pendDest = DEST_NONE;
+          }
           }
         }
       }
@@ -279,7 +293,7 @@
       const int fl = W.stack[slot][0];
       const bool hitValid = (fl & kHitValid) != 0;
       const int nSh = (fl >> kPendShift) & 3;
-      const bool hadAux = (fl & kHasAux) != 0;
+      const bool hadAux = AUX && (fl & kHasAux) != 0;
       const i4 ctl = slot_load(&cs->ctl);
 #ifdef PT_EVLOG
       if (ctl.y >= 100) sEvOn = 1;
@@ -287,7 +301,7 @@
       const v4 thrIn = slot_load(&cs->thr), radIn = slot_load(&cs->rad);
       v4 wh = mk4(0.f, 0.f, 0.f, 0.f), wb = mk4(1.f, 1.f, 1.f, 1.f);
       v4 wp[kPacketShadows], wa[kPacketShadows];
-      if (ctl.w & kCtlHoldsAux) axp = f2i(thrIn.w);
+      if constexpr (AUX) { if (ctl.w & kCtlHoldsAux) axp = f2i(thrIn.w); }
       PT_ROWS(0, 3);
       if (hitValid) { wh = slot_load(&cs->hit); PT_ROWS(0, 1); }
       if (fl & kHasScale) { wb = slot_load(&cs->bsc); PT_ROWS(0, 1); }
@@ -298,8 +312,10 @@
           wp[i] = slot_load(&cs->pend[i]); PT_ROWS(0, 1);
           const int ax = (axp >> (kSlotBits * i)) & kSlotMask;
           const int stt = hadAux ? fl_stat(W.stack[ax][0], 0) : fl_stat(fl, i);
+          if constexpr (GLASS) {
           if (stt == 2) { wa[i] = hadAux ? slot_load(&at32(cold, ax)->att[0]) : slot_load(&cs->att[i]); PT_ROWS(0, 1); }
           else if (stt == 1) wa[i] = mk4(0.f, 0.f, 0.f, 0.f);
+          } else { if (stt == 1) wa[i] = mk4(0.f, 0.f, 0.f, 0.f); }
         }
       }
       const v4 na = W.nodeA[slot], wd = W.nodeB[slot];
@@ -317,7 +333,8 @@
       if (hitValid) { res.bestTri = f2i(wh.x); res.bestPrim = f2i(wh.y); res.beta = wh.z; res.gamma = wh.w; }
       if (ps.mode == M_TRACE) ps.mode = M_RESULT;
     }
-    const SlotSink sink{ cold, slot >= 0 ? slot : 0, W.nodeA, W.nodeB, W.stack, &ps, sc.rootRef, axp };
+    using Sink = std::conditional_t<AUX, SlotSink, OwnSlotSink>;
+    const Sink sink{ cold, slot >= 0 ? slot : 0, W.nodeA, W.nodeB, W.stack, &ps, sc.rootRef, axp };
     if (CNT) { __builtin_amdgcn_s_waitcnt(0); PT_SUB(tBLoad); }
 #ifdef PT_EVLOG
     __builtin_amdgcn_s_waitcnt(0); PT_EV(2, 0);
@@ -343,7 +360,7 @@
       }
       if (run) {
         if (ps.mode == M_RESULT) {
-          on_result_packet<CNT, FAST, SlotSink, (F == 0 && !N64) ? FEAT_SPLIT_HIT : F>(sc, ps, pk, res, att, ct, sink);
+          on_result_packet<CNT, FAST, Sink, (F == 0 && !N64) ? FEAT_SPLIT_HIT : F>(sc, ps, pk, res, att, ct, sink);
         } else {
           int k = atomicAdd(a.workCounter, 1);
           if constexpr (F == 0) {
@@ -368,12 +385,15 @@
     bool useAux = false;
     if (have) {
       SlotCold* cw = at32(cold, slot);
+      if constexpr (AUX) {
       if (axp >= 0 && !(ps.mode == M_TRACE && ps.depth >= a.auxDepth)) {
         for (int j = 0; j < kPacketShadows; j++) { const int ax = (axp >> (kSlotBits * j)) & kSlotMask; atomicOr(&W.freeMask[ax >> 5], 1u << (ax & 31)); }
         atomicAdd(&W.nFree, kPacketShadows);
         axp = -1;
       }
+      }
       int axpNext = axp;
+      if constexpr (AUX) {
       if (auxOn) {
         const bool wantAux = axp < 0 && ps.mode == M_TRACE && ps.depth >= a.auxDepth;
         if (wantAux && W.nFree >= kPacketShadows) {
@@ -390,6 +410,7 @@
           if (got == kPacketShadows) { axpNext = pack; atomicSub(&W.nFree, kPacketShadows); }
           else for (int j = 0; j < got; j++) { const int ax = (pack >> (kSlotBits * j)) & kSlotMask; atomicOr(&W.freeMask[ax >> 5], 1u << (ax & 31)); }
         }
+      }
       }
       i4 ctl; ctl.x = ps.item; ctl.y = ps.depth; ctl.z = (int)ps.seed;
       ctl.w = ps.mode | (pk.nShadow << 3) | (pk.hasBounce << 5) | (pk.hasScale << 6);
@@ -409,7 +430,7 @@
         const bool hitNow = bp0 >= 0;
         if (hitNow) { slot_store(&cw->hit, mk4(i2f(-1), i2f(bp0), 0.f, 0.f)); PT_ROWS(1, 1); }
         PT_ROWS(1, pk.nShadow + ((axp >= 0 || pk.nShadow == 0) ? 0 : pk.nShadow - 1));
-        useAux = axp >= 0 && pk.nShadow > 0;
+        if constexpr (AUX) useAux = axp >= 0 && pk.nShadow > 0;
         const int nOwnSh = useAux ? 0 : pk.nShadow;
         const int nRays = nOwnSh + pk.hasBounce;
         const v4 rb = mk4(ps.d.x, ps.d.y, ps.d.z, tb0);
@@ -434,13 +455,17 @@
       } else {
         W.stack[slot][0] = 0;
         pendDest = (ps.mode == M_NEW_PIXEL) ? Q_GEN : DEST_DONE;
+        if constexpr (AUX) {
         if (auxOn && ps.mode != M_NEW_PIXEL) {
           atomicOr(&W.freeMask[slot >> 5], 1u << (slot & 31)); atomicAdd(&W.nFree, 1);
         }
-      }
-    }
+        }
+      }
+    }
+    if constexpr (AUX) {
     if (auxOn && __ballot(useAux) != 0ull) {
       for (int j = 0; j < kPacketShadows; j++) local_push((useAux && j < pk.nShadow) ? Q_NODE : DEST_NONE, (axp >> (kSlotBits * j)) & kSlotMask);
+    }
     }
     if constexpr (!SHARED) __builtin_amdgcn_fence(__ATOMIC_RELEASE, "workgroup");
     PT_SUB(tBStore);
@@ -461,11 +486,13 @@
           const int nodeOut = (ntv.node == kTravDone && fl_more(nsFlag)) ? kSwitchRef : ntv.node;
           W.nodeB[ns].w = i2f(nodeOut); store_flags(ns, ntv.sp | nsFlag);
           dest = (nodeOut == kTravDone) ? ((nsFlag & kShadeFlag) ? Q_SHADE : Q_GEN) : Q_LEAF;
+          if constexpr (AUX) {
           if (__builtin_expect(nodeOut == kTravDone && (nsFlag & (kHasAux | kAuxSlot)) != 0, 0)) {
             if (nsFlag & kAuxSlot) {
               __builtin_amdgcn_fence(__ATOMIC_RELEASE, "workgroup");
               pushSlot = aux_done(nsFlag, dest);
             } else if (arrive_parks(ns)) dest = DEST_NONE;
+          }
           }
         }
         local_push(dest, pushSlot);
@@ -581,6 +608,7 @@
         int fl = W.stack[slot][0];
         const i4 ctl = slot_load(&cw->ctl);
         if ((ctl.w & 7) != M_TRACE) continue;
+        if constexpr (AUX) {
         if (fl & kHasAux) {
           const int axp = f2i(slot_load(&cw->thr).w);
           const int nS = (fl >> kPendShift) & 3;
@@ -594,6 +622,7 @@
             }
           }
           fl &= ~(kHasAux | kJoinMask);
+        }
         }
         const v4 na = W.nodeA[slot], nb = W.nodeB[slot];
         slot_store(&cw->spare[0], na);
diff --git a/minimaloptix_amd/csrc/pt_path.h b/minimaloptix_amd/csrc/pt_path.h
--- a/minimaloptix_amd/csrc/pt_path.h
+++ b/minimaloptix_amd/csrc/pt_path.h
@@ -71,9 +71,10 @@
   att = (m.brdfType == BRDF_GLASS) ? m.color : mk3(0.f, 0.f, 0.f);
 }
 
+template <bool GLASS = true>
 PT_HD bool shadow_any_hit_tri(const SceneView& sc, int cls, int mat, v3& att) {
   if (cls == SHADOW_NONE) return false;
-  if (cls == SHADOW_GLASS) { att = att * load_const(&at32(sc.mats, mat)->color); return false; }
+  if constexpr (GLASS) { if (cls == SHADOW_GLASS) { att = att * load_const(&at32(sc.mats, mat)->color); return false; } }
   att = mk3(0.f, 0.f, 0.f);
   return true;
 }
@@ -325,7 +326,7 @@
     ch.p0[j] = tp->p0; ch.e0[j] = tp->e0; ch.e1[j] = tp->e1; ch.mat[j] = tp->mat; ch.prim[j] = tp->prim; ch.shadow[j] = tp->shadow;
   }
 }
-template <bool CNT, class Stack>
+template <bool CNT, bool GLASS = true, class Stack>
 PT_HD void trav_leaf_step_fetched(const SceneView& sc, const PathState& ps, Trav& tv, Stack& st, Counters& ct, LeafChunk& ch) {
   {
     const int first = leaf_first(tv.node), count = leaf_count(tv.node);
@@ -347,7 +348,7 @@
               }
             } else if (sc.shadowNearest) {
               shadow_candidate_tri(sc, ch.shadow[j], ch.mat[j], t, triBase + ch.prim[j], ps.tmin, tv.tbest, tv.bestPrim, tv.att);
-            } else if (shadow_any_hit_tri(sc, ch.shadow[j], ch.mat[j], tv.att)) terminated = true;
+            } else if (shadow_any_hit_tri<GLASS>(sc, ch.shadow[j], ch.mat[j], tv.att)) terminated = true;
           }
         }
       }
diff --git a/minimaloptix_amd/csrc/queuekernel.hip b/minimaloptix_amd/csrc/queuekernel.hip
--- a/minimaloptix_amd/csrc/queuekernel.hip
+++ b/minimaloptix_amd/csrc/queuekernel.hip
@@ -559,7 +559,7 @@
   if (a.scene.shadowNearest) pt_queuekernel<CNT, true, FAST, true><<<grid, block, 0, stream>>>(a);
   else                       pt_queuekernel<CNT, true, FAST, false><<<grid, block, 0, stream>>>(a);
 }
-hipError_t PT_QK_EXPORT(launch_queuekernel)(hipStream_t stream, const LaunchArgs& a, int nBlocks, bool counted, bool fastShading, int ) {
+hipError_t PT_QK_EXPORT(launch_queuekernel)(hipStream_t stream, const LaunchArgs& a, int nBlocks, bool counted, bool fastShading, int , bool ) {
   dim3 grid(nBlocks), block(kBlockThreads);
   if (fastShading) { if (counted) launch_qk<true, true>(grid, block, stream, a); else launch_qk<false, true>(grid, block, stream, a); }
   else             { if (counted) launch_qk<true, false>(grid, block, stream, a); else launch_qk<false, false>(grid, block, stream, a); }
```

New measurement: 9520, median of 6. 1.04x the previous value.
